# CUHK-AIM-Group/Depth-Aware-Endoscopy-SR

Hardware: AMD Instinct MI355X
Metric: LR frames/sec fwd+bwd at x8 (128x160 LR) (higher is better)
Workload: dtype f32; 1 GPU; Kvasir x8 synthetic, batch=16 per GPU, fp32, DepthNet nb=16 nf=64 L=256 K=10 (BASELINE.json configs[1]); step = fwd + L1 + dynamic loss + bwd + Adam; global_batch=16, scale=8, parallelism=dp1, mode=train, device=cuda, full=False, hip_graph=False

## Files before the change

### depth-aware-endoscopy-sr_amd/csrc/conv_api.hip

```cpp
#include "dasr_common.h"
#include "conv_kernels.h"

static int check_geom(const ConvGeom& g) {
    if (g.B <= 0 || g.H <= 0 || g.W <= 0 || g.Cin <= 0 || g.Ho <= 0 || g.Wo <= 0 || g.Cout <= 0 || g.KH <= 0 ||
        g.KW <= 0 || g.stride <= 0 || g.pad < 0)
        return DASR_E_SHAPE;
    int eh, ew;
    if (!g.transposed) {
        eh = (g.H + 2 * g.pad - g.KH) / g.stride + 1;
        ew = (g.W + 2 * g.pad - g.KW) / g.stride + 1;
    } else {
        eh = (g.H - 1) * g.stride - 2 * g.pad + g.KH;
        ew = (g.W - 1) * g.stride - 2 * g.pad + g.KW;
    }
    if (eh != g.Ho || ew != g.Wo) return DASR_E_SHAPE;
    return DASR_OK;
}

static int conv2d_fwd_dispatch(const ConvGeom& g, const float* x, const float* w, const float* bias, const float* residual,
                               float* y, int act, int ps_r, void* stream) {
    if (conv_mfma_supported(g)) return conv_mfma_fwd(g, x, w, bias, residual, y, act, ps_r, stream);
    if (conv_c1_supported(g) && ps_r == 1 && !residual) return conv_c1_fwd(g, x, w, bias, y, act, stream);
    if (conv9_mfma_supported(g) && act == DASR_ACT_NONE && ps_r == 1 && !residual)
        return conv9_mfma_fwd(g, x, w, bias, y, stream);
    if (conv_gather_fwd_supported(g) && ps_r == 1 && !residual) return conv_gather_fwd(g, x, w, bias, y, act, stream);
    return conv_direct_fwd(g, x, w, bias, residual, y, act, ps_r, stream);
}
extern "C" int dasr_conv2d_fwd(const float* x, const float* w, const float* bias, const float* residual, float* y,
                               float* y_amax, int B, int H, int W, int Cin, int Ho, int Wo, int Cout, int KH, int KW,
                               int stride, int pad, int transposed, int act, int ps_r, void* stream) {
    DASR_CHECK_PTR(x); DASR_CHECK_PTR(w); DASR_CHECK_PTR(y);
    ConvGeom g{B, H, W, Cin, Ho, Wo, Cout, KH, KW, stride, pad, transposed};
    int rc = check_geom(g);
    if (rc) return rc;
    if (act < 0 || act > 2) return DASR_E_UNSUPPORTED;
    if (ps_r < 1) ps_r = 1;
    if (ps_r > 1 && (Cout % (ps_r * ps_r)) != 0) return DASR_E_SHAPE;
    if (!y_amax) return conv2d_fwd_dispatch(g, x, w, bias, residual, y, act, ps_r, stream);
    if (!conv_mfma_supported(g) && conv_c1_supported(g) && ps_r == 1 && !residual)
        return conv_c1_fwd(g, x, w, bias, y, act, stream, y_amax);
    rc = conv2d_fwd_dispatch(g, x, w, bias, residual, y, act, ps_r, stream);
    if (rc) return rc;
    return absmax_raise(y, (size_t)B * Ho * Wo * Cout, y_amax, stream);
}

extern "C" size_t dasr_conv2d_fwd_stats_workspace(int B, int H, int W, int Cin, int Cout) {
    if (B <= 0 || H <= 0 || W <= 0 || Cin <= 0 || Cout <= 0) return 0;
    ConvGeom g{B, H, W, Cin, H, W, Cout, 3, 3, 1, 1, 0};
    size_t fused = conv_mfma_fwd_stats_supported(g) ? conv_mfma_fwd_stats_workspace(g) : 0;
    size_t plain = dasr_instnorm_stats_workspace(B, H * W, Cout);
    return fused > plain ? fused : plain;
}
extern "C" int dasr_conv2d_fwd_stats(const float* x, const float* w, const float* bias, float* y, float* mean, float* var,
                                     void* workspace, size_t workspace_bytes, int B, int H, int W, int Cin, int Cout,
                                     void* stream) {
    DASR_CHECK_PTR(x); DASR_CHECK_PTR(w); DASR_CHECK_PTR(y); DASR_CHECK_PTR(mean); DASR_CHECK_PTR(var);
    DASR_CHECK_PTR(workspace);
    ConvGeom g{B, H, W, Cin, H, W, Cout, 3, 3, 1, 1, 0};
    int rc = check_geom(g);
    if (rc) return rc;
    if (workspace_bytes < dasr_conv2d_fwd_stats_workspace(B, H, W, Cin, Cout)) return DASR_E_WORKSPACE;
    if (conv_mfma_fwd_stats_supported(g)) return conv_mfma_fwd_stats(g, x, w, bias, y, mean, var, workspace, stream);
    rc = dasr_conv2d_fwd(x, w, bias, nullptr, y, nullptr, B, H, W, Cin, H, W, Cout, 3, 3, 1, 1, 0, DASR_ACT_NONE, 1, stream);
    if (rc) return rc;
    return dasr_instnorm_stats(y, mean, var, workspace, workspace_bytes, B, H * W, Cout, stream);
}

extern "C" int dasr_conv2d_epilogue_bwd(const float* dy, const float* y, float* dconv, float* dconv_amax, int B, int Ho, int Wo,
                                        int Cout, int act, int ps_r, void* stream) {
    DASR_CHECK_PTR(dy); DASR_CHECK_PTR(y); DASR_CHECK_PTR(dconv);
    DASR_CHECK_SHAPE(B > 0 && Ho > 0 && Wo > 0 && Cout > 0);
    if (act < 0 || act > 2) return DASR_E_UNSUPPORTED;
    if (ps_r < 1) ps_r = 1;
    if (ps_r > 1 && (Cout % (ps_r * ps_r)) != 0) return DASR_E_SHAPE;
    ConvGeom g{B, Ho, Wo, 1, Ho, Wo, Cout, 1, 1, 1, 0, 0};
    return conv_epilogue_bwd(g, dy, y, dconv, act, ps_r, stream, dconv_amax);
}

extern "C" int dasr_conv2d_dgrad(const float* dconv, const float* w, float* dx, int accumulate, int B, int H, int W,
                                 int Cin, int Ho, int Wo, int Cout, int KH, int KW, int stride, int pad,
                                 int transposed, void* stream) {
    DASR_CHECK_PTR(dconv); DASR_CHECK_PTR(w); DASR_CHECK_PTR(dx);
    ConvGeom g{B, H, W, Cin, Ho, Wo, Cout, KH, KW, stride, pad, transposed};
    int rc = check_geom(g);
    if (rc) return rc;
    if (conv_mfma_dgrad_supported(g)) return conv_mfma_dgrad(g, dconv, w, dx, accumulate, nullptr, 0, 1, stream);
    if (conv9_mfma_supported(g)) return conv9_mfma_dgrad(g, dconv, w, dx, accumulate, nullptr, 0, 1, stream);
    if (conv_gather_dgrad_supported(g)) return conv_gather_dgrad(g, dconv, w, dx, accumulate, stream);
    return conv_direct_dgrad(g, dconv, w, dx, accumulate, stream);
}

extern "C" size_t dasr_conv2d_wgrad_workspace(int B, int H, int W, int Cin, int Ho, int Wo, int Cout, int KH, int KW,
                                              int stride, int pad, int transposed) {
    ConvGeom g{B, H, W, Cin, Ho, Wo, Cout, KH, KW, stride, pad, transposed};
    if (check_geom(g) == DASR_OK && conv_mfma_wgrad_supported(g)) return conv_mfma_wgrad_workspace(g);
    if (check_geom(g) == DASR_OK && conv9_mfma_supported(g)) return conv9_mfma_wgrad_workspace(g);
    if (check_geom(g) == DASR_OK && conv_gather_wgrad_supported(g)) return conv_gather_wgrad_workspace(g);
    return 0;
}

extern "C" int dasr_conv2d_wgrad(const float* x, const float* dconv, float* dw, float* dbias, void* workspace,
                                 size_t workspace_bytes, int B, int H, int W, int Cin, int Ho, int Wo, int Cout, int KH,
                                 int KW, int stride, int pad, int transposed, void* stream) {
    DASR_CHECK_PTR(x); DASR_CHECK_PTR(dconv); DASR_CHECK_PTR(dw);
    ConvGeom g{B, H, W, Cin, Ho, Wo, Cout, KH, KW, stride, pad, transposed};
    int rc = check_geom(g);
    if (rc) return rc;
    if (conv_c1_supported(g)) return conv_c1_wgrad(g, x, dconv, nullptr, DASR_ACT_NONE, dw, dbias, stream);
    if (conv_mfma_wgrad_supported(g)) {
        if (!workspace) return DASR_E_NULL;
        if (workspace_bytes < conv_mfma_wgrad_workspace(g)) return DASR_E_WORKSPACE;
        return conv_mfma_wgrad(g, x, dconv, dw, dbias, workspace, stream);
    } else if (conv9_mfma_supported(g)) {
        if (!workspace) return DASR_E_NULL;
        if (workspace_bytes < conv9_mfma_wgrad_workspace(g)) return DASR_E_WORKSPACE;
        rc = conv9_mfma_wgrad(g, x, dconv, dw, workspace, stream);
    } else if (conv_gather_wgrad_supported(g)) {
        if (!workspace) return DASR_E_NULL;
        if (workspace_bytes < conv_gather_wgrad_workspace(g)) return DASR_E_WORKSPACE;
        rc = conv_gather_wgrad(g, x, dconv, dw, workspace, stream);
    } else {
        rc = conv_direct_wgrad(g, x, dconv, dw, stream);
    }
    if (rc) return rc;
    if (dbias) rc = conv_colsum(dconv, dbias, (size_t)B * Ho * Wo, Cout, stream);
    return rc;
}

extern "C" int dasr_conv2d_wgrad_act(const float* x, const float* dy, const float* y, float* dw, float* dbias,
                                     float* dconv_scratch, void* workspace, size_t workspace_bytes, int B, int H, int W,
                                     int Cin, int Ho, int Wo, int Cout, int KH, int KW, int stride, int pad,
                                     int transposed, int act, void* stream) {
    DASR_CHECK_PTR(x); DASR_CHECK_PTR(dy); DASR_CHECK_PTR(y); DASR_CHECK_PTR(dw);
    ConvGeom g{B, H, W, Cin, Ho, Wo, Cout, KH, KW, stride, pad, transposed};
    int rc = check_geom(g);
    if (rc) return rc;
    if (act < 0 || act > 2) return DASR_E_UNSUPPORTED;
    if (conv_c1_supported(g)) return conv_c1_wgrad(g, x, dy, y, act, dw, dbias, stream);
    DASR_CHECK_PTR(dconv_scratch);
    rc = conv_epilogue_bwd(g, dy, y, dconv_scratch, act, 1, stream);
    if (rc) return rc;
    return dasr_conv2d_wgrad(x, dconv_scratch, dw, dbias, workspace, workspace_bytes, B, H, W, Cin, Ho, Wo, Cout, KH, KW,
                             stride, pad, transposed, stream);
}

extern "C" int dasr_conv2d_wgrad_act_fused(int B, int H, int W, int Cin, int Ho, int Wo, int Cout, int KH, int KW,
                                           int stride, int pad, int transposed) {
    ConvGeom g{B, H, W, Cin, Ho, Wo, Cout, KH, KW, stride, pad, transposed};
    if (check_geom(g) != DASR_OK) return 0;
    return conv_c1_supported(g) ? 1 : 0;
}

extern "C" int dasr_conv2d_dgrad_act_supported(int B, int H, int W, int Cin, int Ho, int Wo, int Cout, int KH, int KW,
                                               int stride, int pad, int transposed, int ps_r) {
    ConvGeom g{B, H, W, Cin, Ho, Wo, Cout, KH, KW, stride, pad, transposed};
    if (check_geom(g) != DASR_OK) return 0;
    if (ps_r < 1) ps_r = 1;
    if ((H % ps_r) != 0 || (W % ps_r) != 0) return 0;
    return (conv_mfma_dgrad_supported(g) || conv9_mfma_supported(g)) ? 1 : 0;
}

extern "C" int dasr_conv2d_dgrad_act(const float* dconv, const float* w, const float* x_act, float* dprev, int B, int H,
                                     int W, int Cin, int Ho, int Wo, int Cout, int KH, int KW, int stride, int pad,
                                     int transposed, int act, int ps_r, void* stream) {
    DASR_CHECK_PTR(dconv); DASR_CHECK_PTR(w); DASR_CHECK_PTR(x_act); DASR_CHECK_PTR(dprev);
    if (act < 0 || act > 2) return DASR_E_UNSUPPORTED;
    if (!dasr_conv2d_dgrad_act_supported(B, H, W, Cin, Ho, Wo, Cout, KH, KW, stride, pad, transposed, ps_r))
        return DASR_E_UNSUPPORTED;
    ConvGeom g{B, H, W, Cin, Ho, Wo, Cout, KH, KW, stride, pad, transposed};
    if (conv_mfma_dgrad_supported(g)) return conv_mfma_dgrad(g, dconv, w, dprev, 0, x_act, act, ps_r, stream);
    return conv9_mfma_dgrad(g, dconv, w, dprev, 0, x_act, act, ps_r, stream);
}

static int bf16_kind(const ConvGeom& g) {
    if (conv_bf16_supported(g)) return 1;
    if (conv_c1_supported(g)) return 2;
    if (conv9_mfma_supported(g)) return 3;
    return 0;
}
extern "C" int dasr_conv2d_fwd_bf16(const void* x, const void* w, const float* bias, const unsigned short* residual,
                                    void* y, int B, int H, int W, int Cin, int Ho, int Wo, int Cout, int KH, int KW,
                                    int stride, int pad, int transposed, int act, int ps_r, void* stream) {
    DASR_CHECK_PTR(x); DASR_CHECK_PTR(w); DASR_CHECK_PTR(y);
    ConvGeom g{B, H, W, Cin, Ho, Wo, Cout, KH, KW, stride, pad, transposed};
    int rc = check_geom(g);
    if (rc) return rc;
    if (act < 0 || act > 2) return DASR_E_UNSUPPORTED;
    if (ps_r < 1) ps_r = 1;
    if (ps_r > 1 && (Cout % (ps_r * ps_r)) != 0) return DASR_E_SHAPE;
    switch (bf16_kind(g)) {
        case 1:
            return conv_bf16_fwd(g, (const bf16_t*)x, (const bf16_t*)w, bias, (const bf16_t*)residual, (bf16_t*)y, act, ps_r,
                                 stream);
        case 2:
            if (ps_r != 1 || residual) return DASR_E_UNSUPPORTED;
            return conv_c1_fwd_bf16(g, (const float*)x, (const float*)w, bias, (bf16_t*)y, act, stream);
        case 3:
            if (ps_r != 1 || residual || act != DASR_ACT_NONE) return DASR_E_UNSUPPORTED;
            return conv9_bf16_fwd(g, (const bf16_t*)x, (const float*)w, bias, (float*)y, stream);
    }
    return DASR_E_UNSUPPORTED;
}
extern "C" int dasr_conv2d_epilogue_bwd_bf16(const unsigned short* dy, const unsigned short* y, unsigned short* dconv,
                                             int B, int Ho, int Wo, int Cout, int act, int ps_r, void* stream) {
    DASR_CHECK_PTR(dy); DASR_CHECK_PTR(y); DASR_CHECK_PTR(dconv);
    DASR_CHECK_SHAPE(B > 0 && Ho > 0 && Wo > 0 && Cout > 0);
    if (act < 0 || act > 2) return DASR_E_UNSUPPORTED;
    if (ps_r < 1) ps_r = 1;
    if (ps_r > 1 && (Cout % (ps_r * ps_r)) != 0) return DASR_E_SHAPE;
    ConvGeom g{B, Ho, Wo, 1, Ho, Wo, Cout, 1, 1, 1, 0, 0};
    return conv_epilogue_bwd_bf16(g, (const bf16_t*)dy, (const bf16_t*)y, (bf16_t*)dconv, act, ps_r, stream);
}
extern "C" int dasr_conv2d_dgrad_bf16(const void* dconv, const void* w, unsigned short* dx, int accumulate, int B, int H,
                                      int W, int Cin, int Ho, int Wo, int Cout, int KH, int KW, int stride, int pad,
                                      int transposed, void* stream) {
    DASR_CHECK_PTR(dconv); DASR_CHECK_PTR(w); DASR_CHECK_PTR(dx);
    ConvGeom g{B, H, W, Cin, Ho, Wo, Cout, KH, KW, stride, pad, transposed};
    int rc = check_geom(g);
    if (rc) return rc;
    if (conv_bf16_dgrad_supported(g))
        return conv_bf16_dgrad(g, (const bf16_t*)dconv, (const bf16_t*)w, (bf16_t*)dx, accumulate, stream);
    if (conv9_mfma_supported(g))
        return conv9_bf16_dgrad(g, (const float*)dconv, (const float*)w, (bf16_t*)dx, accumulate, stream);
    return DASR_E_UNSUPPORTED;
}
extern "C" size_t dasr_conv2d_wgrad_workspace_bf16(int B, int H, int W, int Cin, int Ho, int Wo, int Cout, int KH, int KW,
                                                   int stride, int pad, int transposed) {
    ConvGeom g{B, H, W, Cin, Ho, Wo, Cout, KH, KW, stride, pad, transposed};
    if (check_geom(g) != DASR_OK) return 0;
    if (conv_bf16_wgrad_supported(g)) return conv_bf16_wgrad_workspace(g);
    if (conv9_mfma_supported(g)) return conv9_bf16_wgrad_workspace(g);
    return 0;
}
extern "C" int dasr_conv2d_wgrad_bf16(const unsigned short* x, const void* dconv, float* dw, float* dbias, void* workspace,
                                      size_t workspace_bytes, int B, int H, int W, int Cin, int Ho, int Wo, int Cout, int KH,
                                      int KW, int stride, int pad, int transposed, void* stream) {
    DASR_CHECK_PTR(x); DASR_CHECK_PTR(dconv); DASR_CHECK_PTR(dw); DASR_CHECK_PTR(workspace);
    ConvGeom g{B, H, W, Cin, Ho, Wo, Cout, KH, KW, stride, pad, transposed};
    int rc = check_geom(g);
    if (rc) return rc;
    if (conv_bf16_wgrad_supported(g)) {
        if (workspace_bytes < conv_bf16_wgrad_workspace(g)) return DASR_E_WORKSPACE;
        return conv_bf16_wgrad(g, (const bf16_t*)x, (const bf16_t*)dconv, dw, dbias, workspace, stream);
    }
    if (conv9_mfma_supported(g)) {
        if (workspace_bytes < conv9_bf16_wgrad_workspace(g)) return DASR_E_WORKSPACE;
        rc = conv9_bf16_wgrad(g, (const bf16_t*)x, (const float*)dconv, dw, workspace, stream);
        if (rc) return rc;
        if (dbias) rc = conv_colsum((const float*)dconv, dbias, (size_t)B * Ho * Wo, Cout, stream);
        return rc;
    }
    return DASR_E_UNSUPPORTED;
}
extern "C" int dasr_conv2d_wgrad_act_bf16(const float* x, const unsigned short* dy, const unsigned short* y, float* dw,
                                          float* dbias, int B, int H, int W, int Cin, int Ho, int Wo, int Cout, int KH,
                                          int KW, int stride, int pad, int transposed, int act, void* stream) {
    DASR_CHECK_PTR(x); DASR_CHECK_PTR(dy); DASR_CHECK_PTR(y); DASR_CHECK_PTR(dw);
    ConvGeom g{B, H, W, Cin, Ho, Wo, Cout, KH, KW, stride, pad, transposed};
    int rc = check_geom(g);
    if (rc) return rc;
    if (act < 0 || act > 2) return DASR_E_UNSUPPORTED;
    if (!conv_c1_supported(g)) return DASR_E_UNSUPPORTED;
    return conv_c1_wgrad_bf16(g, x, (const bf16_t*)dy, (const bf16_t*)y, act, dw, dbias, stream);
}
```

### depth-aware-endoscopy-sr_amd/csrc/conv_c1.hip

```cpp
#include "dasr_common.h"
#include "bf16.h"
#include "conv_kernels.h"

#define C1_MAXW 4096
template <int CIN>
__device__ __forceinline__ void c1_stage_rows(const float* __restrict__ x, float* sRow, int b, int y, int H, int W) {
    const float* xb = x + (size_t)b * H * W * CIN;
    const int RW = (W + 2) * CIN, n = 3 * RW;
    for (int i0 = threadIdx.x; i0 < n; i0 += 4 * 256) {
        float v[4];
        bool in[4];
#pragma unroll
        for (int u = 0; u < 4; ++u) {
            const int i = i0 + 256 * u < n ? i0 + 256 * u : 0;
            const int r = i / RW, c = i - r * RW;
            const int iy = y + r - 1, ix = c / CIN - 1;
            in[u] = iy >= 0 && iy < H && ix >= 0 && ix < W;
            v[u] = xb[in[u] ? ((size_t)iy * W + ix) * CIN + c % CIN : 0];
        }
#pragma unroll
        for (int u = 0; u < 4; ++u)
            if (i0 + 256 * u < n) sRow[i0 + 256 * u] = in[u] ? v[u] : 0.f;
    }
}

template <typename T, int CIN>
__global__ void __launch_bounds__(256) k_conv3x3_c1_fwd(const float* __restrict__ x, const float* __restrict__ w,
                                                        const float* __restrict__ bias, T* __restrict__ y, int B,
                                                        int H, int W, int Cout, int act, float* __restrict__ amax) {
    DASR_DYN_SMEM(smem);
    float* sRow = (float*)smem;
    const int nq = Cout / 4;
    const int q = threadIdx.x % nq, pl = threadIdx.x / nq, npl = 256 / nq;
    constexpr int NT = 9 * CIN;
    const int RW = (W + 2) * CIN;
    float4 wt[NT];
#pragma unroll
    for (int t = 0; t < NT; ++t) wt[t] = *(const float4*)(w + (size_t)t * Cout + 4 * q);
    const float4 bv = bias ? *(const float4*)(bias + 4 * q) : make_float4(0.f, 0.f, 0.f, 0.f);
    const float slope = act == DASR_ACT_LRELU02 ? 0.2f : 1.f;
    const bool relu = act == DASR_ACT_RELU;
    auto neg = [&](float v) { return relu ? 0.f : slope * v; };
    float om = 0.f;
    for (int row = blockIdx.x; row < B * H; row += gridDim.x) {
        const int b = row / H, py = row - b * H;
        __syncthreads();
        c1_stage_rows<CIN>(x, sRow, b, py, H, W);
        __syncthreads();
        T* yrow = y + ((size_t)row * W) * Cout + 4 * q;
        for (int px = pl; px < W; px += npl) {
            float4 acc = bv;
#pragma unroll
            for (int t = 0; t < NT; ++t) {
                const float d = sRow[(t / (3 * CIN)) * RW + (px + (t / CIN) % 3) * CIN + t % CIN];
                acc.x = fmaf(d, wt[t].x, acc.x); acc.y = fmaf(d, wt[t].y, acc.y);
                acc.z = fmaf(d, wt[t].z, acc.z); acc.w = fmaf(d, wt[t].w, acc.w);
            }
            acc.x = acc.x > 0.f ? acc.x : neg(acc.x); acc.y = acc.y > 0.f ? acc.y : neg(acc.y);
            acc.z = acc.z > 0.f ? acc.z : neg(acc.z); acc.w = acc.w > 0.f ? acc.w : neg(acc.w);
            st4(yrow + (size_t)px * Cout, acc);
            om = dasr_amax4(om, acc);
        }
    }
    if (amax) dasr_amax_commit(amax, om, sRow, dasr_flat_wg(), dasr_flat_nwg());
}

template <typename T, int CIN, bool HASY>
__global__ void __launch_bounds__(256) k_conv3x3_c1_wgrad(const float* __restrict__ x, const T* __restrict__ dy,
                                                          const T* __restrict__ yact, float* __restrict__ dw,
                                                          float* __restrict__ dbias, int B, int H, int W, int Cout,
                                                          int act) {
    DASR_DYN_SMEM(smem);
    constexpr int NT = 9 * CIN;
    const int RW = (W + 2) * CIN;
    float* red = (float*)smem;
    float* sRow = red + 256 * 4;
    const int nq = Cout / 4;
    const int q = threadIdx.x % nq, pl = threadIdx.x / nq, npl = 256 / nq;
    const float slope = act == DASR_ACT_RELU ? 0.f : act == DASR_ACT_LRELU02 ? 0.2f : 1.f;
    float4 acc[NT + 1];
#pragma unroll
    for (int t = 0; t < NT + 1; ++t) acc[t] = make_float4(0.f, 0.f, 0.f, 0.f);
    constexpr int NPX = sizeof(T) == 2 ? 8 : 4;
    typedef typename raw4<T>::type Raw;
    Raw gq[NPX], yq[NPX];
    const int nrows = B * H, step = NPX * npl;
    auto issue = [&](int row, int base) {
        const size_t ro = ((size_t)row * W) * Cout + 4 * q;
#pragma unroll
        for (int u = 0; u < NPX; ++u) {
            const int px = base + pl + u * npl < W ? base + pl + u * npl : W - 1;
            gq[u] = ld4_raw(dy + ro + (size_t)px * Cout);
            if (HASY) yq[u] = ld4_raw(yact + ro + (size_t)px * Cout);
        }
    };
    if ((int)blockIdx.x < nrows) issue(blockIdx.x, 0);
    for (int row = blockIdx.x; row < nrows; row += gridDim.x) {
        const int b = row / H, py = row - b * H;
        __syncthreads();
        c1_stage_rows<CIN>(x, sRow, b, py, H, W);
        __syncthreads();
        for (int base = 0; base < W; base += step) {
            float4 g[NPX];
#pragma unroll
            for (int u = 0; u < NPX; ++u) {
                g[u] = cvt4<T>(gq[u]);
                if (HASY) {
                    const float4 yv = cvt4<T>(yq[u]);
                    g[u].x *= yv.x > 0.f ? 1.f : slope; g[u].y *= yv.y > 0.f ? 1.f : slope;
                    g[u].z *= yv.z > 0.f ? 1.f : slope; g[u].w *= yv.w > 0.f ? 1.f : slope;
                }
            }
            {
                int nb = base + step, nr = row;
                if (nb >= W) {
                    nb = 0;
                    nr = row + (int)gridDim.x < nrows ? row + (int)gridDim.x : row;
                }
                DASR_SCHED_BARRIER();
                issue(nr, nb);
                DASR_SCHED_BARRIER();
            }
#pragma unroll
            for (int u = 0; u < NPX; ++u) {
                const int px = base + pl + u * npl;
                if (px >= W) g[u] = make_float4(0.f, 0.f, 0.f, 0.f);
                const int pc = px < W ? px : W - 1;
                acc[NT].x += g[u].x; acc[NT].y += g[u].y; acc[NT].z += g[u].z; acc[NT].w += g[u].w;
#pragma unroll
                for (int t = 0; t < NT; ++t) {
                    const float d = sRow[(t / (3 * CIN)) * RW + (pc + (t / CIN) % 3) * CIN + t % CIN];
                    acc[t].x = fmaf(d, g[u].x, acc[t].x); acc[t].y = fmaf(d, g[u].y, acc[t].y);
                    acc[t].z = fmaf(d, g[u].z, acc[t].z); acc[t].w = fmaf(d, g[u].w, acc[t].w);
                }
            }
        }
    }
#pragma unroll
    for (int t = 0; t < NT + 1; ++t) {
        __syncthreads();
        *(float4*)(red + threadIdx.x * 4) = acc[t];
        __syncthreads();
        for (int co = threadIdx.x; co < Cout; co += 256) {
            const int qq = co / 4, j = co % 4;
            float s = 0.f;
            for (int l = 0; l < npl; ++l) s += red[(l * nq + qq) * 4 + j];
            if (t < NT) atomicAdd(&dw[(size_t)t * Cout + co], s);
            else if (dbias) atomicAdd(&dbias[co], s);
        }
    }
}

__global__ void __launch_bounds__(256) k_c1_zero(float* __restrict__ dw, int nw, float* __restrict__ dbias, int nb) {
    const int i = blockIdx.x * 256 + threadIdx.x;
    if (i < nw) dw[i] = 0.f;
    else if (dbias && i < nw + nb) dbias[i - nw] = 0.f;
}

bool conv_c1_supported(const ConvGeom& g) {
    return g.KH == 3 && g.KW == 3 && g.stride == 1 && g.pad == 1 && !g.transposed && (g.Cin == 1 || g.Cin == 3) &&
           (g.Cout % 4) == 0 && g.Cout <= (g.Cin == 1 ? 1024 : 256) && (256 % (g.Cout / 4)) == 0 && g.H == g.Ho &&
           g.W == g.Wo && g.W <= C1_MAXW;
}
template <typename T>
static int conv_c1_fwd_impl(const ConvGeom& g, const float* x, const float* w, const float* bias, T* y, int act, void* stream,
                            float* amax = nullptr) {
    unsigned grid = (unsigned)(g.B * g.H);
    if (grid > 256 * 8) grid = 256 * 8;
    const size_t lds = sizeof(float) * 3 * (g.W + 2) * g.Cin;
    if (g.Cin == 3) DASR_LAUNCH((k_conv3x3_c1_fwd<T, 3>), dim3(grid), dim3(256), lds, stream, x, w, bias, y, g.B, g.H, g.W, g.Cout, act, amax);
    else            DASR_LAUNCH((k_conv3x3_c1_fwd<T, 1>), dim3(grid), dim3(256), lds, stream, x, w, bias, y, g.B, g.H, g.W, g.Cout, act, amax);
    DASR_RETURN_LAUNCH_STATUS();
}
int conv_c1_fwd(const ConvGeom& g, const float* x, const float* w, const float* bias, float* y, int act, void* stream,
                float* amax) {
    return conv_c1_fwd_impl<float>(g, x, w, bias, y, act, stream, amax);
}
int conv_c1_fwd_bf16(const ConvGeom& g, const float* x, const float* w, const float* bias, bf16_t* y, int act, void* stream) {
    return conv_c1_fwd_impl<bf16_t>(g, x, w, bias, y, act, stream);
}
template <typename T>
static int conv_c1_wgrad_impl(const ConvGeom& g, const float* x, const T* dy, const T* yact, int act, float* dw, float* dbias,
                              void* stream) {
    DASR_LAUNCH(k_c1_zero, dim3(dasr_cdiv((size_t)(9 * g.Cin + 1) * g.Cout, 256)), dim3(256), 0, stream, dw, 9 * g.Cin * g.Cout,
                dbias, g.Cout);
    unsigned grid = (unsigned)(g.B * g.H);
#ifndef C1_WGRAD_WGS_BF16
#define C1_WGRAD_WGS_BF16 1024
#endif
#ifndef C1_WGRAD_WGS_F32
#define C1_WGRAD_WGS_F32 512
#endif
    const unsigned cap = sizeof(T) == 2 ? C1_WGRAD_WGS_BF16 : C1_WGRAD_WGS_F32;
    if (grid > cap) grid = cap;
    const size_t lds = sizeof(float) * (256 * 4 + 3 * (g.W + 2) * g.Cin);
#define C1_WGRAD(CIN, HASY) \
    DASR_LAUNCH((k_conv3x3_c1_wgrad<T, CIN, HASY>), dim3(grid), dim3(256), lds, stream, x, dy, yact, dw, dbias, g.B, g.H, g.W, g.Cout, act)
    const bool hasy = yact != nullptr && act != DASR_ACT_NONE;
    if (g.Cin == 3) { if (hasy) C1_WGRAD(3, true); else C1_WGRAD(3, false); }
    else            { if (hasy) C1_WGRAD(1, true); else C1_WGRAD(1, false); }
#undef C1_WGRAD
    DASR_RETURN_LAUNCH_STATUS();
}
int conv_c1_wgrad(const ConvGeom& g, const float* x, const float* dy, const float* yact, int act, float* dw, float* dbias,
                  void* stream) {
    return conv_c1_wgrad_impl<float>(g, x, dy, yact, act, dw, dbias, stream);
}
int conv_c1_wgrad_bf16(const ConvGeom& g, const float* x, const bf16_t* dy, const bf16_t* yact, int act, float* dw,
                       float* dbias, void* stream) {
    return conv_c1_wgrad_impl<bf16_t>(g, x, dy, yact, act, dw, dbias, stream);
}
```

### depth-aware-endoscopy-sr_amd/csrc/conv_direct.hip

```cpp
#include "dasr_common.h"
#include "bf16.h"
#include "conv_kernels.h"

__global__ void __launch_bounds__(256) k_conv_direct_fwd(ConvGeom g, const float* __restrict__ x,
                                                         const float* __restrict__ w, const float* __restrict__ bias,
                                                         const float* __restrict__ residual, float* __restrict__ y,
                                                         int act, int ps_r) {
    size_t n = (size_t)g.B * g.Ho * g.Wo * g.Cout;
    for (size_t idx = (size_t)blockIdx.x * blockDim.x + threadIdx.x; idx < n; idx += (size_t)gridDim.x * blockDim.x) {
        int co = (int)(idx % g.Cout);
        size_t pix = idx / g.Cout;
        int ox = (int)(pix % g.Wo), oy = (int)((pix / g.Wo) % g.Ho), b = (int)(pix / ((size_t)g.Wo * g.Ho));
        float acc = bias ? bias[co] : 0.f;
        for (int kh = 0; kh < g.KH; ++kh) {
            int iy;
            if (!g.transposed) {
                iy = oy * g.stride - g.pad + kh;
            } else {
                int ty = oy + g.pad - kh;
                if (ty < 0 || (ty % g.stride) != 0) continue;
                iy = ty / g.stride;
            }
            if (iy < 0 || iy >= g.H) continue;
            for (int kw = 0; kw < g.KW; ++kw) {
// ... 16 lines not shown
        y[conv_out_index(g, b, oy, ox, co, ps_r)] = acc;
    }
}

template <typename T>
__global__ void __launch_bounds__(256) k_conv_epilogue_bwd(ConvGeom g, const T* __restrict__ dy,
                                                           const T* __restrict__ y, T* __restrict__ dconv,
                                                           int act, int ps_r, float* __restrict__ amax) {
    __shared__ float s_part[16];
    size_t n = (size_t)g.B * g.Ho * g.Wo * g.Cout;
    float om = 0.f;
    for (size_t idx = (size_t)blockIdx.x * blockDim.x + threadIdx.x; idx < n; idx += (size_t)gridDim.x * blockDim.x) {
        int co = (int)(idx % g.Cout);
        size_t pix = idx / g.Cout;
        int ox = (int)(pix % g.Wo), oy = (int)((pix / g.Wo) % g.Ho), b = (int)(pix / ((size_t)g.Wo * g.Ho));
        size_t o = conv_out_index(g, b, oy, ox, co, ps_r);
        const float v = ld1(dy + o) * dasr_act_grad_from_out(ld1(y + o), act);
        st1(dconv + idx, v);
        om = dasr_amax1(om, v);
    }
    if (amax) dasr_amax_commit(amax, om, s_part, dasr_flat_wg(), dasr_flat_nwg());
}

__global__ void __launch_bounds__(256) k_conv_direct_dgrad(ConvGeom g, const float* __restrict__ dconv,
                                                           const float* __restrict__ w, float* __restrict__ dx,
                                                           int accumulate) {
    size_t n = (size_t)g.B * g.H * g.W * g.Cin;
    for (size_t idx = (size_t)blockIdx.x * blockDim.x + threadIdx.x; idx < n; idx += (size_t)gridDim.x * blockDim.x) {
        int ci = (int)(idx % g.Cin);
        size_t pix = idx / g.Cin;
        int ix = (int)(pix % g.W), iy = (int)((pix / g.W) % g.H), b = (int)(pix / ((size_t)g.W * g.H));
        float acc = 0.f;
        for (int kh = 0; kh < g.KH; ++kh) {
            int oy;
            if (!g.transposed) {
                int ty = iy + g.pad - kh;
                if (ty < 0 || (ty % g.stride) != 0) continue;
                oy = ty / g.stride;
            } else {
                oy = iy * g.stride - g.pad + kh;
            }
            if (oy < 0 || oy >= g.Ho) continue;
            for (int kw = 0; kw < g.KW; ++kw) {
                int ox;
                if (!g.transposed) {
                    int tx = ix + g.pad - kw;
                    if (tx < 0 || (tx % g.stride) != 0) continue;
                    ox = tx / g.stride;
                } else {
                    ox = ix * g.stride - g.pad + kw;
                }
                if (ox < 0 || ox >= g.Wo) continue;
                const float* dp = dconv + (((size_t)b * g.Ho + oy) * g.Wo + ox) * g.Cout;
                const float* wp = w + ((size_t)(kh * g.KW + kw) * g.Cin + ci) * g.Cout;
                for (int co = 0; co < g.Cout; ++co) acc = fmaf(dp[co], wp[co], acc);
            }
        }
        dx[idx] = accumulate ? dx[idx] + acc : acc;
    }
}

__global__ void __launch_bounds__(256) k_conv_direct_wgrad(ConvGeom g, const float* __restrict__ x,
                                                           const float* __restrict__ dconv, float* __restrict__ dw,
                                                           size_t pix_per_split) {
    size_t nW = (size_t)g.KH * g.KW * g.Cin * g.Cout;
    size_t e = (size_t)blockIdx.x * blockDim.x + threadIdx.x;
    if (e >= nW) return;
    int co = (int)(e % g.Cout);
    int ci = (int)((e / g.Cout) % g.Cin);
    int tap = (int)(e / ((size_t)g.Cout * g.Cin));
    int kh = tap / g.KW, kw = tap % g.KW;
    size_t npix = (size_t)g.B * g.Ho * g.Wo;
    size_t p0 = (size_t)blockIdx.y * pix_per_split;
    size_t p1 = p0 + pix_per_split < npix ? p0 + pix_per_split : npix;
    float acc = 0.f;
    for (size_t p = p0; p < p1; ++p) {
        int ox = (int)(p % g.Wo), oy = (int)((p / g.Wo) % g.Ho), b = (int)(p / ((size_t)g.Wo * g.Ho));
        int iy, ix;
        if (!g.transposed) {
            iy = oy * g.stride - g.pad + kh;
            ix = ox * g.stride - g.pad + kw;
        } else {
            int ty = oy + g.pad - kh, tx = ox + g.pad - kw;
            if (ty < 0 || tx < 0 || (ty % g.stride) != 0 || (tx % g.stride) != 0) continue;
            iy = ty / g.stride;
            ix = tx / g.stride;
        }
        if (iy < 0 || iy >= g.H || ix < 0 || ix >= g.W) continue;
        acc = fmaf(x[(((size_t)b * g.H + iy) * g.W + ix) * g.Cin + ci], dconv[p * g.Cout + co], acc);
    }
    atomicAdd(&dw[e], acc);
}

__global__ void __launch_bounds__(256) k_colsum(const float* __restrict__ m, float* __restrict__ out, size_t rows,
                                                int C, size_t rows_per_split) {
    __shared__ float red[256];
    int c = blockIdx.x * 64 + (threadIdx.x & 63);
    int rl = threadIdx.x >> 6;
    size_t r0 = (size_t)blockIdx.y * rows_per_split;
    size_t r1 = r0 + rows_per_split < rows ? r0 + rows_per_split : rows;
    float acc = 0.f;
    if (c < C)
        for (size_t r = r0 + rl; r < r1; r += 4) acc += m[r * C + c];
    red[threadIdx.x] = acc;
    __syncthreads();
    if (rl == 0 && c < C) atomicAdd(&out[c], red[threadIdx.x] + red[threadIdx.x + 64] + red[threadIdx.x + 128] +
                                                 red[threadIdx.x + 192]);
}

__global__ void __launch_bounds__(256) k_colsum_small(const float* __restrict__ m, float* __restrict__ out, size_t rows,
                                                      int C) {
    __shared__ float red[8][4];
    float acc[8];
#pragma unroll
    for (int c = 0; c < 8; ++c) acc[c] = 0.f;
    for (size_t r = (size_t)blockIdx.x * 256 + threadIdx.x; r < rows; r += (size_t)gridDim.x * 256) {
        const float* p = m + r * C;
#pragma unroll
        for (int c = 0; c < 8; ++c)
            if (c < C) acc[c] += p[c];
    }
#pragma unroll
    for (int c = 0; c < 8; ++c) {
        float v = acc[c];
        for (int off = 32; off > 0; off >>= 1) v += __shfl_down(v, off, 64);
        if ((threadIdx.x & 63) == 0) red[c][threadIdx.x >> 6] = v;
    }
    __syncthreads();
    if (threadIdx.x < C) atomicAdd(&out[threadIdx.x], red[threadIdx.x][0] + red[threadIdx.x][1] + red[threadIdx.x][2] +
                                                          red[threadIdx.x][3]);
}

int conv_direct_fwd(const ConvGeom& g, const float* x, const float* w, const float* bias, const float* residual,
                    float* y, int act, int ps_r, void* stream) {
    size_t n = (size_t)g.B * g.Ho * g.Wo * g.Cout;
    DASR_LAUNCH(k_conv_direct_fwd, dim3(dasr_ew_grid(n)), dim3(256), 0, stream, g, x, w, bias, residual, y, act, ps_r);
    DASR_RETURN_LAUNCH_STATUS();
}
template <typename T>
__global__ void __launch_bounds__(256) k_conv_epilogue_bwd_flat4(const T* __restrict__ dy, const T* __restrict__ y,
                                                                 T* __restrict__ dconv, size_t n4, int act,
                                                                 float* __restrict__ amax) {
    __shared__ float s_part[16];
    float om = 0.f;
    for (size_t i = (size_t)blockIdx.x * blockDim.x + threadIdx.x; i < n4; i += (size_t)gridDim.x * blockDim.x) {
        const float4 d = ld4(dy + 4 * i), v = ld4(y + 4 * i);
        const float4 o = make_float4(d.x * dasr_act_grad_from_out(v.x, act), d.y * dasr_act_grad_from_out(v.y, act),
                                     d.z * dasr_act_grad_from_out(v.z, act), d.w * dasr_act_grad_from_out(v.w, act));
        st4(dconv + 4 * i, o);
        om = dasr_amax4(om, o);
    }
    if (amax) dasr_amax_commit(amax, om, s_part, dasr_flat_wg(), dasr_flat_nwg());
}
template <int R, typename T>
__global__ void __launch_bounds__(256) k_conv_epilogue_bwd_ps(const T* __restrict__ dy, const T* __restrict__ y,
                                                              T* __restrict__ dconv, int Wo, int Cq, int act, int rows,
                                                              float* __restrict__ amax) {
    __shared__ float s_part[16];
    const int e0 = blockIdx.x * 256 + threadIdx.x;
    const bool livee = e0 < Wo * Cq;
    const int e = livee ? e0 : Wo * Cq - 1;
    const int ox = e / Cq, c = e - ox * Cq;
    const size_t srow = (size_t)Wo * R * Cq;
    float om = 0.f;
    for (size_t row0 = blockIdx.y; row0 < (size_t)rows; row0 += 2 * (size_t)gridDim.y) {
        const size_t row1 = row0 + gridDim.y;
        const bool two = row1 < (size_t)rows;
        const size_t rws[2] = {row0, two ? row1 : row0};
        float out[2][R * R];
#pragma unroll
        for (int h = 0; h < 2; ++h) {
            const T* dyp = dy + rws[h] * R * srow + (size_t)ox * R * Cq + c;
            const T* yp = y + rws[h] * R * srow + (size_t)ox * R * Cq + c;
#pragma unroll
            for (int i = 0; i < R; ++i)
#pragma unroll
                for (int j = 0; j < R; ++j) {
                    const size_t o = (size_t)i * srow + (size_t)j * Cq;
                    out[h][i * R + j] = ld1(dyp + o) * dasr_act_grad_from_out(ld1(yp + o), act);
                }
        }
#pragma unroll
        for (int h = 0; h < 2; ++h) {
            if (h == 1 && !two) break;
            T* dst = dconv + (rws[h] * Wo + ox) * (size_t)(Cq * R * R) + (size_t)c * (R * R);
            if (livee) {
                if (R == 2) {
                    st4(dst, make_float4(out[h][0], out[h][1], out[h][2], out[h][3]));
                } else {
#pragma unroll
                    for (int q = 0; q < R * R; ++q) st1(dst + q, out[h][q]);
                }
            }
#pragma unroll
            for (int q = 0; q < R * R; ++q) om = dasr_amax1(om, out[h][q]);
        }
    }
    if (amax) dasr_amax_commit(amax, om, s_part, dasr_flat_wg(), dasr_flat_nwg());
}

template <typename T>
static int conv_epilogue_bwd_impl(const ConvGeom& g, const T* dy, const T* y, T* dconv, int act, int ps_r, void* stream,
                                  float* amax = nullptr) {
    size_t n = (size_t)g.B * g.Ho * g.Wo * g.Cout;
    const size_t rows = (size_t)g.B * g.Ho;
    if (ps_r <= 1 && (n % 4) == 0) {
        DASR_LAUNCH((k_conv_epilogue_bwd_flat4<T>), dim3(dasr_ew_grid(n / 4)), dim3(256), 0, stream, dy, y, dconv, n / 4, act, amax);
    } else if ((ps_r == 2 || ps_r == 3) && (g.Cout % (ps_r * ps_r)) == 0 && rows < ((size_t)1 << 31) &&
               (size_t)g.Wo * (g.Cout / (ps_r * ps_r)) < (1u << 30)) {
        const int Cq = g.Cout / (ps_r * ps_r);
        const unsigned gx = dasr_cdiv((size_t)g.Wo * Cq, 256);
        size_t gy = rows < 65535 ? rows : 65535;
        if (amax && (size_t)gx * gy > DASR_AMAX_MAX_PARTS) gy = DASR_AMAX_MAX_PARTS / gx > 0 ? DASR_AMAX_MAX_PARTS / gx : 1;
        if (amax && (size_t)gx * gy > DASR_AMAX_MAX_PARTS) return DASR_E_UNSUPPORTED;
        const dim3 grid(gx, (unsigned)gy);
        if (ps_r == 2)
            DASR_LAUNCH((k_conv_epilogue_bwd_ps<2, T>), grid, dim3(256), 0, stream, dy, y, dconv, g.Wo, Cq, act, (int)rows, amax);
        else
            DASR_LAUNCH((k_conv_epilogue_bwd_ps<3, T>), grid, dim3(256), 0, stream, dy, y, dconv, g.Wo, Cq, act, (int)rows, amax);
    } else {
        DASR_LAUNCH((k_conv_epilogue_bwd<T>), dim3(dasr_ew_grid(n)), dim3(256), 0, stream, g, dy, y, dconv, act, ps_r, amax);
    }
    DASR_RETURN_LAUNCH_STATUS();
}
int conv_epilogue_bwd(const ConvGeom& g, const float* dy, const float* y, float* dconv, int act, int ps_r, void* stream,
                      float* amax) {
    return conv_epilogue_bwd_impl<float>(g, dy, y, dconv, act, ps_r, stream, amax);
}
int conv_epilogue_bwd_bf16(const ConvGeom& g, const bf16_t* dy, const bf16_t* y, bf16_t* dconv, int act, int ps_r,
                           void* stream) {
    return conv_epilogue_bwd_impl<bf16_t>(g, dy, y, dconv, act, ps_r, stream);
}
int conv_direct_dgrad(const ConvGeom& g, const float* dconv, const float* w, float* dx, int accumulate, void* stream) {
    size_t n = (size_t)g.B * g.H * g.W * g.Cin;
    DASR_LAUNCH(k_conv_direct_dgrad, dim3(dasr_ew_grid(n)), dim3(256), 0, stream, g, dconv, w, dx, accumulate);
    DASR_RETURN_LAUNCH_STATUS();
}
int conv_colsum(const float* m, float* out, size_t rows, int C, void* stream) {
    hipError_t e = hipMemsetAsync(out, 0, sizeof(float) * C, (hipStream_t)stream);
    if (e != hipSuccess) return (int)e;
    if (C <= 8) {
        DASR_LAUNCH(k_colsum_small, dim3(dasr_ew_grid(rows)), dim3(256), 0, stream, m, out, rows, C);
        DASR_RETURN_LAUNCH_STATUS();
    }
    unsigned nsplit = (unsigned)((rows + 255) / 256);
    if (nsplit > 2048) nsplit = 2048;
    if (nsplit < 1) nsplit = 1;
    size_t rps = (rows + nsplit - 1) / nsplit;
    DASR_LAUNCH(k_colsum, dim3(dasr_cdiv(C, 64), nsplit), dim3(256), 0, stream, m, out, rows, C, rps);
    DASR_RETURN_LAUNCH_STATUS();
}
int conv_direct_wgrad(const ConvGeom& g, const float* x, const float* dconv, float* dw, void* stream) {
    size_t nW = (size_t)g.KH * g.KW * g.Cin * g.Cout;
    hipError_t e = hipMemsetAsync(dw, 0, sizeof(float) * nW, (hipStream_t)stream);
    if (e != hipSuccess) return (int)e;
    size_t npix = (size_t)g.B * g.Ho * g.Wo;
    unsigned gx = dasr_cdiv(nW, 256);
    unsigned nsplit = 4096 / gx;
    if (nsplit < 1) nsplit = 1;
    size_t max_split = (npix + 63) / 64;
    if (nsplit > max_split) nsplit = (unsigned)max_split;
    if (nsplit > 65535) nsplit = 65535;
    size_t pps = (npix + nsplit - 1) / nsplit;
    DASR_LAUNCH(k_conv_direct_wgrad, dim3(gx, nsplit), dim3(256), 0, stream, g, x, dconv, dw, pps);
    DASR_RETURN_LAUNCH_STATUS();
}
```

### depth-aware-endoscopy-sr_amd/csrc/conv_kernels.h

```cpp
#pragma once
#include "dasr_common.h"
#include "bf16.h"

struct ConvGeom {
    int B, H, W, Cin, Ho, Wo, Cout, KH, KW, stride, pad, transposed;
};

__host__ __device__ __forceinline__ size_t conv_out_index(const ConvGeom& g, int b, int oy, int ox, int co, int ps_r) {
    if (ps_r <= 1) return (((size_t)b * g.Ho + oy) * g.Wo + ox) * g.Cout + co;
    int rr = ps_r * ps_r;
    int c = co / rr, i = (co / ps_r) % ps_r, j = co % ps_r;
    return (((size_t)b * g.Ho * ps_r + (size_t)oy * ps_r + i) * ((size_t)g.Wo * ps_r) + (size_t)ox * ps_r + j) *
               (g.Cout / rr) + c;
}

int conv_direct_fwd(const ConvGeom& g, const float* x, const float* w, const float* bias, const float* residual,
                    float* y, int act, int ps_r, void* stream);
int conv_epilogue_bwd(const ConvGeom& g, const float* dy, const float* y, float* dconv, int act, int ps_r,
                      void* stream, float* amax = nullptr);
int conv_direct_dgrad(const ConvGeom& g, const float* dconv, const float* w, float* dx, int accumulate, void* stream);
int conv_direct_wgrad(const ConvGeom& g, const float* x, const float* dconv, float* dw, void* stream);
int conv_colsum(const float* m, float* out, size_t rows, int C, void* stream);

bool conv_mfma_supported(const ConvGeom& g);
bool conv_mfma_fwd_stats_supported(const ConvGeom& g);
size_t conv_mfma_fwd_stats_workspace(const ConvGeom& g);
int conv_mfma_fwd_stats(const ConvGeom& g, const float* x, const float* w, const float* bias, float* y, float* mean,
                        float* var, void* workspace, void* stream);
bool conv_mfma_dgrad_supported(const ConvGeom& g);
bool conv_mfma_wgrad_supported(const ConvGeom& g);
int conv_mfma_fwd(const ConvGeom& g, const float* x, const float* w, const float* bias, const float* residual,
                  float* y, int act, int ps_r, void* stream);
int conv_mfma_dgrad(const ConvGeom& g, const float* dconv, const float* w, float* dx, int accumulate,
                    const float* mask_src, int mask_act, int unps_r, void* stream);
size_t conv_mfma_wgrad_workspace(const ConvGeom& g);
int conv_mfma_wgrad(const ConvGeom& g, const float* x, const float* dconv, float* dw, float* dbias, void* workspace,
                    void* stream);

bool conv9_mfma_supported(const ConvGeom& g);
int conv9_mfma_fwd(const ConvGeom& g, const float* x, const float* w, const float* bias, float* y, void* stream);
int conv9_mfma_dgrad(const ConvGeom& g, const float* dconv, const float* w, float* dx, int accumulate,
                     const float* mask_src, int mask_act, int unps_r, void* stream);
size_t conv9_mfma_wgrad_workspace(const ConvGeom& g);
int conv9_mfma_wgrad(const ConvGeom& g, const float* x, const float* dconv, float* dw, void* workspace, void* stream);

bool conv_gather_fwd_supported(const ConvGeom& g);
bool conv_gather_dgrad_supported(const ConvGeom& g);
bool conv_gather_wgrad_supported(const ConvGeom& g);
int conv_gather_fwd(const ConvGeom& g, const float* x, const float* w, const float* bias, float* y, int act,
                    void* stream);
int conv_gather_dgrad(const ConvGeom& g, const float* dconv, const float* w, float* dx, int accumulate, void* stream);
size_t conv_gather_wgrad_workspace(const ConvGeom& g);
int conv_gather_wgrad(const ConvGeom& g, const float* x, const float* dconv, float* dw, void* workspace, void* stream);
int wgrad_reduce_launch(const float* slabs, float* dw, size_t n, int P, void* stream, const float* bslabs = nullptr,
                        float* dbias = nullptr, int Cout = 0);

bool conv_c1_supported(const ConvGeom& g);
int conv_c1_fwd(const ConvGeom& g, const float* x, const float* w, const float* bias, float* y, int act, void* stream,
                float* amax = nullptr);
int absmax_raise(const float* x, size_t n, float* amax, void* stream);
int conv_c1_wgrad(const ConvGeom& g, const float* x, const float* dy, const float* yact, int act, float* dw, float* dbias,
                  void* stream);

bool conv_bf16_supported(const ConvGeom& g);
bool conv_bf16_dgrad_supported(const ConvGeom& g);
bool conv_bf16_wgrad_supported(const ConvGeom& g);
int conv_bf16_fwd(const ConvGeom& g, const bf16_t* x, const bf16_t* w, const float* bias, const bf16_t* residual,
                  bf16_t* y, int act, int ps_r, void* stream);
int conv_bf16_dgrad(const ConvGeom& g, const bf16_t* dconv, const bf16_t* w, bf16_t* dx, int accumulate, void* stream);
size_t conv_bf16_wgrad_workspace(const ConvGeom& g);
int conv_bf16_wgrad(const ConvGeom& g, const bf16_t* x, const bf16_t* dconv, float* dw, float* dbias, void* workspace,
                    void* stream);
bool conv_bf16_v2_supported(int H, int W, int Cin, int Cout, int ps_r, bool has_residual, bool accumulate);
int conv_bf16_v2_fwd(const ConvGeom& g, const bf16_t* x, const bf16_t* w, const float* bias, const bf16_t* residual,
                     bf16_t* y, int act, int ps_r, void* stream);
int conv_bf16_v2_dgrad(const ConvGeom& g, const bf16_t* dconv, const bf16_t* w, bf16_t* dx, int accumulate, void* stream);
int conv_epilogue_bwd_bf16(const ConvGeom& g, const bf16_t* dy, const bf16_t* y, bf16_t* dconv, int act, int ps_r,
                           void* stream);
int conv_c1_fwd_bf16(const ConvGeom& g, const float* x, const float* w, const float* bias, bf16_t* y, int act, void* stream);
int conv_c1_wgrad_bf16(const ConvGeom& g, const float* x, const bf16_t* dy, const bf16_t* yact, int act, float* dw,
                       float* dbias, void* stream);
int conv9_bf16_fwd(const ConvGeom& g, const bf16_t* x, const float* w, const float* bias, float* y, void* stream);
int conv9_bf16_dgrad(const ConvGeom& g, const float* dconv, const float* w, bf16_t* dx, int accumulate, void* stream);
size_t conv9_bf16_wgrad_workspace(const ConvGeom& g);
int conv9_bf16_wgrad(const ConvGeom& g, const bf16_t* x, const float* dconv, float* dw, void* workspace, void* stream);

bool conv9_split_supported(const ConvGeom& g);
int conv9_split_fwd(const ConvGeom& g, const float* x, const float* xmax, const float* w, const float* wmax, const float* bias,
                    float* y, void* stream);
int conv9_split_dgrad(const ConvGeom& g, const float* dconv, const float* dmax, const float* w, const float* wmax, float* dx,
                      int accumulate, void* stream);
size_t conv9_split_wgrad_workspace(const ConvGeom& g);
int conv9_split_wgrad(const ConvGeom& g, const float* x, const float* xmax, const float* dconv, const float* dmax, float* dw,
                      void* workspace, void* stream);
```

### depth-aware-endoscopy-sr_amd/csrc/conv_split_bf16.hip

```cpp
#include "bf16.h"
#include "conv_kernels.h"

typedef _Float16 f16_t;
typedef _Float16 f16x8 __attribute__((ext_vector_type(8)));
typedef _Float16 f16x2_t __attribute__((ext_vector_type(2)));

#define SP_HW 34
#define SP_NWV 8
#define SP_NTHR 512
#define SP_TH 16
#define SP_HPIX (18 * SP_HW)
#define SP_NHP 5
#define SP_HBYTES (SP_NHP * SP_NTHR * 16)
#define SP_EPITCH 144

DASR_DEVICE_CONST __attribute__((aligned(64))) unsigned sp_zero_page[64] = {0};

struct ConvSplitArgs {
    const float* x;
    const bf16_t* ws;
    const float* bias;
    const float* residual;
    float* y;
    int B, H, W, Cin, Cout, accumulate, act, ps_r;
    int tiles_x, tiles_y, nsl, nitems, Q, G8;
    const float* xmax;
    const float* wmax;
    float* ymax;
};

template <int N>
__device__ __forceinline__ void sp_wait_vm() {
#ifndef DASR_HIPEMU
    asm volatile("s_waitcnt vmcnt(%0)" ::"n"(N) : "memory");
#endif
}

__device__ __forceinline__ void sp_wait_vm_n(int n) {
    switch (n) {
#define SP_W(N) case N: sp_wait_vm<N>(); break;
        SP_W(0) SP_W(1) SP_W(2) SP_W(3) SP_W(4) SP_W(5) SP_W(6) SP_W(7) SP_W(8) SP_W(9) SP_W(10) SP_W(11) SP_W(12)
#undef SP_W
        default: sp_wait_vm<0>(); break;
    }
}

__device__ __forceinline__ void sp_split3(const float (&x)[8], bf16x8& a0, bf16x8& a1, bf16x8& a2) {
#pragma unroll
    for (int e = 0; e < 8; e += 2) {
        const bf16x2_t h0 = dasr_f2bf2(x[e], x[e + 1]);
        const float r0 = x[e] - dasr_bf2f(h0[0]), r1 = x[e + 1] - dasr_bf2f(h0[1]);
        const bf16x2_t h1 = dasr_f2bf2(r0, r1);
        const float s0 = r0 - dasr_bf2f(h1[0]), s1 = r1 - dasr_bf2f(h1[1]);
        const bf16x2_t h2 = dasr_f2bf2(s0, s1);
        a0[e] = h0[0]; a0[e + 1] = h0[1];
        a1[e] = h1[0]; a1[e + 1] = h1[1];
        a2[e] = h2[0]; a2[e + 1] = h2[1];
    }
}

__host__ __device__ static inline int sp_scale_exp(float m) {
    unsigned u;
    memcpy(&u, &m, 4);
    int k = 14 - ((int)((u >> 23) & 0xffu) - 127);
    return k < -60 ? -60 : (k > 60 ? 60 : k);
}
__host__ __device__ static inline float sp_pow2(int k) {
    const unsigned u = (unsigned)(127 + k) << 23;
    float f;
    memcpy(&f, &u, 4);
    return f;
}
__device__ __forceinline__ void sp_split2(const float (&x)[8], float s, f16x8& a0, f16x8& a1) {
#pragma unroll
    for (int e = 0; e < 8; e += 2) {
        const float v0 = x[e] * s, v1 = x[e + 1] * s;
        const f16_t h0 = (f16_t)v0, g0 = (f16_t)v1;
        a0[e] = h0; a0[e + 1] = g0;
        a1[e] = (f16_t)(v0 - (float)h0); a1[e + 1] = (f16_t)(v1 - (float)g0);
    }
}
template <int NP> struct SpFrag;
template <> struct SpFrag<3> {
    typedef bf16x8 type;
    typedef bf16_t elem;
    static __device__ __forceinline__ void split(const float (&x)[8], float, type (&a)[3]) { sp_split3(x, a[0], a[1], a[2]); }
    static __device__ __forceinline__ f32x16 mma(const type (&w)[3], const type (&x)[3], f32x16 c) {
        c = __builtin_amdgcn_mfma_f32_32x32x16_bf16(w[2], x[0], c, 0, 0, 0);
        c = __builtin_amdgcn_mfma_f32_32x32x16_bf16(w[1], x[1], c, 0, 0, 0);
        c = __builtin_amdgcn_mfma_f32_32x32x16_bf16(w[0], x[2], c, 0, 0, 0);
        c = __builtin_amdgcn_mfma_f32_32x32x16_bf16(w[1], x[0], c, 0, 0, 0);
        c = __builtin_amdgcn_mfma_f32_32x32x16_bf16(w[0], x[1], c, 0, 0, 0);
        c = __builtin_amdgcn_mfma_f32_32x32x16_bf16(w[0], x[0], c, 0, 0, 0);
        return c;
    }
};
template <> struct SpFrag<2> {
    typedef f16x8 type;
    typedef f16_t elem;
    static __device__ __forceinline__ void split(const float (&x)[8], float s, type (&a)[2]) { sp_split2(x, s, a[0], a[1]); }
    static __device__ __forceinline__ f32x16 mma(const type (&w)[2], const type (&x)[2], f32x16 c) {
        c = __builtin_amdgcn_mfma_f32_32x32x16_f16(w[1], x[0], c, 0, 0, 0);
        c = __builtin_amdgcn_mfma_f32_32x32x16_f16(w[0], x[1], c, 0, 0, 0);
        c = __builtin_amdgcn_mfma_f32_32x32x16_f16(w[0], x[0], c, 0, 0, 0);
        return c;
    }
};
struct SpScale { float sx, inv; };
__device__ __forceinline__ float sp_amax_share(const float* buf) {
    int n;
    memcpy(&n, buf, 4);
    float m = 0.f;
    for (int i = threadIdx.x; i < n; i += blockDim.x) m = fmaxf(m, buf[1 + i]);
#pragma unroll
    for (int o = 32; o > 0; o >>= 1) m = fmaxf(m, __shfl_xor(m, o));
    return m;
}
template <int NP>
__device__ __forceinline__ void sp_scales_gather(const float* xmax, const float* wmax, float* s_red) {
    if (NP == 2) {
        const float mx = sp_amax_share(xmax), mw = sp_amax_share(wmax);
        if ((threadIdx.x & 63) == 0) {
            s_red[threadIdx.x >> 6] = mx;
            s_red[16 + (threadIdx.x >> 6)] = mw;
        }
    }
}
template <int NP>
__device__ __forceinline__ SpScale sp_scales_take(const float* s_red) {
    SpScale r = {1.f, 1.f};
    if (NP == 2) {
        const int nw = (int)(blockDim.x >> 6);
        float mx = s_red[0], mw = s_red[16];
        for (int w = 1; w < nw; ++w) { mx = fmaxf(mx, s_red[w]); mw = fmaxf(mw, s_red[16 + w]); }
        const int kx = sp_scale_exp(mx), kw = sp_scale_exp(mw);
        r.sx = sp_pow2(kx);
        r.inv = sp_pow2(-(kx + kw));
    }
    return r;
}

typedef _Float16 f16x4 __attribute__((ext_vector_type(4)));
template <int NWV = SP_NWV>
__device__ __forceinline__ void sp_presplit(char* hb, float sx, int tid) {
    constexpr int NHP = SP_HBYTES / (1024 * NWV);
    float4 raw[NHP];
#pragma unroll
    for (int u = 0; u < NHP; ++u) raw[u] = *(const float4*)(hb + 1024 * NWV * u + 16 * tid);
#pragma unroll
    for (int u = 0; u < NHP; ++u) {
        const float f[4] = {raw[u].x * sx, raw[u].y * sx, raw[u].z * sx, raw[u].w * sx};
        f16x8 o;
#pragma unroll
        for (int j = 0; j < 4; ++j) {
            const f16_t h0 = (f16_t)f[j];
            o[j] = h0;
            o[4 + j] = (f16_t)(f[j] - (float)h0);
        }
        *(f16x8*)(hb + 1024 * NWV * u + 16 * tid) = o;
    }
}
__device__ __forceinline__ f16x8 sp_frag(const char* px, int lh, int key, int pl) {
    const f16x4 lo = *(const f16x4*)(px + ((((2 * lh) ^ key)) << 4) + 8 * pl);
    const f16x4 hi = *(const f16x4*)(px + ((((2 * lh + 1) ^ key)) << 4) + 8 * pl);
    f16x8 r;
    __builtin_memcpy(&r, &lo, 8);
    __builtin_memcpy((char*)&r + 8, &hi, 8);
    return r;
}

template <int NT, int NP, int RW = 2>
__device__ __forceinline__ void sp_epilogue(f32x16 (&acc)[RW][NT], const ConvSplitArgs& a, char* const scr, const float* sBias,
                                            const float inv, const int x0, const int y0, const int n0, const int bb,
                                            const int rbase, const int lane, const int li, const int lh, float& om) {
    const int wvalid = a.W - x0;
    const bool is_relu = a.act == DASR_ACT_RELU;
    const float slope = a.act == DASR_ACT_LRELU02 ? 0.2f : 1.f;
    const bool has_act = a.act != DASR_ACT_NONE;
#pragma unroll
    for (int m = 0; m < RW; ++m) {
        const int gy = y0 + rbase + m;
#pragma unroll
        for (int n = 0; n < NT; ++n) {
#pragma unroll
            for (int g = 0; g < 4; ++g) {
                f32x4 pk = {acc[m][n][4 * g], acc[m][n][4 * g + 1], acc[m][n][4 * g + 2], acc[m][n][4 * g + 3]};
                *(f32x4*)(scr + li * SP_EPITCH + (8 * g + 4 * lh) * 4) = pk;
            }
            DASR_WAVE_SYNC();
            if (gy < a.H) {
                if (a.ps_r == 1) {
#pragma unroll
                    for (int u = 0; u < 2; ++u) {
                        const int v = lane + 64 * u, pix = v >> 2, cg = v & 3;
                        if (pix >= wvalid) continue;
                        const float4 lo = *(const float4*)(scr + pix * SP_EPITCH + 32 * cg);
                        const float4 hi = *(const float4*)(scr + pix * SP_EPITCH + 32 * cg + 16);
                        float o[8] = {lo.x, lo.y, lo.z, lo.w, hi.x, hi.y, hi.z, hi.w};
                        if (NP == 2) {
                            const float* bp = sBias + n0 + 32 * n + 8 * cg;
#pragma unroll
                            for (int t = 0; t < 8; ++t) o[t] = fmaf(o[t], inv, bp[t]);
                        }
                        const size_t idx = (((size_t)bb * a.H + gy) * a.W + x0 + pix) * a.Cout + n0 + 32 * n + 8 * cg;
                        if (a.residual) {
                            const float4 r0 = *(const float4*)(a.residual + idx), r1 = *(const float4*)(a.residual + idx + 4);
                            o[0] += r0.x; o[1] += r0.y; o[2] += r0.z; o[3] += r0.w;
                            o[4] += r1.x; o[5] += r1.y; o[6] += r1.z; o[7] += r1.w;
                        }
                        if (has_act) {
#pragma unroll
                            for (int t = 0; t < 8; ++t) o[t] = is_relu ? fmaxf(o[t], 0.f) : fmaxf(o[t], o[t] * slope);
                        }
                        float* yp = a.y + idx;
                        if (a.accumulate) {
                            const float4 o0 = *(const float4*)yp, o1 = *(const float4*)(yp + 4);
                            o[0] += o0.x; o[1] += o0.y; o[2] += o0.z; o[3] += o0.w;
                            o[4] += o1.x; o[5] += o1.y; o[6] += o1.z; o[7] += o1.w;
                        }
                        *(float4*)yp = make_float4(o[0], o[1], o[2], o[3]);
                        *(float4*)(yp + 4) = make_float4(o[4], o[5], o[6], o[7]);
                        om = dasr_amax4(dasr_amax4(om, make_float4(o[0], o[1], o[2], o[3])), make_float4(o[4], o[5], o[6], o[7]));
                    }
                } else {
                    const int Cq = a.Cout / 4;
#pragma unroll
                    for (int u = 0; u < 2; ++u) {
                        const int v = lane + 64 * u, j = v & 1, pix = (v >> 1) & 31, i = v >> 6;
                        if (pix >= wvalid) continue;
                        const float* sp = (const float*)(scr + pix * SP_EPITCH) + 2 * i + j;
                        float o[8];
#pragma unroll
                        for (int t = 0; t < 8; ++t) {
                            const float q = NP == 2 ? fmaf(sp[4 * t], inv, sBias[n0 + 32 * n + 4 * t + 2 * i + j]) : sp[4 * t];
                            o[t] = !has_act ? q : (is_relu ? fmaxf(q, 0.f) : fmaxf(q, q * slope));
                        }
                        float* yp = a.y + (((size_t)bb * a.H * 2 + 2 * gy + i) * ((size_t)a.W * 2) + 2 * (x0 + pix) + j) * Cq +
                                    (n0 + 32 * n) / 4;
                        *(float4*)yp = make_float4(o[0], o[1], o[2], o[3]);
                        *(float4*)(yp + 4) = make_float4(o[4], o[5], o[6], o[7]);
                        om = dasr_amax4(dasr_amax4(om, make_float4(o[0], o[1], o[2], o[3])), make_float4(o[4], o[5], o[6], o[7]));
                    }
                }
            }
            DASR_WAVE_SYNC();
        }
    }
}

template <int NT, int NP, int RW = 2, int CW = 1>
__global__ void __launch_bounds__(64 * (SP_TH / RW), RW == 4 ? 1 : 2) k_conv3x3_split(ConvSplitArgs a) {
    DASR_DYN_SMEM(smem);
    typedef SpFrag<NP> F;
    static_assert(CW == 1 || (CW == 2 && NP == 2 && RW == 2 && (NT % 2) == 0), "channel halves: fp16 x 2, eight waves");
    constexpr int MR = RW * CW, NW = NT / CW;
    constexpr int NWV = SP_TH / RW, NTHR = 64 * NWV, NHP = SP_HBYTES / (16 * NTHR);
    constexpr int NTILE = 32 * NT, PIECE = NTILE * 32, SLAB = NP * PIECE;
    constexpr int WP = SLAB / 16;
    constexpr int WQ = WP / NTHR, WR = (WP - WQ * NTHR) / 64;
    char* const sH = smem;
    constexpr int TPS = NP == 2 ? 3 : 1, NS = 9 / TPS;
    constexpr int R = 3, D = 2;
    char* const sW = smem + 2 * SP_HBYTES;
    float* const sBias = (float*)(sW + R * TPS * SLAB);
    float* const sRed = sBias + a.Cout;
    const int tid = threadIdx.x, lane = tid & 63, wv = DASR_UNIFORM((int)(tid >> 6));
    const int li = lane & 31, lh = lane >> 5;
    const int wr = wv / CW, wc = wv % CW;
    const int nwq = WQ + (wv < WR ? 1 : 0);
    const dasr_lds_addr_t ldsH = DASR_LDS_ADDR(sH) + 1024 * wv, ldsW = DASR_LDS_ADDR(sW) + 1024 * wv;

    const int xcd = blockIdx.x & 7, jwg = blockIdx.x >> 3;
    const int ibeg = xcd * a.Q;
    const int iend = ibeg + a.Q < a.nitems ? ibeg + a.Q : a.nitems;
    int item = ibeg + jwg;
    if (item >= iend) {
        if (a.ymax) dasr_amax_commit_idle(a.ymax, dasr_flat_wg(), dasr_flat_nwg());
        return;
    }
    const int NC = a.Cin >> 4;
    const int pixb = a.Cin * 4, rowb = a.W * pixb;
    const size_t sampb = (size_t)a.H * rowb;
    const char* const zp = (const char*)sp_zero_page;

    for (int i = tid; i < a.Cout; i += NTHR) sBias[i] = a.bias ? a.bias[i] : 0.f;
    sp_scales_gather<NP>(a.xmax, a.wmax, sRed);
    __syncthreads();
    const SpScale sc = sp_scales_take<NP>(sRed);

    int x0, y0, n0, bb;
    auto decode = [&](int it, int& ox0, int& oy0, int& on0, int& ob) {
        const int ns = it % a.nsl, pt = it / a.nsl;
        const int tile = pt % (a.tiles_x * a.tiles_y);
        ob = pt / (a.tiles_x * a.tiles_y);
        ox0 = (tile % a.tiles_x) * 32;
        oy0 = (tile / a.tiles_x) * SP_TH;
        on0 = ns * NTILE;
    };
    decode(item, x0, y0, n0, bb);
    int hoff[NHP];
    unsigned hok = 0;
    const char* hxb;
    auto halo_setup = [&](int fx0, int fy0, int fb, bool real) {
        hxb = (const char*)a.x + (size_t)fb * sampb;
        const int org = (fy0 - 1) * rowb + (fx0 - 1) * pixb;
        int t = tid;
#ifndef DASR_HIPEMU
        asm volatile("" : "+v"(t));
#endif
        hok = 0;
#pragma unroll
        for (int u = 0; u < NHP; ++u) {
            const int P = (t >> 2) + (NTHR / 4) * u;
            const int pr = P / SP_HW, pc = P - pr * SP_HW;
            hoff[u] = org + pr * rowb + pc * pixb + 16 * ((t & 3) ^ ((P >> 2) & 3));
            const bool ok = real && P < SP_HPIX && (unsigned)(fy0 - 1 + pr) < (unsigned)a.H && (unsigned)(fx0 - 1 + pc) < (unsigned)a.W;
            hok |= ok ? (1u << u) : 0u;
        }
    };
    auto halo_issue = [&](int u, int cc, int buf) {
        const char* src = ((hok >> u) & 1u) ? hxb + hoff[u] + 64 * cc : zp;
        DASR_GLDS16(src, ldsH + buf * SP_HBYTES + 1024 * NWV * u);
    };
    auto w_issue = [&](int cc, int st, int fn0) {
#pragma unroll
        for (int j = 0; j < TPS; ++j) {
            const int tap = CW == 2 ? 3 * j + st : TPS * st + j;
            const char* src = (const char*)a.ws + (size_t)(((fn0 / NTILE) * 9 + tap) * NC + cc) * SLAB + 16 * tid;
            const dasr_lds_addr_t dst = ldsW + ((st % R) * TPS + j) * SLAB;
#pragma unroll
            for (int q = 0; q < WQ; ++q) DASR_GLDS16(src + 16 * NTHR * q, dst + 1024 * NWV * q);
            if (WR > 0 && wv < WR) DASR_GLDS16(src + 16 * NTHR * WQ, dst + 1024 * NWV * WQ);
        }
    };
    constexpr int HC0 = (NHP + 1) / 2;
    auto halo_first = [](int st) { return TPS == 1 ? st : (st == 0 ? 0 : (st == 1 ? HC0 : NHP)); };
    auto halo_count = [](int st) { return TPS == 1 ? (st < NHP ? 1 : 0) : (st == 0 ? HC0 : (st == 1 ? NHP - HC0 : 0)); };

    const int Pl = MR * wr * SP_HW + li;
    const int boff = li * 32 + ((lh ^ ((li >> 3) & 1)) << 4) + wc * NW * 1024;

    int par = 0;
    float om = 0.f;
    halo_setup(x0, y0, bb, true);
#pragma unroll
    for (int u = 0; u < NHP; ++u) halo_issue(u, 0, 0);
#pragma unroll
    for (int t = 0; t < D; ++t) w_issue(0, t, n0);

    for (;;) {
        const int nitem = item + a.G8;
        const bool has_next = nitem < iend;
        int nx0 = x0, ny0 = y0, nn0 = n0, nb = bb;
        if (has_next) decode(nitem, nx0, ny0, nn0, nb);

        f32x16 acc[MR][NW];
#pragma unroll
        for (int n = 0; n < NW; ++n)
#pragma unroll
            for (int g = 0; g < 4; ++g) {
                float4 bv = *(const float4*)(sBias + n0 + 32 * n + 8 * g + 4 * lh);
                if (NP == 2) bv = make_float4(0.f, 0.f, 0.f, 0.f);
#pragma unroll
                for (int m = 0; m < MR; ++m) {
                    acc[m][n][4 * g] = bv.x; acc[m][n][4 * g + 1] = bv.y;
                    acc[m][n][4 * g + 2] = bv.z; acc[m][n][4 * g + 3] = bv.w;
                }
            }

        for (int cc = 0; cc < NC; ++cc) {
            const bool last = cc == NC - 1;
            if (last) halo_setup(nx0, ny0, nb, has_next);
            const int fcc = last ? 0 : cc + 1;
            const char* const hb = sH + par * SP_HBYTES;
#pragma unroll
            for (int st = 0; st < NS; ++st) {
                {
                    int nh = 0;
#pragma unroll
                    for (int k = 1; k < D; ++k) nh += halo_count((st - k + NS) % NS);
                    sp_wait_vm_n(nh + (D - 1) * TPS * nwq);
                }
                if (NP == 2 && st == 0) {
                    sp_presplit<NWV>(sH + par * SP_HBYTES, sc.sx, tid);
                    DASR_LDS_BARRIER();
                } else {
                    DASR_RAW_BARRIER();
                }
#pragma unroll
                for (int u = 0; u < halo_count(st); ++u) halo_issue(halo_first(st) + u, fcc, par ^ 1);
                if (st + D < NS) w_issue(cc, st + D, n0);
                else             w_issue(fcc, st + D - NS, last ? nn0 : n0);
                if constexpr (CW == 2) {
                    int Pq = Pl;
#ifndef DASR_HIPEMU
                    asm volatile("" : "+v"(Pq));
#endif
                    typename F::type A6[MR + 2][NP];
#pragma unroll
                    for (int r = 0; r < MR + 2; ++r) {
// ... 292 lines not shown
    while (lo < hi) {
        const int mid = (lo + hi + 1) >> 1;
        if (jobs[mid].wg_begin <= (int)blockIdx.x) lo = mid; else hi = mid - 1;
    }
    const dasr_split_job J = jobs[lo];
    sp_split_weights<2>(J.w_packed, J.w_split, J.Cin, J.Cout, J.wmax, blockIdx.x - J.wg_begin, 1 << 30);
}

__global__ void __launch_bounds__(256) k_absmax(const float* __restrict__ x, size_t n4, size_t n, float* __restrict__ out) {
    __shared__ float s_part[16];
    unsigned m = 0;
    const size_t stride = (size_t)gridDim.x * 256;
    if (n4 > 0)
        for (size_t i = (size_t)blockIdx.x * 256 + threadIdx.x; i < n4; i += 4 * stride) {
            float4 v[4];
#pragma unroll
            for (int u = 0; u < 4; ++u) {
                const size_t j = i + u * stride;
                v[u] = ((const float4*)x)[j < n4 ? j : n4 - 1];
            }
#pragma unroll
            for (int u = 0; u < 4; ++u) {
                unsigned a, b, c, d;
                memcpy(&a, &v[u].x, 4); memcpy(&b, &v[u].y, 4); memcpy(&c, &v[u].z, 4); memcpy(&d, &v[u].w, 4);
                a &= 0x7fffffffu; b &= 0x7fffffffu; c &= 0x7fffffffu; d &= 0x7fffffffu;
                a = a > b ? a : b; c = c > d ? c : d; a = a > c ? a : c;
                m = m > a ? m : a;
            }
        }
    if (blockIdx.x == 0)
        for (size_t i = 4 * n4 + threadIdx.x; i < n; i += 256) {
            unsigned a;
            memcpy(&a, x + i, 4);
            a &= 0x7fffffffu;
            m = m > a ? m : a;
        }
#pragma unroll
    for (int o = 32; o > 0; o >>= 1) {
        const unsigned t = (unsigned)__shfl_xor((int)m, o);
        m = m > t ? m : t;
    }
    if ((threadIdx.x & 63) == 0) memcpy(&s_part[threadIdx.x >> 6], &m, 4);
    __syncthreads();
    if (threadIdx.x == 0) {
        unsigned r[4];
        memcpy(r, s_part, 16);
        unsigned a = r[0] > r[1] ? r[0] : r[1], b = r[2] > r[3] ? r[2] : r[3];
        a = a > b ? a : b;
        memcpy(&out[1 + blockIdx.x], &a, 4);
        if (blockIdx.x == 0) {
            const int np = (int)gridDim.x;
            memcpy(out, &np, 4);
        }
    }
}

static bool sp_ok(int H, int W, int K, int N) {
    return H > 0 && W > 0 && (K % 16) == 0 && (N % 32) == 0 && N <= 1024 && (size_t)H * W * (K > N ? K : N) * 4 < ((size_t)1 << 31);
}
extern "C" int dasr_conv3x3_split_supported(int H, int W, int Cin, int Cout) {
    return (sp_ok(H, W, Cin, Cout) && sp_ok(H, W, Cout, Cin)) ? 1 : 0;
}
int absmax_raise(const float* x, size_t n, float* amax, void* stream) {
    DASR_CHECK_PTR(x); DASR_CHECK_PTR(amax);
    DASR_CHECK_SHAPE(n > 0 && (((size_t)x) & 15) == 0);
    const size_t n4 = n / 4;
    size_t g = (n4 + 256 * 8 - 1) / (256 * 8);
    if (g > 2048) g = 2048;
    if (g < 1) g = 1;
    DASR_LAUNCH(k_absmax, dim3((unsigned)g), dim3(256), 0, stream, x, n4, n, amax);
    DASR_RETURN_LAUNCH_STATUS();
}
extern "C" int dasr_absmax(const float* x, size_t n, float* amax, void* stream) { return absmax_raise(x, n, amax, stream); }
static unsigned sp_weight_slabs_all(int Cin, int Cout) {
    return (unsigned)((Cout / sp_ntile(Cout)) * 9 * (Cin / 16) + (Cin / sp_ntile(Cin)) * 9 * (Cout / 16));
}
static unsigned sp_weight_slabs(int Cin, int Cout) {
    const unsigned n = sp_weight_slabs_all(Cin, Cout);
    return n > 2048 ? 2048 : n;
}
extern "C" size_t dasr_conv3x3_split_weights_bytes(int Cin, int Cout) {
    if (Cin <= 0 || Cout <= 0) return 0;
    return sizeof(bf16_t) * (size_t)54 * Cin * Cout;
}
extern "C" size_t dasr_conv3x3_split2_weights_bytes(int Cin, int Cout) {
    if (Cin <= 0 || Cout <= 0) return 0;
    return sizeof(f16_t) * (size_t)36 * Cin * Cout;
}
extern "C" int dasr_conv3x3_split_weights(const float* w_packed, unsigned short* w_split, int Cin, int Cout, void* stream) {
    DASR_CHECK_PTR(w_packed); DASR_CHECK_PTR(w_split);
    DASR_CHECK_SHAPE(Cin > 0 && Cout > 0 && (Cin % 32) == 0 && (Cout % 32) == 0);
    DASR_LAUNCH((k_split_weights<3>), dim3(sp_weight_slabs(Cin, Cout)), dim3(256), 0, stream, w_packed, w_split, Cin, Cout,
                (const float*)nullptr);
    DASR_RETURN_LAUNCH_STATUS();
}
extern "C" int dasr_conv3x3_split2_weights(const float* w_packed, const float* wmax, unsigned short* w_split, int Cin, int Cout,
                                           void* stream) {
    DASR_CHECK_PTR(w_packed); DASR_CHECK_PTR(w_split); DASR_CHECK_PTR(wmax);
    DASR_CHECK_SHAPE(Cin > 0 && Cout > 0 && (Cin % 32) == 0 && (Cout % 32) == 0);
    DASR_LAUNCH((k_split_weights<2>), dim3(sp_weight_slabs(Cin, Cout)), dim3(256), 0, stream, w_packed, w_split, Cin, Cout,
                wmax);
    DASR_RETURN_LAUNCH_STATUS();
}
extern "C" int dasr_conv3x3_split2_weights_slabs(int Cin, int Cout) {
    if (Cin <= 0 || Cout <= 0 || (Cin % 32) != 0 || (Cout % 32) != 0) return 0;
    return (int)sp_weight_slabs_all(Cin, Cout);
}
extern "C" int dasr_conv3x3_split2_weights_multi(const dasr_split_job* jobs_host, const dasr_split_job* jobs_device, int njobs,
                                                 void* stream) {
    DASR_CHECK_PTR(jobs_host); DASR_CHECK_PTR(jobs_device);
    DASR_CHECK_SHAPE(njobs > 0);
    long long total = 0;
    for (int j = 0; j < njobs; ++j) {
        const dasr_split_job& J = jobs_host[j];
        DASR_CHECK_PTR(J.w_packed); DASR_CHECK_PTR(J.w_split); DASR_CHECK_PTR(J.wmax);
        DASR_CHECK_SHAPE(J.Cin > 0 && J.Cout > 0 && (J.Cin % 32) == 0 && (J.Cout % 32) == 0);
        DASR_CHECK_SHAPE(J.wg_begin == total);
        total += sp_weight_slabs_all(J.Cin, J.Cout);
        DASR_CHECK_SHAPE(total < (1ll << 30));
    }
    DASR_LAUNCH(k_split_weights_multi, dim3((unsigned)total), dim3(256), 0, stream, jobs_device, njobs);
    DASR_RETURN_LAUNCH_STATUS();
}
template <int NP>
static int sp_launch(ConvSplitArgs& a, void* stream) {
    const int NT = sp_ntile(a.Cout) / 32;
    a.tiles_x = (a.W + 31) / 32;
    a.tiles_y = (a.H + SP_TH - 1) / SP_TH;
    a.nsl = a.Cout / (32 * NT);
    a.nitems = a.tiles_x * a.tiles_y * a.B * a.nsl;
    a.Q = (a.nitems + 7) / 8;
    a.G8 = a.Q < 32 ? a.Q : 32;
    if ((dasr_get_conv_bf16_impl() & 3) == 2) a.G8 = 1;
    const bool chunk2 = NT == 2 && NP == 2 && (dasr_get_conv_bf16_impl() & 512) != 0;
    const size_t lds = 2 * (size_t)SP_HBYTES +
                       (NT == 1 || chunk2 ? 2 * (size_t)(9 * NP * 32 * NT * 32) : 3 * (size_t)((NP == 2 ? 3 : 1) * NP * 32 * NT * 32)) +
                       sizeof(float) * (size_t)(a.Cout + 32);
    if (lds > 160 * 1024) return DASR_E_UNSUPPORTED;
    const dim3 grid(8 * a.G8);
    if (NT == 4 && NP == 2 && (dasr_get_conv_bf16_impl() & 256) != 0)
        DASR_LAUNCH((k_conv3x3_split<4, 2, 4>), grid, dim3(256), lds, stream, a);
    else if (NT == 4 && NP == 2 && (dasr_get_conv_bf16_impl() & 1024) == 0)
        DASR_LAUNCH((k_conv3x3_split<4, 2, 2, 2>), grid, dim3(SP_NTHR), lds, stream, a);
    else if (NT == 2 && NP == 2 && (dasr_get_conv_bf16_impl() & 1024) != 0)
        DASR_LAUNCH((k_conv3x3_split<2, 2, 2, 2>), grid, dim3(SP_NTHR), lds, stream, a);
    else if (NT == 4) DASR_LAUNCH((k_conv3x3_split<4, NP>), grid, dim3(SP_NTHR), lds, stream, a);
    else if (chunk2)  DASR_LAUNCH((k_conv3x3_split_n32<2, 2>), grid, dim3(SP_NTHR), lds, stream, a);
    else if (NT == 2) DASR_LAUNCH((k_conv3x3_split<2, NP>), grid, dim3(SP_NTHR), lds, stream, a);
    else              DASR_LAUNCH((k_conv3x3_split_n32<NP>), grid, dim3(SP_NTHR), lds, stream, a);
    DASR_RETURN_LAUNCH_STATUS();
}
static int sp_fwd(const float* x, const float* xmax, const unsigned short* w_split, const float* wmax, const float* bias,
                  const float* residual, float* y, float* ymax, int B, int H, int W, int Cin, int Cout, int act, int ps_r,
                  void* stream) {
    DASR_CHECK_PTR(x); DASR_CHECK_PTR(w_split); DASR_CHECK_PTR(y);
    DASR_CHECK_SHAPE(B > 0);
    if (!dasr_conv3x3_split_supported(H, W, Cin, Cout)) return DASR_E_UNSUPPORTED;
    if (act < 0 || act > 2) return DASR_E_UNSUPPORTED;
    if (ps_r < 1) ps_r = 1;
    if (ps_r > 2 || (ps_r == 2 && (residual != nullptr || (Cout % 128) != 0))) return DASR_E_UNSUPPORTED;
    ConvSplitArgs a{x, (const bf16_t*)w_split, bias, residual, y, B, H, W, Cin, Cout, 0, act, ps_r, 0, 0, 0, 0, 0, 0, xmax, wmax, ymax};
    return xmax ? sp_launch<2>(a, stream) : sp_launch<3>(a, stream);
}
extern "C" int dasr_conv3x3_fwd_split(const float* x, const unsigned short* w_split, const float* bias,
                                      const float* residual, float* y, int B, int H, int W, int Cin, int Cout, int act,
                                      int ps_r, void* stream) {
    return sp_fwd(x, nullptr, w_split, nullptr, bias, residual, y, nullptr, B, H, W, Cin, Cout, act, ps_r, stream);
}
extern "C" int dasr_conv3x3_fwd_split2(const float* x, const float* xmax, const unsigned short* w_split, const float* wmax,
                                       const float* bias, const float* residual, float* y, float* y_amax, int B, int H,
                                       int W, int Cin, int Cout, int act, int ps_r, void* stream) {
    DASR_CHECK_PTR(xmax); DASR_CHECK_PTR(wmax);
    return sp_fwd(x, xmax, w_split, wmax, bias, residual, y, y_amax, B, H, W, Cin, Cout, act, ps_r, stream);
}
static int sp_dgrad(const float* dconv, const float* dmax, const unsigned short* w_split, const float* wmax, float* dx,
                    int accumulate, int B, int H, int W, int Cin, int Cout, void* stream) {
    DASR_CHECK_PTR(dconv); DASR_CHECK_PTR(w_split); DASR_CHECK_PTR(dx);
    DASR_CHECK_SHAPE(B > 0);
    if (!dasr_conv3x3_split_supported(H, W, Cin, Cout)) return DASR_E_UNSUPPORTED;
    const size_t mode1 = (size_t)9 * (dmax ? 2 : 3) * Cin * Cout;
    ConvSplitArgs a{dconv, (const bf16_t*)w_split + mode1, nullptr, nullptr, dx, B, H, W, Cout, Cin,
                    accumulate, DASR_ACT_NONE, 1, 0, 0, 0, 0, 0, 0, dmax, wmax, nullptr};
    return dmax ? sp_launch<2>(a, stream) : sp_launch<3>(a, stream);
}
extern "C" int dasr_conv3x3_dgrad_split(const float* dconv, const unsigned short* w_split, float* dx, int accumulate, int B,
                                        int H, int W, int Cin, int Cout, void* stream) {
    return sp_dgrad(dconv, nullptr, w_split, nullptr, dx, accumulate, B, H, W, Cin, Cout, stream);
}
extern "C" int dasr_conv3x3_dgrad_split2(const float* dconv, const float* dmax, const unsigned short* w_split, const float* wmax,
                                         float* dx, int accumulate, int B, int H, int W, int Cin, int Cout, void* stream) {
    DASR_CHECK_PTR(dmax); DASR_CHECK_PTR(wmax);
    return sp_dgrad(dconv, dmax, w_split, wmax, dx, accumulate, B, H, W, Cin, Cout, stream);
}

#define SW_TW 32
__host__ __device__ constexpr int sw_th(int MT, int NTW) { return MT * NTW == 4 ? 2 : (MT * NTW == 2 ? 4 : 8); }

struct SplitWgradArgs {
    const float* xmax;
    const float* dmax;
    const float* x;
    const float* dy;
    float* slabs;
    float* bslabs;
    int B, H, W, Cin, Cout;
    int P, ntiles;
};

__device__ __forceinline__ void sp_split_pair(float v0, float v1, bf16x2_t& h0, bf16x2_t& h1, bf16x2_t& h2) {
    h0 = dasr_f2bf2(v0, v1);
    const float r0 = v0 - dasr_bf2f(h0[0]), r1 = v1 - dasr_bf2f(h0[1]);
    h1 = dasr_f2bf2(r0, r1);
    h2 = dasr_f2bf2(r0 - dasr_bf2f(h1[0]), r1 - dasr_bf2f(h1[1]));
}

__device__ __forceinline__ void sp_split_pair2(float v0, float v1, float s, f16x2_t& h0, f16x2_t& h1) {
    v0 *= s; v1 *= s;
    h0[0] = (f16_t)v0; h0[1] = (f16_t)v1;
    h1[0] = (f16_t)(v0 - (float)h0[0]); h1[1] = (f16_t)(v1 - (float)h0[1]);
}

template <int MT, int NTW, int NP>
__global__ void __launch_bounds__(256, 2) k_conv3x3_wgrad_split(SplitWgradArgs a) {
    DASR_DYN_SMEM(smem);
    typedef SpFrag<NP> F;
    typedef typename F::elem E;
    constexpr int CIG = 32 * MT, COG = 32 * NTW, TH = sw_th(MT, NTW), HW = SW_TW + 2;
    constexpr int PAIRS = MT * NTW, G = 4 / PAIRS;
    float* sX = (float*)smem;
    float* sD = sX + (TH + 2) * HW * CIG;
    const int tid = threadIdx.x, lane = tid & 63, wv = DASR_UNIFORM((int)(tid >> 6));
    const int li = lane & 31, lh = lane >> 5;
    const int pair = wv % PAIRS, grp = wv / PAIRS;
    const int mt = pair / NTW, nt = pair % NTW;
    const int cgroups = a.Cout / COG;
    const int bgrp = blockIdx.x, bpar = blockIdx.y;
    const int ci0 = (bgrp / cgroups) * CIG, co0 = (bgrp % cgroups) * COG;
    const int tiles_x = (a.W + SW_TW - 1) / SW_TW, tiles_y = (a.H + TH - 1) / TH;

    f32x16 acc[9];
#pragma unroll
    for (int t = 0; t < 9; ++t)
#pragma unroll
        for (int r = 0; r < 16; ++r) acc[t][r] = 0.f;
    const bool do_bias = a.bslabs != nullptr && ci0 == 0 && tid < COG;
    float bsum = 0.f;
    float sx = 1.f, sd = 1.f, inv = 1.f;
    if (NP == 2) {
        __shared__ float s_red[32];
        sp_scales_gather<2>(a.xmax, a.dmax, s_red);
        __syncthreads();
        const int nw = (int)(blockDim.x >> 6);
        float mx = s_red[0], md = s_red[16];
        for (int w = 1; w < nw; ++w) { mx = fmaxf(mx, s_red[w]); md = fmaxf(md, s_red[16 + w]); }
        const int kx = sp_scale_exp(mx), kd = sp_scale_exp(md);
        sx = sp_pow2(kx); sd = sp_pow2(kd); inv = sp_pow2(-(kx + kd));
    }

    for (int tile = bpar; tile < a.ntiles; tile += a.P) {
        const int tx = tile % tiles_x, ty = (tile / tiles_x) % tiles_y, b = tile / (tiles_x * tiles_y);
        const int x0 = tx * SW_TW, y0 = ty * TH;
        constexpr int NX = (TH + 2) * HW * (CIG / 4), NXI = (NX + 255) / 256;
        constexpr int ND = TH * SW_TW * (COG / 4), NDI = (ND + 255) / 256;
        constexpr int XA = NDI >= 8 ? 1 : (8 - NDI < NXI ? 8 - NDI : NXI);
        float4 vx[NXI - XA > XA ? NXI - XA : XA], vd[NDI];
        auto ldx = [&](int u) {
            const int idx = tid + 256 * u;
            const int c4 = idx % (CIG / 4), pix = idx / (CIG / 4);
            const int gy = y0 + pix / HW - 1, gx = x0 + pix % HW - 1;
            float4 v = make_float4(0.f, 0.f, 0.f, 0.f);
            if (idx < NX && gy >= 0 && gy < a.H && gx >= 0 && gx < a.W)
                v = *(const float4*)(a.x + (((size_t)b * a.H + gy) * a.W + gx) * a.Cin + ci0 + 4 * c4);
            return v;
        };
        auto stx = [&](int u, float4 v) {
            const int idx = tid + 256 * u;
            if (idx < NX) *(float4*)(sX + (idx / (CIG / 4)) * CIG + 4 * (idx % (CIG / 4))) = v;
        };
#pragma unroll
        for (int u = 0; u < XA; ++u) vx[u] = ldx(u);
#pragma unroll
        for (int u = 0; u < NDI; ++u) {
            const int idx = tid + 256 * u;
            const int c4 = idx % (COG / 4), pix = idx / (COG / 4);
            const int gy = y0 + pix / SW_TW, gx = x0 + pix % SW_TW;
            float4 v = make_float4(0.f, 0.f, 0.f, 0.f);
            if (idx < ND && gy < a.H && gx < a.W)
                v = *(const float4*)(a.dy + (((size_t)b * a.H + gy) * a.W + gx) * a.Cout + co0 + 4 * c4);
            vd[u] = v;
        }
        __syncthreads();
#pragma unroll
        for (int u = 0; u < XA; ++u) stx(u, vx[u]);
#pragma unroll
        for (int u = 0; u < NDI; ++u) {
            const int idx = tid + 256 * u;
            if (idx < ND) *(float4*)(sD + (idx / (COG / 4)) * COG + 4 * (idx % (COG / 4))) = vd[u];
        }
#pragma unroll
        for (int u = XA; u < NXI; ++u) vx[u - XA] = ldx(u);
#pragma unroll
        for (int u = XA; u < NXI; ++u) stx(u, vx[u - XA]);
        __syncthreads();
        if (do_bias) {
#pragma unroll 8
            for (int px = 0; px < TH * SW_TW; ++px) bsum += sD[px * COG + tid];
        }
#pragma unroll 1
        for (int s = grp; s < TH * 2; s += G) {
            const int py = s >> 1, pc = 16 * (s & 1) + 8 * lh;
            typename F::type Bd[NP];
            {
                const float* dp = sD + (py * SW_TW + pc) * COG + 32 * nt + li;
#pragma unroll
                for (int e = 0; e < 8; e += 2) {
                    if constexpr (NP == 3) {
                        bf16x2_t h0, h1, h2;
                        sp_split_pair(dp[e * COG], dp[(e + 1) * COG], h0, h1, h2);
                        Bd[0][e] = h0[0]; Bd[0][e + 1] = h0[1];
                        Bd[1][e] = h1[0]; Bd[1][e + 1] = h1[1];
                        Bd[2][e] = h2[0]; Bd[2][e + 1] = h2[1];
                    } else {
                        f16x2_t h0, h1;
                        sp_split_pair2(dp[e * COG], dp[(e + 1) * COG], sd, h0, h1);
                        Bd[0][e] = h0[0]; Bd[0][e + 1] = h0[1];
                        Bd[1][e] = h1[0]; Bd[1][e + 1] = h1[1];
// ... 358 lines not shown
```

### depth-aware-endoscopy-sr_amd/csrc/dasr_common.h

```cpp
#pragma once

#ifdef DASR_HIPEMU
#include "hipemu.h"
#define DASR_LAUNCH(kernel, grid, block, shmem, stream, ...) \
    hipemu::launch((grid), (block), (shmem), [&]() { kernel(__VA_ARGS__); })
#define DASR_DYN_SMEM(name) char* name = hipemu::dyn_smem
#define DASR_DEVICE_BUILD 0
#define DASR_UNIFORM(x) (x)
#define DASR_MUL24(a, b) ((a) * (b))
#define DASR_SCHED_BARRIER() ((void)0)
#define DASR_WAVE_SYNC() hipemu::wave_barrier()
typedef char* dasr_lds_addr_t;
#define DASR_LDS_ADDR(p) ((char*)(p))
#define DASR_GLDS16(gsrc, lds_base) memcpy((lds_base) + 16 * hipemu::lane_id(), (const void*)(gsrc), 16)
#define DASR_WAIT_VM(n) ((void)0)
#define DASR_RAW_BARRIER() hipemu::block_barrier()
#define DASR_LDS_BARRIER() hipemu::block_barrier()
#define DASR_SETPRIO(n) ((void)0)
#define DASR_SCHED_GROUP(mask, n) ((void)0)
#define DASR_DEVICE_CONST static const
#else
#include <hip/hip_runtime.h>
#define DASR_LAUNCH(kernel, grid, block, shmem, stream, ...) \
    hipLaunchKernelGGL(kernel, (grid), (block), (shmem), (hipStream_t)(stream), __VA_ARGS__)
#define DASR_DYN_SMEM(name) extern __shared__ __attribute__((aligned(16))) char name[]
#define DASR_DEVICE_BUILD 1
#define DASR_UNIFORM(x) __builtin_amdgcn_readfirstlane(x)
#define DASR_MUL24(a, b) __mul24((a), (b))
#define DASR_SCHED_BARRIER() __builtin_amdgcn_sched_barrier(0)
#define DASR_WAVE_SYNC() do { __builtin_amdgcn_fence(__ATOMIC_RELEASE, "wavefront"); __builtin_amdgcn_wave_barrier(); __builtin_amdgcn_fence(__ATOMIC_ACQUIRE, "wavefront"); } while (0)
typedef float f32x4 __attribute__((ext_vector_type(4)));
typedef float f32x16 __attribute__((ext_vector_type(16)));
typedef unsigned dasr_lds_addr_t;
#define DASR_LDS_ADDR(p) ((unsigned)(size_t)(__attribute__((address_space(3))) char*)(p))
__device__ __forceinline__ void dasr_glds16(const void* gsrc, unsigned lds_base_uniform) {
    unsigned keep;
    asm volatile("s_mov_b32 %0, m0\n\ts_mov_b32 m0, %2\n\ts_nop 0\n\tglobal_load_lds_dwordx4 %1, off\n\ts_mov_b32 m0, %0"
                 : "=&s"(keep) : "v"(gsrc), "s"(lds_base_uniform) : "memory");
}
#define DASR_GLDS16(gsrc, lds_base) dasr_glds16((const void*)(gsrc), __builtin_amdgcn_readfirstlane(lds_base))
#define DASR_WAIT_VM(n) asm volatile("s_waitcnt vmcnt(" #n ")" ::: "memory")
#define DASR_RAW_BARRIER() do { asm volatile("" ::: "memory"); __builtin_amdgcn_s_barrier(); asm volatile("" ::: "memory"); } while (0)
#define DASR_LDS_BARRIER() do { asm volatile("s_waitcnt lgkmcnt(0)" ::: "memory"); __builtin_amdgcn_s_barrier(); asm volatile("" ::: "memory"); } while (0)
#define DASR_SETPRIO(n) __builtin_amdgcn_s_setprio(n)
#define DASR_SCHED_GROUP(mask, n) __builtin_amdgcn_sched_group_barrier((mask), (n), 0)
#define DASR_DEVICE_CONST __device__ const
#endif

#include "../../include/dasr.h"

#define DASR_CHECK_PTR(p) \
    do {                  \
        if (!(p)) return DASR_E_NULL; \
    } while (0)
#define DASR_CHECK_SHAPE(cond) \
    do {                       \
        if (!(cond)) return DASR_E_SHAPE; \
    } while (0)
#define DASR_RETURN_LAUNCH_STATUS() return (int)hipGetLastError()

static inline unsigned dasr_cdiv(size_t a, size_t b) { return (unsigned)((a + b - 1) / b); }
static inline unsigned dasr_ew_grid(size_t n, unsigned block = 256) {
    size_t g = (n + block - 1) / block;
    if (g > 256 * 8) g = 256 * 8;
    if (g < 1) g = 1;
    return (unsigned)g;
}

__device__ __forceinline__ float dasr_amax1(float m, float v) { return fmaxf(m, fabsf(v)); }
__device__ __forceinline__ float dasr_amax4(float m, float4 o) {
    return fmaxf(fmaxf(m, fmaxf(fabsf(o.x), fabsf(o.y))), fmaxf(fabsf(o.z), fabsf(o.w)));
}
__device__ __forceinline__ void dasr_amax_commit(float* amax, float m, float* s_part, unsigned wg, unsigned nwg) {
#pragma unroll
    for (int o = 32; o > 0; o >>= 1) m = fmaxf(m, __shfl_xor(m, o));
    __syncthreads();
    if ((threadIdx.x & 63) == 0) s_part[threadIdx.x >> 6] = m;
    __syncthreads();
    if (threadIdx.x == 0) {
        const int nw = (int)((blockDim.x * blockDim.y * blockDim.z + 63) >> 6);
        float r = s_part[0];
        for (int w = 1; w < nw; ++w) r = fmaxf(r, s_part[w]);
        amax[1 + wg] = r;
        if (wg == 0) {
            const int n = (int)nwg;
            memcpy(amax, &n, 4);
        }
    }
}
__device__ __forceinline__ void dasr_amax_commit_idle(float* amax, unsigned wg, unsigned nwg) {
    if (threadIdx.x == 0) {
        amax[1 + wg] = 0.f;
        if (wg == 0) {
            const int n = (int)nwg;
            memcpy(amax, &n, 4);
        }
    }
}
__device__ __forceinline__ unsigned dasr_flat_wg() { return blockIdx.x + gridDim.x * (blockIdx.y + gridDim.y * blockIdx.z); }
__device__ __forceinline__ unsigned dasr_flat_nwg() { return gridDim.x * gridDim.y * gridDim.z; }

__device__ __forceinline__ float dasr_act(float v, int act) {
    if (act == DASR_ACT_RELU) return v > 0.f ? v : 0.f;
    if (act == DASR_ACT_LRELU02) return v > 0.f ? v : 0.2f * v;
    return v;
}
__device__ __forceinline__ float dasr_act_grad_from_out(float out, int act) {
    if (act == DASR_ACT_RELU) return out > 0.f ? 1.f : 0.f;
    if (act == DASR_ACT_LRELU02) return out > 0.f ? 1.f : 0.2f;
    return 1.f;
}

__device__ __forceinline__ float dasr_double_in_scale(float var, float eps) {
    float r1 = 1.0f / sqrtf(var + eps);
    float v2 = var / (var + eps);
    return r1 / sqrtf(v2 + eps);
}
__device__ __forceinline__ float dasr_double_in_dscale(float var, float eps) {
    float a = var + eps;
    float v2 = var / a;
    float b = v2 + eps;
    float s = (1.0f / sqrtf(a)) / sqrtf(b);
    return s * (-0.5f / a - 0.5f * (eps / (a * a)) / b);
}
```

### depth-aware-endoscopy-sr_amd/graph.py

```python
import math

import torch

from . import ops
from .tape import Tape, Var, accum


FUSE_DGRAD_ACT = False

SIDE_STREAM = True
import os as _os
import threading as _threading
TAIL_WGRAD_SIDE = False
FUSE_INSTNORM_STATS = False
ENCODER_S2D = True
SPLIT_BF16 = True
SPLIT_WGRAD = True
SPLIT_PIECES = 2
FUSE_AMAX = True
SPLIT_CONV9 = True
SPLIT_MIN_PIXELS = 1 << 14
WGRAD_STREAM = False
_SIDE = {}
_SIDE_LOCK = _threading.Lock()


def _side_stream(device, which="branch"):
    key = (str(device), which)
    with _SIDE_LOCK:
        if key not in _SIDE:
            _SIDE[key] = torch.cuda.Stream(device=device, priority=-1)
        return _SIDE[key]


def _folded(tape, key, tensors, make):
    cache = tape.fold_cache
    if tape.enabled or cache is None or key is None:
        return make()
    ver = tuple((t.data_ptr(), ops.tensor_version(t)) for t in tensors)
    key = key + (str(tensors[0].device),)
    hit = cache.get(key)
    if hit is not None and hit[0] == ver:
        return hit[1]
    val = make()
    cache[key] = (ver, val)
    return val


PREPACK = True


class Prepack:

    def __init__(self):
        self.sig = None
        self.ready = False
        self.entries = {}
        self.tables = None
        self.misses = 0
        self.off = False
        self.lock = _threading.Lock()

    def __deepcopy__(self, memo):
        return Prepack()

    def __reduce__(self):
        return (Prepack, ())

    @staticmethod
    def signature(inp, act_dtype):
        return (tuple(inp.shape), str(inp.device), str(act_dtype), SPLIT_BF16, SPLIT_WGRAD, SPLIT_PIECES, SPLIT_CONV9,
                SPLIT_MIN_PIXELS, ENCODER_S2D)

    def begin(self, P, sig):
        if self.ready and sig == self.sig and all(P[n].data.data_ptr() == ptr and P[n].data.shape == shp
                                                  for n, ptr, shp in self.sources):
            ops.weight_pack_multi(self.tables[0])
            if self.tables[1] is not None:
                ops.conv3x3_split2_weights_multi(self.tables[1])
            self.misses = 0
            return
        if self.ready:
            self.misses += 1
            self.off = self.off or self.misses >= 3
        self.sig, self.ready, self.entries, self.tables = sig, False, {}, None

    def get(self, key):
        return self.entries.get(key) if self.ready else None

    def note(self, key, jobs, w, inv=None):
        if not self.ready and not self.off and key is not None:
            self.entries[key] = {"jobs": jobs, "w": w, "inv": inv, "split": None}

    def note_split(self, key, split):
        if not self.ready and key in self.entries:
            self.entries[key]["split"] = split

    def finish(self):
        if self.ready or not self.entries:
            return
        pj, sj, keep, sources = [], [], [], []
        npk = nsl = 0
        for e in self.entries.values():
            w, am = e["w"], None
            if e["split"] is not None:
                am = ops.amax_buffer(w)
                if isinstance(e["split"][0], str):
                    e["split"] = (e["split"][0], am)
                else:
                    ws = e["split"][0]
                    job, n = ops.split_job(w, am, ws, nsl)
                    sj.append(job)
                    nsl += n
                    e["split"] = (ws, am)
            for v, g, transposed, o_off, plain in e["jobs"]:
                job, n = ops.pack_job(v.data, g.data if g is not None else None, w, e["inv"], am, transposed, o_off, plain, npk)
                pj.append(job)
                npk += n
                for t in (v, g):
                    if t is not None:
                        sources.append((t.name, t.data.data_ptr(), t.data.shape))
            keep.append((w, e["inv"], am, e["split"]))
            e["jobs"] = None
        dev = keep[0][0].device
        self.tables = (ops.JobTable(pj, dev, keep), ops.JobTable(sj, dev, keep) if sj else None)
        self.sources = sources
        self.ready = True


def pack(tape, v, g=None, transposed=False, dtype=torch.float32):
    srcs = [v.data] + ([g.data] if g is not None else [])
    key = ("pack", v.name, str(dtype)) if v.name else None
    pp = tape.prepack if (key is not None and (g is None or g.name)) else None
    hit = pp.get(key) if pp is not None else None
    if hit is not None:
        w, inv = hit["w"], hit["inv"]
    else:
        w, inv = _folded(tape, key, srcs,
                         lambda: ops.weight_pack(v.data, g.data if g is not None else None, transposed, dtype=dtype))
        if pp is not None:
            pp.note(key, [(v, g, transposed, 0, False)], w, inv)
    out = Var(w, v.requires_grad or (g is not None and g.requires_grad))
    if pp is not None:
        out.pack = key
        out.split = hit["split"] if hit is not None else None

    def bwd():
        if out.grad is None:
            return
        if out.grad_event is not None:
            torch.cuda.current_stream().wait_event(out.grad_event)
            out.grad.record_stream(torch.cuda.current_stream())
        dv, dg = ops.weight_pack_bwd(out.grad, v.data, g.data if g is not None else None, inv, transposed)
        out.grad = None
        accum(v, dv)
        if g is not None:
            accum(g, dg)

    tape.record(bwd)
    return out


def pack_pair(tape, va, vb, dtype=torch.float32):
    Oa, I, KH, KW = va.data.shape
    Ob = vb.data.shape[0]

    def make():
        w = ops.empty((2, KH, KW, I, Oa + Ob), va.data, dtype)
        ops.weight_pack(va.data, None, False, out=w, o_off=0)
        ops.weight_pack(vb.data, None, False, out=w, o_off=Oa)
        return w

    key = ("pair", va.name, str(dtype)) if va.name else None
    pp = tape.prepack if (key is not None and vb.name) else None
    hit = pp.get(key) if pp is not None else None
    if hit is not None:
        w = hit["w"]
    else:
        w = _folded(tape, key, [va.data, vb.data], make)
        if pp is not None:
            pp.note(key, [(va, None, False, 0, False), (vb, None, False, Oa, False)], w)
    out = Var(w, va.requires_grad or vb.requires_grad)
    if pp is not None:
        out.pack = key
        out.split = hit["split"] if hit is not None else None

    def bwd():
        if out.grad is None:
            return
        if out.grad_event is not None:
            torch.cuda.current_stream().wait_event(out.grad_event)
            out.grad.record_stream(torch.cuda.current_stream())
        da, _ = ops.weight_pack_bwd(out.grad, va.data, None, None, False, o_off=0)
        db, _ = ops.weight_pack_bwd(out.grad, vb.data, None, None, False, o_off=Oa)
        out.grad = None
        accum(va, da)
        accum(vb, db)

    tape.record(bwd)
    return out


def bias_pair(tape, ba, bb):
    na, nb = ba.data.numel(), bb.data.numel()

    def make():
        buf = ops.empty((na + nb,), ba.data)
        ops.copy_(buf[:na], ba.data)
        ops.copy_(buf[na:], bb.data)
        return buf

    key = ("bias", ba.name) if ba.name else None
    pp = tape.prepack if (key is not None and bb.name and ba.data.dtype == torch.float32) else None
    hit = pp.get(key) if pp is not None else None
    if hit is not None:
        buf = hit["w"]
    else:
        buf = _folded(tape, key, [ba.data, bb.data], make)
        if pp is not None:
            pp.note(key, [(ba, None, False, 0, True), (bb, None, False, na, True)], buf)
    out = Var(buf, ba.requires_grad or bb.requires_grad)

    def bwd():
        if out.grad is None:
            return
        if out.grad_event is not None:
            torch.cuda.current_stream().wait_event(out.grad_event)
            out.grad.record_stream(torch.cuda.current_stream())
        g = out.grad
        out.grad = None
        accum(ba, g[:na])
        accum(bb, g[na:])

    tape.record(bwd)
    return out


def _is_c9(w):
    return isinstance(w.split, tuple) and isinstance(w.split[0], str)


def _amax(var):
    a = ops.get_amax(var.data)
    if a is not None:
        return a
    key = torch.cuda.current_stream().cuda_stream if var.data.is_cuda else 0
    if var.amax is None or var.amax[0] != key:
        var.amax = (key, ops.absmax(var.data))
    return var.amax[1]


def _amax_t(t):
    a = ops.get_amax(t)
    return a if a is not None else ops.absmax(t)


def want_amax(tape, like, shape=None):
    if not (SPLIT_BF16 and SPLIT_PIECES == 2 and FUSE_AMAX) or like.dtype != torch.float32 or tape.act_dtype != torch.float32:
        return None
    shape = tuple(like.shape) if shape is None else shape
    if len(shape) != 4 or shape[0] * shape[1] * shape[2] < SPLIT_MIN_PIXELS:
        return None
    return ops.amax_buffer(like)


def conv(tape, x, w, bias=None, *, stride=1, pad=1, transposed=False, act=ops.ACT_NONE, ps_r=1, residual=None,
         side_wgrad=False, want_stats=False, out_dtype=None):
    stats = None
    f32 = x.data.dtype == torch.float32 and out_dtype in (None, torch.float32)
    if (want_stats and FUSE_INSTNORM_STATS and f32 and act == ops.ACT_NONE and ps_r == 1 and residual is None and
            stride == 1 and pad == 1 and not transposed and tuple(w.data.shape[1:3]) == (3, 3)):
        y, mean, var = ops.conv2d_fwd_stats(x.data, w.data, bias.data if bias is not None else None)
        stats = (mean, var)
    elif (SPLIT_BF16 and f32 and w.data.dtype == torch.float32 and stride == 1 and pad == 1 and not transposed
          and tuple(w.data.shape[1:3]) == (3, 3)
          and (ps_r == 1 or (ps_r == 2 and residual is None and w.data.shape[4] % 128 == 0))
          and x.data.shape[0] * x.data.shape[1] * x.data.shape[2] >= SPLIT_MIN_PIXELS
          and ops.conv3x3_split_supported(x.data.shape[1], x.data.shape[2], w.data.shape[3], w.data.shape[4])):
        if w.split is None:
            w.split = _folded(tape, ("split%d" % SPLIT_PIECES, "@%x" % w.data.data_ptr()), [w.data],
                              (lambda: ops.conv3x3_split2_weights(w.data)) if SPLIT_PIECES == 2 else
                              (lambda: ops.conv3x3_split_weights(w.data)))
            if w.pack is not None and isinstance(w.split, tuple):
                tape.prepack.note_split(w.pack, w.split)
        if isinstance(w.split, tuple):
            y = ops.conv3x3_fwd_split2(x.data, _amax(x), w.split, bias.data if bias is not None else None, w.data.shape[4],
                                       residual.data if residual is not None else None, act, ps_r,
                                       amax=want_amax(tape, x.data))
        else:
            y = ops.conv3x3_fwd_split(x.data, w.split, bias.data if bias is not None else None, w.data.shape[4],
                                      residual.data if residual is not None else None, act, ps_r)
    elif (SPLIT_BF16 and SPLIT_PIECES == 2 and SPLIT_CONV9 and f32 and w.data.dtype == torch.float32 and stride == 1 and pad == 4
          and not transposed and tuple(w.data.shape[1:3]) == (9, 9) and act == ops.ACT_NONE and ps_r == 1 and residual is None
          and x.data.shape[0] * x.data.shape[1] * x.data.shape[2] >= SPLIT_MIN_PIXELS
          and ops.conv9_split_supported(x.data.shape[1], x.data.shape[2], w.data.shape[3], w.data.shape[4])):
        if w.split is None:
            w.split = ("c9", _folded(tape, ("c9max", "@%x" % w.data.data_ptr()), [w.data], lambda: ops.absmax(w.data[0])))
            if w.pack is not None:
                tape.prepack.note_split(w.pack, w.split)
        y = ops.conv9_fwd_split2(x.data, _amax(x), w.data, w.split[1], bias.data if bias is not None else None)
    else:
        am = want_amax(tape, x.data) if (f32 and x.data.shape[3] in (1, 3) and ps_r == 1) else None
        y = ops.conv2d_fwd(x.data, w.data, bias.data if bias is not None else None,
                           residual.data if residual is not None else None, stride, pad, transposed, act, ps_r, out_dtype,
                           amax=am)
    needs = x.requires_grad or w.requires_grad or (bias is not None and bias.requires_grad) or \
        (residual is not None and residual.requires_grad)
    out = Var(y, needs)
    out.stats = stats
    x.uses += 1
    if residual is not None:
        residual.uses += 1
    if (act != ops.ACT_NONE or ps_r > 1) and residual is None:
        out.epilogue = (act, ps_r)
    KH, KW, Cin, Cout = w.data.shape[1:]
    wshape = (KH, KW, Cin, Cout)
    B, H, W_, _ = x.data.shape
    Ho, Wo = ops.conv_out_hw(H, W_, KH, KW, stride, pad, transposed)

    def bwd():
        if out.grad is None:
            return
        dy = out.grad
        out.grad = None
        if out.grad_event is not None:
            torch.cuda.current_stream().wait_event(out.grad_event)
            dy.record_stream(torch.cuda.current_stream())
        if not x.requires_grad and residual is None and ps_r == 1 and act != ops.ACT_NONE:
            dw, db = ops.conv2d_wgrad_act(x.data, dy, y, wshape, act, stride, pad, transposed,
                                          want_bias=bias is not None)
            accum(w, dw)
            if bias is not None:
                accum(bias, db)
            return
        if out.grad_is_preact:
            dconv = dy
        elif act != ops.ACT_NONE or ps_r > 1:
            dconv = ops.conv2d_epilogue_bwd(dy, y, Ho, Wo, Cout, act, ps_r,
                                            amax=want_amax(tape, dy, (B, Ho, Wo, Cout)) if isinstance(w.split, tuple) else None)
        else:
            dconv = dy
        dmax = None
        if w.requires_grad or (bias is not None and bias.requires_grad):
            ws = _side_stream(dconv.device, "wgrad") if (WGRAD_STREAM and dconv.is_cuda) else None
            if ws is None and side_wgrad and TAIL_WGRAD_SIDE and SIDE_STREAM and dconv.is_cuda:
                ws = _side_stream(dconv.device)
            if ws is None and _is_c9(w):
                dmax = _amax_t(dconv)
                dw, db = ops.conv9_wgrad_split2(x.data, _amax(x), dconv, dmax, want_bias=bias is not None)
            elif ws is None and w.split is not None and SPLIT_WGRAD:
                if isinstance(w.split, tuple):
                    dmax = _amax_t(dconv)
                    dw, db = ops.conv3x3_wgrad_split2(x.data, _amax(x), dconv, dmax, want_bias=bias is not None)
                else:
                    dw, db = ops.conv3x3_wgrad_split(x.data, dconv, want_bias=bias is not None)
            elif ws is None:
                dw, db = ops.conv2d_wgrad(x.data, dconv, wshape, stride, pad, transposed, want_bias=bias is not None)
            else:
                cur = torch.cuda.current_stream()
                ready = cur.record_event()
                if ws not in tape.side_streams:
                    tape.side_streams.append(ws)
                with torch.cuda.stream(ws):
                    ws.wait_event(ready)
                    dconv.record_stream(ws)
                    dw, db = ops.conv2d_wgrad(x.data, dconv, wshape, stride, pad, transposed,
                                              want_bias=bias is not None)
                    done = ws.record_event()
                w.grad_event = done
                if bias is not None:
                    bias.grad_event = done
            accum(w, dw)
            if bias is not None:
                accum(bias, db)
        if x.requires_grad:
            if (FUSE_DGRAD_ACT and f32 and x.grad is None and x.uses == 1 and x.epilogue is not None and
                    ops.conv2d_dgrad_act_supported(x.data.shape, w.data, dconv.shape, stride, pad, transposed,
                                                   x.epilogue[1])):
                x.grad = ops.conv2d_dgrad_act(dconv, w.data, x.data, x.epilogue[0], x.epilogue[1], stride, pad,
                                              transposed)
                x.grad_is_preact = True
            elif _is_c9(w):
                if dmax is None:
                    dmax = _amax_t(dconv)
                x.grad = ops.conv9_dgrad_split2(dconv, dmax, w.data, w.split[1], x.data.shape, out=x.grad)
            elif isinstance(w.split, tuple):
                if dmax is None:
                    dmax = _amax_t(dconv)
                x.grad = ops.conv3x3_dgrad_split2(dconv, dmax, w.split, x.data.shape, out=x.grad)
            elif w.split is not None:
                if x.grad is None:
                    x.grad = ops.conv3x3_dgrad_split(dconv, w.split, x.data.shape)
                else:
                    ops.conv3x3_dgrad_split(dconv, w.split, x.data.shape, out=x.grad)
            elif x.grad is None:
                x.grad = ops.conv2d_dgrad(dconv, w.data, x.data.shape, stride, pad, transposed, out_dtype=x.data.dtype)
            else:
                ops.conv2d_dgrad(dconv, w.data, x.data.shape, stride, pad, transposed, out=x.grad)
        if residual is not None:
            accum(residual, dconv)

    tape.record(bwd)
    return out


def to_bf16(tape, x):
    x.uses += 1
    out = Var(ops.cast_to_bf16(x.data), x.requires_grad)

    def bwd():
        if out.grad is None:
            return
        g = out.grad
        out.grad = None
        if x.requires_grad:
            if x.grad is None:
                x.grad = ops.cast_to_f32(g)
            else:
                ops.accumulate_(x.grad, g)

    tape.record(bwd)
    return out


def to_f32(tape, x):
    x.uses += 1
    out = Var(ops.cast_to_f32(x.data), x.requires_grad)

    def bwd():
        if out.grad is None:
            return
        g = out.grad
        out.grad = None
        if x.requires_grad:
            accum(x, ops.cast_to_bf16(g))

    tape.record(bwd)
    return out


def space_to_depth2(tape, x, valid_hw=None):
    x.uses += 1
    out = Var(ops.space_to_depth2(x.data, valid_hw), x.requires_grad)

    def bwd():
        if out.grad is None:
            return
        g = out.grad
        out.grad = None
        if x.requires_grad:
            if x.grad is None:
                x.grad = ops.depth_to_space2_bwd(g, x.data.shape, x.data.dtype, valid_hw=valid_hw)
            else:
                ops.depth_to_space2_bwd(g, x.data.shape, x.data.dtype, out=x.grad, valid_hw=valid_hw)

    tape.record(bwd)
    return out


def expand_s2(tape, wp):
    _, _, _, Cin, Cout = wp.data.shape
    out = Var(_folded(tape, ("s2", "@%x" % wp.data.data_ptr()), [wp.data], lambda: ops.weight_expand_s2(wp.data)), wp.requires_grad)

    def bwd():
        if out.grad is None:
            return
        if out.grad_event is not None:
            torch.cuda.current_stream().wait_event(out.grad_event)
            out.grad.record_stream(torch.cuda.current_stream())
        g = out.grad
        out.grad = None
        accum(wp, ops.weight_collapse_s2(g, Cin, Cout))

    tape.record(bwd)
    return out


def expand_t2(tape, wp, bias):
    _, _, _, Cin, Cout = wp.data.shape
    w4, b4 = _folded(tape, ("t2", "@%x" % wp.data.data_ptr()), [wp.data] + ([bias.data] if bias is not None else []),
                     lambda: ops.weight_expand_t2(wp.data, bias.data if bias is not None else None))
    wout = Var(w4, wp.requires_grad)
    bout = Var(b4, bias.requires_grad) if bias is not None else None

    def bwd():
        if wout.grad is None:
            return
        for v in (wout, bout):
            if v is not None and v.grad_event is not None:
                torch.cuda.current_stream().wait_event(v.grad_event)
                if v.grad is not None:
                    v.grad.record_stream(torch.cuda.current_stream())
# ... 350 lines not shown
```

### depth-aware-endoscopy-sr_amd/ops.py

```python
import ctypes

import torch

from . import _lib

ACT_NONE, ACT_RELU, ACT_LRELU = 0, 1, 2
IN_EPS = 1e-5


BF16 = torch.bfloat16


def _p(t, allow_none=False):
    return _lib.ptr(t, allow_none)


def _pa(t, allow_none=False):
    if t is None:
        return _lib.ptr(t, allow_none)
    return _lib.ptr(t, allow_none, dtype=t.dtype if t.dtype in (torch.float32, BF16) else torch.float32)


def _is_bf(*ts):
    kinds = {t.dtype for t in ts if t is not None}
    if len(kinds) > 1:
        raise TypeError("dasr_amd: mixed activation dtypes %s" % sorted(str(k) for k in kinds))
    return kinds == {BF16}


def _call(name, *args):
    fn = getattr(_lib.get(), name)
    _lib.check(fn(*args, _lib.stream()), name)


def empty(shape, like, dtype=torch.float32):
    return torch.empty(shape, dtype=dtype, device=like.device)


def nchw_to_nhwc(x):
    B, C, H, W = x.shape
    out = empty((B, H, W, C), x)
    _call("dasr_nchw_to_nhwc", _p(x), _p(out), B, C, H, W)
    return out


def nhwc_to_nchw(x):
    B, H, W, C = x.shape
    out = empty((B, C, H, W), x)
    _call("dasr_nhwc_to_nchw", _p(x), _p(out), B, C, H, W)
    return out


def clamp_to_nchw(y, lo, hi):
    B, H, W, C = y.shape
    out = empty((B, C, H, W), y)
    _call("dasr_clamp_to_nchw", _p(y), _p(out), B, C, H, W, float(lo), float(hi))
    return out


def clamp_to_nchw_bwd(dout, y, lo, hi):
    B, H, W, C = y.shape
    dy = empty(y.shape, y)
    _call("dasr_clamp_to_nchw_bwd", _p(dout), _p(y), _p(dy), B, C, H, W, float(lo), float(hi))
    return dy


def resize_nearest_nchw(x, H, W):
    B, C, h, w = x.shape
    if (h, w) == (H, W):
        return x
    out = empty((B, C, H, W), x)
    _call("dasr_resize_nearest_nchw", _p(x), _p(out), B * C, h, w, H, W)
    return out


def resize_nearest_u8(region, H, W):
    B, h, w = region.shape
    if (h, w) == (H, W):
        return region
    out = torch.empty((B, H, W), dtype=torch.uint8, device=region.device)
    _call("dasr_resize_nearest_u8", _lib.ptr(region, dtype=torch.uint8), _lib.ptr(out, dtype=torch.uint8), B, h, w, H, W)
    return out


AMAX_FLOATS = 4097


def amax_buffer(like):
    return torch.empty((AMAX_FLOATS,), dtype=torch.float32, device=like.device)


def amax_value(buf):
    h = buf.detach().cpu()
    n = int(h[:1].view(torch.int32).item())
    assert 1 <= n < AMAX_FLOATS, n
    return float(h[1:1 + n].max().item())


def set_amax(t, amax):
    if amax is not None:
        t._dasr_amax = amax
    return t


def get_amax(t):
    return getattr(t, "_dasr_amax", None)


def drop_amax(t):
    if t is not None and getattr(t, "_dasr_amax", None) is not None:
        t._dasr_amax = None


def add(a, b):
    out = torch.empty_like(a)
    if _is_bf(a, b):
        _call("dasr_add_bf16", _pa(a), _pa(b), _pa(out), a.numel())
    else:
        _call("dasr_add", _p(a), _p(b), _p(out), a.numel())
    return out


def accumulate_(dst, src):
    assert dst.shape == src.shape
    drop_amax(dst)
    if dst.dtype == torch.float32 and src.dtype == BF16:
        _call("dasr_cast_bf16_to_f32", _pa(src), _p(dst), 1, dst.numel())
    elif _is_bf(dst, src):
        _call("dasr_accumulate_bf16", _pa(dst), _pa(src), dst.numel())
    else:
        _call("dasr_accumulate", _p(dst), _p(src), dst.numel())
    return dst


def copy_(dst, src):
    assert dst.numel() == src.numel() and dst.dtype == src.dtype
    drop_amax(dst)
    if dst.dtype == BF16:
        assert dst.numel() % 2 == 0
        _call("dasr_copy", _pa(dst), _pa(src), dst.numel() // 2)
    else:
        _call("dasr_copy", _p(dst), _p(src), dst.numel())
    return dst


def cast_to_bf16(x):
    out = torch.empty(x.shape, dtype=BF16, device=x.device)
    _call("dasr_cast_f32_to_bf16", _p(x), _pa(out), x.numel())
    return out


def cast_to_f32(x):
    out = torch.empty(x.shape, dtype=torch.float32, device=x.device)
    _call("dasr_cast_bf16_to_f32", _pa(x), _p(out), 0, x.numel())
    return out


def set_conv_bf16_impl(impl):
    _call("dasr_set_conv_bf16_impl", int(impl))


def conv_bf16_v2_launches():
    return int(_lib.get().dasr_conv_bf16_v2_launches())


def tensor_version(t):
    try:
        return t._version
    except RuntimeError:
        return -1


def space_to_depth2(x, valid_hw=None):
    B, H, W, C = x.shape
    Hv, Wv = valid_hw if valid_hw is not None else (H, W)
    out = torch.empty((B, (H + 1) // 2, (W + 1) // 2, 4 * C), dtype=BF16, device=x.device)
    _call("dasr_space_to_depth2_bf16", _pa(x), 1 if x.dtype == BF16 else 0, _pa(out), B, H, W, C, Hv, Wv)
    return out


def depth_to_space2_bwd(dy, x_shape, dtype, out=None, valid_hw=None):
    B, H, W, C = x_shape
    Hv, Wv = valid_hw if valid_hw is not None else (H, W)
    acc = out is not None
    if out is None:
        out = torch.empty(tuple(x_shape), dtype=dtype, device=dy.device)
    drop_amax(out)
    _call("dasr_depth_to_space2_bwd_bf16", _pa(dy), _pa(out), 1 if out.dtype == BF16 else 0, 1 if acc else 0, B, H, W, C,
          Hv, Wv)
    return out


def weight_expand_s2(w_packed):
    _, KH, KW, Cin, Cout = w_packed.shape
    assert (KH, KW) == (3, 3)
    out = torch.empty((2, 3, 3, 4 * Cin, Cout), dtype=BF16, device=w_packed.device)
    _call("dasr_weight_expand_s2_bf16", _p(w_packed), _pa(out), Cin, Cout)
    return out


def weight_collapse_s2(dw_expanded, Cin, Cout):
    out = torch.empty((3, 3, Cin, Cout), dtype=torch.float32, device=dw_expanded.device)
    _call("dasr_weight_collapse_s2", _p(dw_expanded), _p(out), Cin, Cout)
    return out


def weight_expand_t2(w_packed, bias):
    _, KH, KW, Cin, Cout = w_packed.shape
    assert (KH, KW) == (3, 3)
    out = torch.empty((2, 3, 3, Cin, 4 * Cout), dtype=BF16, device=w_packed.device)
    b4 = torch.empty((4 * Cout,), dtype=torch.float32, device=w_packed.device) if bias is not None else None
    _call("dasr_weight_expand_t2_bf16", _p(w_packed), _p(bias, True), _pa(out), _p(b4, True), Cin, Cout)
    return out, b4


def weight_collapse_t2(dw_expanded, db_expanded, Cin, Cout):
    dw = torch.empty((3, 3, Cin, Cout), dtype=torch.float32, device=dw_expanded.device)
    db = torch.empty((Cout,), dtype=torch.float32, device=dw_expanded.device) if db_expanded is not None else None
    _call("dasr_weight_collapse_t2", _p(dw_expanded), _p(db_expanded, True), _p(dw), _p(db, True), Cin, Cout)
    return dw, db


def zeros(shape, like):
    return torch.zeros(shape, dtype=torch.float32, device=like.device)


def weight_pack(v, g, transposed=False, out=None, o_off=0, dtype=torch.float32):
    if transposed:
        I, O, KH, KW = v.shape
    else:
        O, I, KH, KW = v.shape
    if out is None:
        out = empty((2, KH, KW, I, O), v, dtype)
    ldo = out.shape[4]
    inv = empty((I if transposed else O,), v) if g is not None else None
    if out.dtype == BF16:
        _call("dasr_weight_pack_fwd_bf16", _p(v), _p(g, True), _pa(out), _p(inv, True), O, I, KH, KW, int(transposed), ldo,
              int(o_off))
    else:
        _call("dasr_weight_pack_fwd", _p(v), _p(g, True), _p(out), _p(inv, True), O, I, KH, KW, int(transposed), ldo,
              int(o_off))
    return out, inv


class PackJob(ctypes.Structure):
    _fields_ = [("v", ctypes.c_void_p), ("g", ctypes.c_void_p), ("w", ctypes.c_void_p), ("inv_norm", ctypes.c_void_p),
                ("amax", ctypes.c_void_p)] + [(n, ctypes.c_int) for n in
                                              ("O", "I", "KK", "transposed", "ldo", "o_off", "bf16", "plain", "wg_begin", "reserved")]


class SplitJob(ctypes.Structure):
    _fields_ = [("w_packed", ctypes.c_void_p), ("wmax", ctypes.c_void_p), ("w_split", ctypes.c_void_p)] + \
               [(n, ctypes.c_int) for n in ("Cin", "Cout", "wg_begin", "reserved")]


class JobTable:

    def __init__(self, jobs, device, keep):
        self.n = len(jobs)
        self.host = (type(jobs[0]) * self.n)(*jobs)
        self.dev = torch.frombuffer(bytearray(bytes(self.host)), dtype=torch.uint8).to(device)
        self.keep = keep


def pack_job(v, g, w, inv, amax, transposed, o_off, plain, wg_begin):
    if plain:
        O, I, KK, ldo = v.numel(), 1, 1, w.numel()
    else:
        if transposed:
            I, O, KH, KW = v.shape
        else:
            O, I, KH, KW = v.shape
        KK, ldo = KH * KW, w.shape[4]
    bf = w.dtype == BF16
    return PackJob(_p(v), _p(g, True), _lib.ptr(w, False, w.dtype), _p(inv, True), _p(amax, True), O, I, KK, int(transposed), ldo,
                   int(o_off), int(bf), int(plain), int(wg_begin), 0), (I if transposed else O)


def weight_pack_multi(table):
    _call("dasr_weight_pack_multi", ctypes.addressof(table.host), table.dev.data_ptr(), table.n)


def split_job(w, wmax, ws, wg_begin):
    KH, KW, Cin, Cout = _wdims(w)
    assert (KH, KW) == (3, 3) and w.dtype == torch.float32
    return (SplitJob(_p(w), _p(wmax), _lib.ptr(ws, False, torch.float16), Cin, Cout, int(wg_begin), 0),
            int(_lib.get().dasr_conv3x3_split2_weights_slabs(Cin, Cout)))


def conv3x3_split2_weights_multi(table):
    _call("dasr_conv3x3_split2_weights_multi", ctypes.addressof(table.host), table.dev.data_ptr(), table.n)


def weight_pack_bwd(dw, v, g, inv, transposed=False, o_off=0):
    if transposed:
        I, O, KH, KW = v.shape
    else:
        O, I, KH, KW = v.shape
    dv = torch.empty_like(v)
    dg = torch.empty_like(g) if g is not None else None
    assert dw.dim() == 4, "weight gradients are plain HWIO"
    _call("dasr_weight_pack_bwd", _p(dw), _p(v), _p(g, True), _p(inv, True), _p(dv), _p(dg, True), O, I, KH, KW,
          int(transposed), dw.shape[3], int(o_off))
    return dv, dg


def conv_out_hw(H, W, KH, KW, stride, pad, transposed):
    if transposed:
        return (H - 1) * stride - 2 * pad + KH, (W - 1) * stride - 2 * pad + KW
    return (H + 2 * pad - KH) // stride + 1, (W + 2 * pad - KW) // stride + 1


def pack_hwio(w4):
    KH, KW, I, O = w4.shape
    out = torch.empty((2, KH, KW, I, O), dtype=w4.dtype, device=w4.device)
    out[0].copy_(w4)
    out[1].view(KH, KW, O, I).copy_(w4.permute(0, 1, 3, 2))
    return out


def _wdims(w):
    if w.dim() != 5 or w.shape[0] != 2:
        raise ValueError("dasr_amd: convolution kernels must be packed (ops.weight_pack / ops.pack_hwio)")
    return tuple(w.shape[1:])


def conv2d_fwd(x, w, bias=None, residual=None, stride=1, pad=1, transposed=False, act=ACT_NONE, ps_r=1, out_dtype=None,
               amax=None):
    B, H, W, Cin = x.shape
    KH, KW, wi, Cout = _wdims(w)
    assert wi == Cin, (w.shape, x.shape)
    Ho, Wo = conv_out_hw(H, W, KH, KW, stride, pad, transposed)
    bf = x.dtype == BF16 or out_dtype == BF16
    ydt = torch.float32
    if bf and not (KH == 9 and Cout <= 3):
        ydt = BF16
    if ps_r > 1:
        y = empty((B, Ho * ps_r, Wo * ps_r, Cout // (ps_r * ps_r)), x, ydt)
    else:
        y = empty((B, Ho, Wo, Cout), x, ydt)
    if bf:
        _call("dasr_conv2d_fwd_bf16", _pa(x), _pa(w), _p(bias, True), _pa(residual, True), _pa(y), B, H, W, Cin, Ho, Wo,
              Cout, KH, KW, stride, pad, int(transposed), act, ps_r)
    else:
        _call("dasr_conv2d_fwd", _p(x), _p(w), _p(bias, True), _p(residual, True), _p(y), _p(amax, True), B, H, W, Cin, Ho, Wo,
              Cout, KH, KW, stride, pad, int(transposed), act, ps_r)
        set_amax(y, amax)
    return y


def conv2d_epilogue_bwd(dy, y, Ho, Wo, Cout, act, ps_r, amax=None):
    B = y.shape[0]
    dconv = empty((B, Ho, Wo, Cout), y, y.dtype)
    if _is_bf(dy, y):
        _call("dasr_conv2d_epilogue_bwd_bf16", _pa(dy), _pa(y), _pa(dconv), B, Ho, Wo, Cout, act, ps_r)
    else:
        _call("dasr_conv2d_epilogue_bwd", _p(dy), _p(y), _p(dconv), _p(amax, True), B, Ho, Wo, Cout, act, ps_r)
        set_amax(dconv, amax)
    return dconv


def conv2d_dgrad(dconv, w, x_shape, stride=1, pad=1, transposed=False, out=None, out_dtype=torch.float32):
    B, H, W, Cin = x_shape
    KH, KW, _, Cout = _wdims(w)
    _, Ho, Wo, _ = dconv.shape
    acc = out is not None
    if out is None:
        out = torch.empty(x_shape, dtype=out_dtype, device=dconv.device)
    drop_amax(out)
    if out.dtype == BF16:
        _call("dasr_conv2d_dgrad_bf16", _pa(dconv), _pa(w), _pa(out), int(acc), B, H, W, Cin, Ho, Wo, Cout, KH, KW, stride,
              pad, int(transposed))
    else:
        _call("dasr_conv2d_dgrad", _p(dconv), _p(w), _p(out), int(acc), B, H, W, Cin, Ho, Wo, Cout, KH, KW, stride, pad,
              int(transposed))
    return out


def conv2d_dgrad_act_supported(x_shape, w, dconv_shape, stride, pad, transposed, ps_r):
    B, H, W, Cin = x_shape
    KH, KW, _, Cout = _wdims(w)
    _, Ho, Wo, _ = dconv_shape
    return bool(_lib.get().dasr_conv2d_dgrad_act_supported(B, H, W, Cin, Ho, Wo, Cout, KH, KW, stride, pad,
                                                          int(transposed), ps_r))


def conv2d_dgrad_act(dconv, w, x_act, act, ps_r, stride=1, pad=1, transposed=False):
    B, H, W, Cin = x_act.shape
    KH, KW, _, Cout = _wdims(w)
    _, Ho, Wo, _ = dconv.shape
    out = torch.empty((B, H // ps_r, W // ps_r, Cin * ps_r * ps_r), dtype=torch.float32, device=dconv.device)
    _call("dasr_conv2d_dgrad_act", _p(dconv), _p(w), _p(x_act), _p(out), B, H, W, Cin, Ho, Wo, Cout, KH, KW, stride, pad,
          int(transposed), act, ps_r)
    return out


def conv2d_wgrad(x, dconv, w_shape, stride=1, pad=1, transposed=False, want_bias=True):
    B, H, W, Cin = x.shape
    KH, KW, _, Cout = w_shape
    _, Ho, Wo, _ = dconv.shape
    lib = _lib.get()
    bf = x.dtype == BF16
    wsfn = lib.dasr_conv2d_wgrad_workspace_bf16 if bf else lib.dasr_conv2d_wgrad_workspace
    nbytes = wsfn(B, H, W, Cin, Ho, Wo, Cout, KH, KW, stride, pad, int(transposed))
    ws = torch.empty((max(1, (nbytes + 3) // 4),), dtype=torch.float32, device=x.device)
    dw = empty(w_shape, x)
    db = empty((Cout,), x) if want_bias else None
    if bf:
        _call("dasr_conv2d_wgrad_bf16", _pa(x), _pa(dconv), _p(dw), _p(db, True), _p(ws), nbytes, B, H, W, Cin, Ho, Wo,
              Cout, KH, KW, stride, pad, int(transposed))
    else:
        _call("dasr_conv2d_wgrad", _p(x), _p(dconv), _p(dw), _p(db, True), _p(ws), nbytes, B, H, W, Cin, Ho, Wo, Cout, KH,
              KW, stride, pad, int(transposed))
    return dw, db


def conv2d_wgrad_act(x, dy, y, w_shape, act, stride=1, pad=1, transposed=False, want_bias=True):
    B, H, W, Cin = x.shape
    KH, KW, _, Cout = w_shape
    _, Ho, Wo, _ = y.shape
    lib = _lib.get()
    if _is_bf(dy, y):
        dw = empty(w_shape, x)
        db = empty((Cout,), x) if want_bias else None
        _call("dasr_conv2d_wgrad_act_bf16", _p(x), _pa(dy), _pa(y), _p(dw), _p(db, True), B, H, W, Cin, Ho, Wo, Cout, KH, KW,
              stride, pad, int(transposed), act)
        return dw, db
    nbytes = lib.dasr_conv2d_wgrad_workspace(B, H, W, Cin, Ho, Wo, Cout, KH, KW, stride, pad, int(transposed))
    ws = torch.empty((max(1, (nbytes + 3) // 4),), dtype=torch.float32, device=x.device)
    fused = bool(lib.dasr_conv2d_wgrad_act_fused(B, H, W, Cin, Ho, Wo, Cout, KH, KW, stride, pad, int(transposed)))
    scratch = None if fused else torch.empty_like(y)
    dw = empty(w_shape, x)
    db = empty((Cout,), x) if want_bias else None
    _call("dasr_conv2d_wgrad_act", _p(x), _p(dy), _p(y), _p(dw), _p(db, True), _p(scratch, True), _p(ws), nbytes, B, H,
          W, Cin, Ho, Wo, Cout, KH, KW, stride, pad, int(transposed), act)
    return dw, db


def conv3x3_split_supported(H, W, Cin, Cout):
    return bool(_lib.get().dasr_conv3x3_split_supported(H, W, Cin, Cout))


def conv3x3_split_weights(w):
    KH, KW, Cin, Cout = _wdims(w)
    assert (KH, KW) == (3, 3) and w.dtype == torch.float32
    n = int(_lib.get().dasr_conv3x3_split_weights_bytes(Cin, Cout)) // 2
    ws = torch.empty((n,), dtype=BF16, device=w.device)
    _call("dasr_conv3x3_split_weights", _p(w), _pa(ws), Cin, Cout)
    return ws


def conv3x3_fwd_split(x, ws, bias, Cout, residual=None, act=ACT_NONE, ps_r=1):
    B, H, W, Cin = x.shape
    if ps_r > 1:
        y = empty((B, H * ps_r, W * ps_r, Cout // (ps_r * ps_r)), x)
    else:
        y = empty((B, H, W, Cout), x)
    _call("dasr_conv3x3_fwd_split", _p(x), _pa(ws), _p(bias, True), _p(residual, True), _p(y), B, H, W, Cin, Cout, act, ps_r)
    return y


def conv3x3_wgrad_split(x, dconv, want_bias=True):
    B, H, W, Cin = x.shape
    Cout = dconv.shape[3]
    nbytes = int(_lib.get().dasr_conv3x3_wgrad_split_workspace(B, H, W, Cin, Cout))
    ws = torch.empty((max(1, (nbytes + 3) // 4),), dtype=torch.float32, device=x.device)
    dw = empty((3, 3, Cin, Cout), x)
    db = empty((Cout,), x) if want_bias else None
    _call("dasr_conv3x3_wgrad_split", _p(x), _p(dconv), _p(dw), _p(db, True), _p(ws), nbytes, B, H, W, Cin, Cout)
    return dw, db


def conv3x3_dgrad_split(dconv, ws, x_shape, out=None):
    B, H, W, Cin = x_shape
    Cout = dconv.shape[3]
    acc = out is not None
    if out is None:
        out = empty(tuple(x_shape), dconv)
    drop_amax(out)
    _call("dasr_conv3x3_dgrad_split", _p(dconv), _pa(ws), _p(out), 1 if acc else 0, B, H, W, Cin, Cout)
    return out


def absmax(x):
    assert x.dtype == torch.float32 and x.is_contiguous()
    out = amax_buffer(x)
    _call("dasr_absmax", _p(x), x.numel(), _p(out))
    return out


def conv3x3_split2_weights(w):
    KH, KW, Cin, Cout = _wdims(w)
    assert (KH, KW) == (3, 3) and w.dtype == torch.float32
    wmax = absmax(w[0])
    n = int(_lib.get().dasr_conv3x3_split2_weights_bytes(Cin, Cout)) // 2
    ws = torch.empty((n,), dtype=torch.float16, device=w.device)
    _call("dasr_conv3x3_split2_weights", _p(w), _p(wmax), _lib.ptr(ws, False, torch.float16), Cin, Cout)
    return ws, wmax


def conv3x3_fwd_split2(x, xmax, ws, bias, Cout, residual=None, act=ACT_NONE, ps_r=1, amax=None):
    B, H, W, Cin = x.shape
    if ps_r > 1:
        y = empty((B, H * ps_r, W * ps_r, Cout // (ps_r * ps_r)), x)
    else:
        y = empty((B, H, W, Cout), x)
    _call("dasr_conv3x3_fwd_split2", _p(x), _p(xmax), _lib.ptr(ws[0], False, torch.float16), _p(ws[1]), _p(bias, True),
          _p(residual, True), _p(y), _p(amax, True), B, H, W, Cin, Cout, act, ps_r)
    return set_amax(y, amax)


def conv3x3_wgrad_split2(x, xmax, dconv, dmax, want_bias=True):
    B, H, W, Cin = x.shape
    Cout = dconv.shape[3]
    nbytes = int(_lib.get().dasr_conv3x3_wgrad_split_workspace(B, H, W, Cin, Cout))
    ws = torch.empty((max(1, (nbytes + 3) // 4),), dtype=torch.float32, device=x.device)
    dw = empty((3, 3, Cin, Cout), x)
    db = empty((Cout,), x) if want_bias else None
    _call("dasr_conv3x3_wgrad_split2", _p(x), _p(xmax), _p(dconv), _p(dmax), _p(dw), _p(db, True), _p(ws), nbytes, B, H, W, Cin,
          Cout)
    return dw, db


def conv3x3_dgrad_split2(dconv, dmax, ws, x_shape, out=None):
    B, H, W, Cin = x_shape
    Cout = dconv.shape[3]
    acc = out is not None
    if out is None:
        out = empty(tuple(x_shape), dconv)
    drop_amax(out)
    _call("dasr_conv3x3_dgrad_split2", _p(dconv), _p(dmax), _lib.ptr(ws[0], False, torch.float16), _p(ws[1]), _p(out), 1 if acc else 0, B, H, W, Cin, Cout)
    return out


def conv9_split_supported(H, W, Cin, Cout):
    return bool(_lib.get().dasr_conv9_split_supported(H, W, Cin, Cout))


def conv9_fwd_split2(x, xmax, w, wmax, bias):
    B, H, W, Cin = x.shape
    Cout = w.shape[4]
    y = empty((B, H, W, Cout), x)
    _call("dasr_conv9_fwd_split2", _p(x), _p(xmax), _p(w), _p(wmax), _p(bias, True), _p(y), B, H, W, Cin, Cout)
    return y


def conv9_dgrad_split2(dconv, dmax, w, wmax, x_shape, out=None):
    B, H, W, Cin = x_shape
    Cout = dconv.shape[3]
    acc = out is not None
    if out is None:
        out = empty(tuple(x_shape), dconv)
    drop_amax(out)
    _call("dasr_conv9_dgrad_split2", _p(dconv), _p(dmax), _p(w), _p(wmax), _p(out), 1 if acc else 0, B, H, W, Cin, Cout)
    return out


def conv9_wgrad_split2(x, xmax, dconv, dmax, want_bias=True):
    B, H, W, Cin = x.shape
    Cout = dconv.shape[3]
    nbytes = int(_lib.get().dasr_conv9_wgrad_split2_workspace(B, H, W, Cin, Cout))
    ws = torch.empty((max(1, (nbytes + 3) // 4),), dtype=torch.float32, device=x.device)
    dw = empty((9, 9, Cin, Cout), x)
    db = empty((Cout,), x) if want_bias else None
    _call("dasr_conv9_wgrad_split2", _p(x), _p(xmax), _p(dconv), _p(dmax), _p(dw), _p(db, True), _p(ws), nbytes, B, H, W, Cin, Cout)
    return dw, db


def conv2d_fwd_stats(x, w, bias):
    B, H, W, Cin = x.shape
    KH, KW, Cin2, Cout = w.shape[1:]
    assert (KH, KW) == (3, 3) and Cin2 == Cin
    y = empty((B, H, W, Cout), x)
    mean = empty((B, Cout), x)
    var = empty((B, Cout), x)
    nbytes = int(_lib.get().dasr_conv2d_fwd_stats_workspace(B, H, W, Cin, Cout))
    ws = torch.empty((max(1, (nbytes + 3) // 4),), dtype=torch.float32, device=x.device)
    _call("dasr_conv2d_fwd_stats", _p(x), _p(w), _p(bias, True), _p(y), _p(mean), _p(var), _p(ws), nbytes, B, H, W, Cin,
          Cout)
    return y, mean, var


def instnorm_stats(x):
    B, H, W, C = x.shape
    mean = empty((B, C), x)
    var = empty((B, C), x)
    nbytes = _lib.get().dasr_instnorm_stats_workspace(B, H * W, C)
    ws = torch.empty((max(1, nbytes // 4),), dtype=torch.float32, device=x.device)
    if x.dtype == BF16:
        _call("dasr_instnorm_stats_bf16", _pa(x), _p(mean), _p(var), _p(ws), nbytes, B, H * W, C)
    else:
        _call("dasr_instnorm_stats", _p(x), _p(mean), _p(var), _p(ws), nbytes, B, H * W, C)
    return mean, var


def dynk_fwd(st, A_w, A_b, Wg, Wb):
    B, K, L = st.shape
    C = Wg.shape[0]
    stp = torch.empty_like(st)
    D = empty((B, 2, 9, K, C), st)
    _call("dasr_dynk_fwd", _p(st), _p(A_w), _p(A_b), _p(Wg), _p(Wb), _p(stp), _p(D), B, K, L, C)
    return stp, D


def dynk_bwd(dD, st, stp, A_w, Wg, Wb, dst_accum):
    B, K, L = st.shape
    C = Wg.shape[0]
    dWg, dWb = torch.empty_like(Wg), torch.empty_like(Wb)
    dA_w = torch.empty_like(A_w)
    dA_b = empty((K,), st)
    scratch = torch.empty_like(st)
    _call("dasr_dynk_bwd", _p(dD), _p(st), _p(stp), _p(A_w), _p(Wg), _p(Wb), _p(dWg), _p(dWb), _p(dA_w), _p(dA_b),
          _p(dst_accum), _p(scratch), B, K, L, C)
    return dWg, dWb, dA_w, dA_b


def soft_mask_max_regions():
    return int(_lib.get().dasr_sean_soft_mask_max_regions())


def mask_compress(mask):
    B, K, H, W = mask.shape
    region = torch.empty((B, H, W), dtype=torch.uint8, device=mask.device)
    flag = torch.empty((1,), dtype=torch.int32, device=mask.device)
    _call("dasr_mask_compress", _p(mask), _lib.ptr(region, dtype=torch.uint8), _lib.ptr(flag, dtype=torch.int32), B, K,
          H, W)
    return region, flag


def depth_to_masks(depth, num_masks=10, fixed_edges=None, want_planes=True):
    h, w = depth.shape[-2:]
    B = depth.numel() // (h * w)
    d = depth.contiguous()
    planes = torch.empty((B, num_masks, h, w), dtype=torch.float32, device=d.device) if want_planes else None
    region = torch.empty((B, h, w), dtype=torch.uint8, device=d.device)
    nbytes = int(_lib.get().dasr_depth_to_masks_workspace(B, h * w))
    ws = torch.empty((max(nbytes, 4) // 4,), dtype=torch.float32, device=d.device)
    _call("dasr_depth_to_masks", _p(d), _p(fixed_edges, True) if fixed_edges is not None else None,
          _p(planes) if planes is not None else None, _lib.ptr(region, dtype=torch.uint8), _p(ws), nbytes, B, h * w,
          num_masks)
    return planes, region


def _rf(region, flag):
    if region is None:
        return None, None
    return _lib.ptr(region, dtype=torch.uint8), (_lib.ptr(flag, dtype=torch.int32) if flag is not None else None)


def sean_fwd(t, mean, var, gb2, mask, region, flag, D, bias_g, bias_b, alpha_g, alpha_b, residual, relu, amax=None):
    B, H, W, C = t.shape
    K = mask.shape[1]
    assert mask.shape == (B, K, H, W) and gb2.shape == (B, H, W, 2 * C) and D.shape == (B, 2, 9, K, C)
    out = torch.empty_like(t)
    rp, fp = _rf(region, flag)
    if _is_bf(t, gb2, residual):
        _call("dasr_sean_fwd_bf16", _pa(t), _p(mean), _p(var), _pa(gb2), _p(mask), rp, fp, _p(D), _p(bias_g), _p(bias_b),
              _p(alpha_g), _p(alpha_b), _pa(residual, True), _pa(out), int(relu), B, H, W, C, K, IN_EPS)
    else:
# ... 68 lines not shown
```

### depth-aware-endoscopy-sr_amd/tape.py

```python
from . import ops


class Var:
    __slots__ = ("data", "grad", "requires_grad", "name", "uses", "epilogue", "grad_is_preact", "event",
                 "grad_event", "stats", "split", "amax", "pack")

    def __init__(self, data, requires_grad=False, name=None):
        self.data = data
        self.grad = None
        self.requires_grad = requires_grad
        self.name = name
        self.uses = 0
        self.epilogue = None
        self.grad_is_preact = False
        self.event = None
        self.grad_event = None
        self.stats = None
        self.split = None
        self.amax = None
        self.pack = None

    @property
    def shape(self):
        return self.data.shape


class Tape:

    def __init__(self, enabled=True, act_dtype=None):
        import torch
        self.enabled = enabled
        self.act_dtype = act_dtype if act_dtype is not None else torch.float32
        self.nodes = []
        self._stream = None
        self.side_streams = []
        self.fold_cache = None
        self.prepack = None
        self.marks = []
        self.on_mark = None

    def record(self, fn):
        if self.enabled:
            self.nodes.append((fn, self._stream))

    def mark(self):
        if self.enabled:
            self.marks.append(len(self.nodes))

    def on_stream(self, stream):
        tape = self

        class _Ctx:
            def __enter__(self_inner):
                import torch
                self_inner.prev = tape._stream
                tape._stream = stream
                if stream not in tape.side_streams:
                    tape.side_streams.append(stream)
                self_inner.guard = torch.cuda.stream(stream)
                self_inner.guard.__enter__()

            def __exit__(self_inner, *exc):
                self_inner.guard.__exit__(*exc)
                tape._stream = self_inner.prev

        return _Ctx()

    def backward(self):
        import torch
        while self.nodes:
            fn, stream = self.nodes.pop()
            if stream is None:
                fn()
            else:
                with torch.cuda.stream(stream):
                    fn()
            while self.marks and len(self.nodes) <= self.marks[-1]:
                self.marks.pop()
                if self.on_mark is not None:
                    self.on_mark()
        for s in self.side_streams:
            torch.cuda.current_stream().wait_stream(s)


def accum(var, g, owned=True):
    if var is None or not var.requires_grad or g is None:
        return
    if var.grad is None:
        if owned:
            var.grad = g
        else:
            var.grad = ops.copy_(ops.empty(g.shape, g, g.dtype), g)
    else:
        ops.accumulate_(var.grad, g)
```

### include/dasr.h

```cpp
#ifndef DASR_H
#define DASR_H

#include <stddef.h>
#include <stdint.h>

#ifdef __cplusplus
extern "C" {
#endif

#define DASR_OK 0
#define DASR_E_NULL (-1)
#define DASR_E_SHAPE (-2)
#define DASR_E_UNSUPPORTED (-3)
#define DASR_E_WORKSPACE (-4)

#define DASR_ACT_NONE 0
#define DASR_ACT_RELU 1
#define DASR_ACT_LRELU02 2

int dasr_version(void);
const char* dasr_error_string(int code);
int dasr_is_device_build(void);

int dasr_nchw_to_nhwc(const float* src, float* dst, int B, int C, int H, int W, void* stream);
int dasr_nhwc_to_nchw(const float* src, float* dst, int B, int C, int H, int W, void* stream);
int dasr_clamp_to_nchw(const float* y_nhwc, float* out_nchw, int B, int C, int H, int W, float lo, float hi,
                       void* stream);
int dasr_clamp_to_nchw_bwd(const float* dout_nchw, const float* y_nhwc, float* dy_nhwc, int B, int C, int H, int W,
                           float lo, float hi, void* stream);
int dasr_resize_nearest_nchw(const float* src, float* dst, int BC, int h, int w, int H, int W, void* stream);
int dasr_resize_nearest_u8(const unsigned char* src, unsigned char* dst, int B, int h, int w, int H, int W,
                           void* stream);

int dasr_weight_pack_fwd(const float* v, const float* g, float* w_hwio, float* inv_norm, int O, int I, int KH, int KW,
                         int transposed, int ldo, int o_off, void* stream);
typedef struct dasr_pack_job {
    const float* v; const float* g; void* w; float* inv_norm; float* amax;
    int O, I, KK, transposed, ldo, o_off, bf16, plain, wg_begin, reserved;
} dasr_pack_job;
int dasr_weight_pack_multi(const dasr_pack_job* jobs_host, const dasr_pack_job* jobs_device, int njobs, void* stream);
int dasr_weight_pack_bwd(const float* dw_hwio, const float* v, const float* g, const float* inv_norm, float* dv,
                         float* dg, int O, int I, int KH, int KW, int transposed, int ldo, int o_off, void* stream);

int dasr_conv2d_fwd(const float* x, const float* w_hwio, const float* bias, const float* residual, float* y, float* y_amax,
                    int B, int H, int W, int Cin, int Ho, int Wo, int Cout, int KH, int KW, int stride, int pad,
                    int transposed, int act, int ps_r, void* stream);
size_t dasr_conv2d_fwd_stats_workspace(int B, int H, int W, int Cin, int Cout);
int dasr_conv2d_fwd_stats(const float* x, const float* w, const float* bias, float* y, float* mean, float* var,
                          void* workspace, size_t workspace_bytes, int B, int H, int W, int Cin, int Cout, void* stream);

int dasr_conv2d_epilogue_bwd(const float* dy, const float* y, float* dconv, float* dconv_amax, int B, int Ho, int Wo,
                             int Cout, int act, int ps_r, void* stream);
int dasr_conv2d_dgrad(const float* dconv, const float* w_hwio, float* dx, int accumulate, int B, int H, int W, int Cin,
                      int Ho, int Wo, int Cout, int KH, int KW, int stride, int pad, int transposed, void* stream);
int dasr_conv2d_dgrad_act_supported(int B, int H, int W, int Cin, int Ho, int Wo, int Cout, int KH, int KW, int stride,
                                    int pad, int transposed, int ps_r);
int dasr_conv2d_dgrad_act(const float* dconv, const float* w_hwio, const float* x_act, float* dprev, int B, int H, int W,
                          int Cin, int Ho, int Wo, int Cout, int KH, int KW, int stride, int pad, int transposed,
                          int act, int ps_r, void* stream);
size_t dasr_conv2d_wgrad_workspace(int B, int H, int W, int Cin, int Ho, int Wo, int Cout, int KH, int KW, int stride,
                                   int pad, int transposed);
int dasr_conv2d_wgrad(const float* x, const float* dconv, float* dw_hwio, float* dbias, void* workspace,
                      size_t workspace_bytes, int B, int H, int W, int Cin, int Ho, int Wo, int Cout, int KH, int KW,
                      int stride, int pad, int transposed, void* stream);

int dasr_conv2d_wgrad_act_fused(int B, int H, int W, int Cin, int Ho, int Wo, int Cout, int KH, int KW, int stride, int pad,
                                int transposed);
int dasr_conv2d_wgrad_act(const float* x, const float* dy, const float* y, float* dw_hwio, float* dbias,
                          float* dconv_scratch, void* workspace, size_t workspace_bytes, int B, int H, int W, int Cin,
                          int Ho, int Wo, int Cout, int KH, int KW, int stride, int pad, int transposed, int act,
                          void* stream);

int dasr_conv3x3_split_supported(int H, int W, int Cin, int Cout);
size_t dasr_conv3x3_split_weights_bytes(int Cin, int Cout);
int dasr_conv3x3_split_weights(const float* w_packed, unsigned short* w_split, int Cin, int Cout, void* stream);
int dasr_conv3x3_fwd_split(const float* x, const unsigned short* w_split, const float* bias, const float* residual, float* y,
                           int B, int H, int W, int Cin, int Cout, int act, int ps_r, void* stream);
int dasr_conv3x3_dgrad_split(const float* dconv, const unsigned short* w_split, float* dx, int accumulate, int B, int H,
                             int W, int Cin, int Cout, void* stream);
size_t dasr_conv3x3_wgrad_split_workspace(int B, int H, int W, int Cin, int Cout);
int dasr_conv3x3_wgrad_split(const float* x, const float* dconv, float* dw_hwio, float* dbias, void* workspace,
                             size_t workspace_bytes, int B, int H, int W, int Cin, int Cout, void* stream);

#define DASR_AMAX_MAX_PARTS 4096
#define DASR_AMAX_FLOATS (1 + DASR_AMAX_MAX_PARTS)
int dasr_absmax(const float* x, size_t n, float* amax, void* stream);
size_t dasr_conv3x3_split2_weights_bytes(int Cin, int Cout);
int dasr_conv3x3_split2_weights(const float* w_packed, const float* wmax, unsigned short* w_split, int Cin, int Cout,
                                void* stream);
typedef struct dasr_split_job {
    const float* w_packed; const float* wmax; unsigned short* w_split;
    int Cin, Cout, wg_begin, reserved;
} dasr_split_job;
int dasr_conv3x3_split2_weights_slabs(int Cin, int Cout);
int dasr_conv3x3_split2_weights_multi(const dasr_split_job* jobs_host, const dasr_split_job* jobs_device, int njobs, void* stream);
int dasr_conv3x3_fwd_split2(const float* x, const float* xmax, const unsigned short* w_split, const float* wmax,
                            const float* bias, const float* residual, float* y, float* y_amax, int B, int H, int W, int Cin,
                            int Cout, int act, int ps_r, void* stream);
int dasr_conv3x3_dgrad_split2(const float* dconv, const float* dmax, const unsigned short* w_split, const float* wmax,
                              float* dx, int accumulate, int B, int H, int W, int Cin, int Cout, void* stream);
int dasr_conv3x3_wgrad_split2(const float* x, const float* xmax, const float* dconv, const float* dmax, float* dw_hwio,
                              float* dbias, void* workspace, size_t workspace_bytes, int B, int H, int W, int Cin, int Cout,
                              void* stream);

int dasr_conv9_split_supported(int H, int W, int Cin, int Cout);
int dasr_conv9_fwd_split2(const float* x, const float* xmax, const float* w_hwio, const float* wmax, const float* bias, float* y,
                          int B, int H, int W, int Cin, int Cout, void* stream);
int dasr_conv9_dgrad_split2(const float* dconv, const float* dmax, const float* w_hwio, const float* wmax, float* dx,
                            int accumulate, int B, int H, int W, int Cin, int Cout, void* stream);
size_t dasr_conv9_wgrad_split2_workspace(int B, int H, int W, int Cin, int Cout);
int dasr_conv9_wgrad_split2(const float* x, const float* xmax, const float* dconv, const float* dmax, float* dw_hwio, float* dbias,
                            void* workspace, size_t workspace_bytes, int B, int H, int W, int Cin, int Cout, void* stream);

size_t dasr_instnorm_stats_workspace(int B, int HW, int C);
int dasr_instnorm_stats(const float* x, float* mean, float* var, void* workspace, size_t workspace_bytes, int B, int HW,
                        int C, void* stream);

int dasr_dynk_fwd(const float* st, const float* A_w, const float* A_b, const float* W_gamma, const float* W_beta,
                  float* stp, float* D, int B, int K, int L, int C, void* stream);
int dasr_dynk_bwd(const float* dD, const float* st, const float* stp, const float* A_w, const float* W_gamma,
                  const float* W_beta, float* dW_gamma, float* dW_beta, float* dA_w, float* dA_b, float* dst,
                  float* dstp, int B, int K, int L, int C, void* stream);

int dasr_mask_compress(const float* mask, unsigned char* region, int* onehot_flag, int B, int K, int H, int W,
                       void* stream);
int dasr_sean_fwd(const float* t, const float* mean, const float* var, const float* gb2, const float* mask,
                  const unsigned char* region, const int* onehot_flag, const float* D, const float* bias_gamma, const float* bias_beta, const float* alpha_gamma,
                  const float* alpha_beta, const float* residual, float* out, float* out_amax, int relu, int B, int H,
                  int W, int C, int K, float eps, void* stream);
size_t dasr_sean_bwd_workspace(int B, int H, int W, int C, int K);
int dasr_sean_bwd(const float* dout, const float* out, const float* t, const float* mean, const float* var,
                  const float* gb2, const float* mask, const unsigned char* region, const int* onehot_flag,
                  const float* D, const float* bias_gamma, const float* bias_beta,
                  const float* alpha_gamma, const float* alpha_beta, float* dt, float* dgb2, float* dD,
                  float* dbias_gamma, float* dbias_beta, float* dalpha_gamma, float* dalpha_beta, float* dres,
                  float* dt_amax, float* dgb2_amax, void* workspace, size_t workspace_bytes, int relu, int B, int H, int W,
                  int C, int K, float eps, void* stream);

int dasr_sean_soft_mask_max_regions(void);

int dasr_region_pool_fwd(const float* feat, const float* mask, float* maskr, float* area, float* out, int B, int K,
                         int L, int h, int w, int H, int W, void* stream);
int dasr_region_pool_bwd(const float* dout, const float* maskr, const float* area, float* dfeat, int B, int K, int L,
                         int h, int w, void* stream);

size_t dasr_depth_to_masks_workspace(int B, int HW);
int dasr_depth_to_masks(const float* depth, const float* fixed_edges, float* masks, unsigned char* region,
                        void* workspace, size_t workspace_bytes, int B, int HW, int K, void* stream);

int dasr_loss_sums(const float* sr, const float* hr, const unsigned char* region, float* sums, int B, int C, int h,
                   int w, int scale, int K, void* stream);
int dasr_loss_bwd(const float* sr, const float* hr, const unsigned char* region, const float* dsums, float* dsr, int B,
                  int C, int h, int w, int scale, int K, void* stream);

int dasr_add(const float* a, const float* b, float* out, size_t n, void* stream);
int dasr_accumulate(float* dst, const float* src, size_t n, void* stream);
int dasr_copy(float* dst, const float* src, size_t n, void* stream);


int dasr_weight_pack_fwd_bf16(const float* v, const float* g, unsigned short* w, float* inv_norm, int O, int I, int KH, int KW,
                              int transposed, int ldo, int o_off, void* stream);
int dasr_conv2d_fwd_bf16(const void* x, const void* w, const float* bias, const unsigned short* residual, void* y, int B,
                         int H, int W, int Cin, int Ho, int Wo, int Cout, int KH, int KW, int stride, int pad, int transposed,
                         int act, int ps_r, void* stream);
int dasr_conv2d_epilogue_bwd_bf16(const unsigned short* dy, const unsigned short* y, unsigned short* dconv, int B, int Ho,
                                  int Wo, int Cout, int act, int ps_r, void* stream);
int dasr_set_conv_bf16_impl(int impl);
int dasr_get_conv_bf16_impl(void);
int dasr_conv_bf16_v2_launches(void);
int dasr_conv2d_dgrad_bf16(const void* dconv, const void* w, unsigned short* dx, int accumulate, int B, int H, int W, int Cin,
                           int Ho, int Wo, int Cout, int KH, int KW, int stride, int pad, int transposed, void* stream);
size_t dasr_conv2d_wgrad_workspace_bf16(int B, int H, int W, int Cin, int Ho, int Wo, int Cout, int KH, int KW, int stride,
                                        int pad, int transposed);
int dasr_conv2d_wgrad_bf16(const unsigned short* x, const void* dconv, float* dw, float* dbias, void* workspace,
                           size_t workspace_bytes, int B, int H, int W, int Cin, int Ho, int Wo, int Cout, int KH, int KW,
                           int stride, int pad, int transposed, void* stream);
int dasr_conv2d_wgrad_act_bf16(const float* x, const unsigned short* dy, const unsigned short* y, float* dw, float* dbias,
                               int B, int H, int W, int Cin, int Ho, int Wo, int Cout, int KH, int KW, int stride, int pad,
                               int transposed, int act, void* stream);
int dasr_instnorm_stats_bf16(const unsigned short* x, float* mean, float* var, void* workspace, size_t workspace_bytes, int B,
                             int HW, int C, void* stream);
int dasr_sean_fwd_bf16(const unsigned short* t, const float* mean, const float* var, const unsigned short* gb2,
                       const float* mask, const unsigned char* region, const int* onehot_flag, const float* D,
                       const float* bias_gamma, const float* bias_beta, const float* alpha_gamma, const float* alpha_beta,
                       const unsigned short* residual, unsigned short* out, int relu, int B, int H, int W, int C, int K,
                       float eps, void* stream);
int dasr_sean_bwd_bf16(const unsigned short* dout, const unsigned short* out, const unsigned short* t, const float* mean,
                       const float* var, const unsigned short* gb2, const float* mask, const unsigned char* region,
                       const int* onehot_flag, const float* D, const float* bias_gamma, const float* bias_beta,
                       const float* alpha_gamma, const float* alpha_beta, unsigned short* dt, unsigned short* dgb2, float* dD,
                       float* dbias_gamma, float* dbias_beta, float* dalpha_gamma, float* dalpha_beta, unsigned short* dres,
                       void* workspace, size_t workspace_bytes, int relu, int B, int H, int W, int C, int K, float eps,
                       void* stream);
int dasr_add_bf16(const unsigned short* a, const unsigned short* b, unsigned short* out, size_t n, void* stream);
int dasr_accumulate_bf16(unsigned short* dst, const unsigned short* src, size_t n, void* stream);
int dasr_cast_f32_to_bf16(const float* src, unsigned short* dst, size_t n, void* stream);
int dasr_cast_bf16_to_f32(const unsigned short* src, float* dst, int accumulate, size_t n, void* stream);

int dasr_space_to_depth2_bf16(const void* x, int x_is_bf16, unsigned short* y, int B, int H, int W, int C, int Hv, int Wv,
                              void* stream);
int dasr_depth_to_space2_bwd_bf16(const unsigned short* dy, void* dx, int dx_is_bf16, int accumulate, int B, int H, int W,
                                  int C, int Hv, int Wv, void* stream);
int dasr_weight_expand_s2_bf16(const float* w_hwio, unsigned short* out, int Cin, int Cout, void* stream);
int dasr_weight_collapse_s2(const float* dw_expanded, float* dw_hwio, int Cin, int Cout, void* stream);
int dasr_weight_expand_t2_bf16(const float* w_hwio, const float* bias, unsigned short* out, float* bias_out, int Cin,
                               int Cout, void* stream);
int dasr_weight_collapse_t2(const float* dw_expanded, const float* dbias_expanded, float* dw_hwio, float* dbias, int Cin,
                            int Cout, void* stream);

size_t dasr_ssim_workspace(int B, int C, int H, int W);
int dasr_ssim(const float* img1, const float* img2, const float* window11, float* out_per_sample, void* workspace,
              size_t workspace_bytes, int B, int C, int H, int W, void* stream);

#ifdef __cplusplus
}
#endif
#endif
```

Before: 248.5 frames/s.

## Store activation sign bitmasks in forward and use them for backward gradient masking

Forward conv kernels with a LeakyReLU/ReLU epilogue now also write a packed one-bit-per-channel sign mask. The backward epilogue and the fused c1 wgrad read this mask instead of the full fp32 activation. The goal is to cut backward memory traffic for activation-gradient masking by about 32x in bytes read. The cost is an extra mask write in forward, a lane OR-reduction per pixel, and a padded pixel loop in the c1 kernel. Whether the mask path is actually wired into the model's default path is not fully visible.

Result: slower. 237.4 frames/s (-4.5%).

```diff
diff --git a/depth-aware-endoscopy-sr_amd/csrc/conv_api.hip b/depth-aware-endoscopy-sr_amd/csrc/conv_api.hip
--- a/depth-aware-endoscopy-sr_amd/csrc/conv_api.hip
+++ b/depth-aware-endoscopy-sr_amd/csrc/conv_api.hip
@@ -44,6 +44,22 @@
     return absmax_raise(y, (size_t)B * Ho * Wo * Cout, y_amax, stream);
 }
 
+extern "C" size_t dasr_sign_mask_words(int B, int H, int W, int C) {
+    if (B <= 0 || H <= 0 || W <= 0 || C <= 0 || (C % 32) != 0) return 0;
+    return (size_t)B * H * W * (C / 32);
+}
+extern "C" int dasr_conv2d_fwd_mask(const float* x, const float* w, const float* bias, float* y, float* y_amax, int* y_mask, int B,
+                                    int H, int W, int Cin, int Ho, int Wo, int Cout, int KH, int KW, int stride, int pad,
+                                    int transposed, int act, void* stream) {
+    DASR_CHECK_PTR(x); DASR_CHECK_PTR(w); DASR_CHECK_PTR(y); DASR_CHECK_PTR(y_mask);
+    ConvGeom g{B, H, W, Cin, Ho, Wo, Cout, KH, KW, stride, pad, transposed};
+    int rc = check_geom(g);
+    if (rc) return rc;
+    if (act < 0 || act > 2) return DASR_E_UNSUPPORTED;
+    if (conv_mfma_supported(g) || !conv_c1_supported(g) || (Cout % 32) != 0) return DASR_E_UNSUPPORTED;
+    return conv_c1_fwd(g, x, w, bias, y, act, stream, y_amax, (unsigned*)y_mask);
+}
+
 extern "C" size_t dasr_conv2d_fwd_stats_workspace(int B, int H, int W, int Cin, int Cout) {
     if (B <= 0 || H <= 0 || W <= 0 || Cin <= 0 || Cout <= 0) return 0;
     ConvGeom g{B, H, W, Cin, H, W, Cout, 3, 3, 1, 1, 0};
@@ -75,6 +91,17 @@
     if (ps_r > 1 && (Cout % (ps_r * ps_r)) != 0) return DASR_E_SHAPE;
     ConvGeom g{B, Ho, Wo, 1, Ho, Wo, Cout, 1, 1, 1, 0, 0};
     return conv_epilogue_bwd(g, dy, y, dconv, act, ps_r, stream, dconv_amax);
+}
+
+extern "C" int dasr_conv2d_epilogue_bwd_mask(const float* dy, const int* y_mask, float* dconv, float* dconv_amax, int B, int Ho,
+                                             int Wo, int Cout, int act, int ps_r, void* stream) {
+    DASR_CHECK_PTR(dy); DASR_CHECK_PTR(y_mask); DASR_CHECK_PTR(dconv);
+    DASR_CHECK_SHAPE(B > 0 && Ho > 0 && Wo > 0 && Cout > 0);
+    if (act < 0 || act > 2) return DASR_E_UNSUPPORTED;
+    if (ps_r < 1) ps_r = 1;
+    if (ps_r > 1 && (Cout % (ps_r * ps_r)) != 0) return DASR_E_SHAPE;
+    ConvGeom g{B, Ho, Wo, 1, Ho, Wo, Cout, 1, 1, 1, 0, 0};
+    return conv_epilogue_bwd_mask(g, dy, (const unsigned*)y_mask, dconv, act, ps_r, stream, dconv_amax);
 }
 
 extern "C" int dasr_conv2d_dgrad(const float* dconv, const float* w, float* dx, int accumulate, int B, int H, int W,
@@ -144,6 +171,18 @@
                              stride, pad, transposed, stream);
 }
 
+extern "C" int dasr_conv2d_wgrad_act_mask(const float* x, const float* dy, const int* y_mask, float* dw, float* dbias, int B, int H,
+                                          int W, int Cin, int Ho, int Wo, int Cout, int KH, int KW, int stride, int pad,
+                                          int transposed, int act, void* stream) {
+    DASR_CHECK_PTR(x); DASR_CHECK_PTR(dy); DASR_CHECK_PTR(y_mask); DASR_CHECK_PTR(dw);
+    ConvGeom g{B, H, W, Cin, Ho, Wo, Cout, KH, KW, stride, pad, transposed};
+    int rc = check_geom(g);
+    if (rc) return rc;
+    if (act < 0 || act > 2) return DASR_E_UNSUPPORTED;
+    if (!conv_c1_supported(g) || (Cout % 32) != 0) return DASR_E_UNSUPPORTED;
+    return conv_c1_wgrad_mask(g, x, dy, (const unsigned*)y_mask, act, dw, dbias, stream);
+}
+
 extern "C" int dasr_conv2d_wgrad_act_fused(int B, int H, int W, int Cin, int Ho, int Wo, int Cout, int KH, int KW,
                                            int stride, int pad, int transposed) {
     ConvGeom g{B, H, W, Cin, Ho, Wo, Cout, KH, KW, stride, pad, transposed};
diff --git a/depth-aware-endoscopy-sr_amd/csrc/conv_c1.hip b/depth-aware-endoscopy-sr_amd/csrc/conv_c1.hip
--- a/depth-aware-endoscopy-sr_amd/csrc/conv_c1.hip
+++ b/depth-aware-endoscopy-sr_amd/csrc/conv_c1.hip
@@ -27,7 +27,8 @@
 template <typename T, int CIN>
 __global__ void __launch_bounds__(256) k_conv3x3_c1_fwd(const float* __restrict__ x, const float* __restrict__ w,
                                                         const float* __restrict__ bias, T* __restrict__ y, int B,
-                                                        int H, int W, int Cout, int act, float* __restrict__ amax) {
+                                                        int H, int W, int Cout, int act, float* __restrict__ amax,
+                                                        unsigned* __restrict__ smask) {
     DASR_DYN_SMEM(smem);
     float* sRow = (float*)smem;
     const int nq = Cout / 4;
@@ -42,13 +43,18 @@
     const bool relu = act == DASR_ACT_RELU;
     auto neg = [&](float v) { return relu ? 0.f : slope * v; };
     float om = 0.f;
+    const bool wm = sizeof(T) == 4 && smask != nullptr;
+    const int wend = wm ? (W + npl - 1) / npl * npl : W;
+    const int mw = Cout / 32;
     for (int row = blockIdx.x; row < B * H; row += gridDim.x) {
         const int b = row / H, py = row - b * H;
         __syncthreads();
         c1_stage_rows<CIN>(x, sRow, b, py, H, W);
         __syncthreads();
         T* yrow = y + ((size_t)row * W) * Cout + 4 * q;
-        for (int px = pl; px < W; px += npl) {
+        for (int px0 = pl; px0 < wend; px0 += npl) {
+            const bool live = px0 < W;
+            const int px = live ? px0 : W - 1;
             float4 acc = bv;
 #pragma unroll
             for (int t = 0; t < NT; ++t) {
@@ -58,14 +64,18 @@
             }
             acc.x = acc.x > 0.f ? acc.x : neg(acc.x); acc.y = acc.y > 0.f ? acc.y : neg(acc.y);
             acc.z = acc.z > 0.f ? acc.z : neg(acc.z); acc.w = acc.w > 0.f ? acc.w : neg(acc.w);
-            st4(yrow + (size_t)px * Cout, acc);
+            if (live) st4(yrow + (size_t)px * Cout, acc);
             om = dasr_amax4(om, acc);
+            if (wm) {
+                const unsigned word = dasr_or_lanes8(dasr_sign4(acc.x, acc.y, acc.z, acc.w) << (4 * (q & 7)));
+                if (live && (q & 7) == 0) smask[((size_t)row * W + px) * mw + (q >> 3)] = word;
+            }
         }
     }
     if (amax) dasr_amax_commit(amax, om, sRow, dasr_flat_wg(), dasr_flat_nwg());
 }
 
-template <typename T, int CIN, bool HASY>
+template <typename T, int CIN, int YM>
 __global__ void __launch_bounds__(256) k_conv3x3_c1_wgrad(const float* __restrict__ x, const T* __restrict__ dy,
                                                           const T* __restrict__ yact, float* __restrict__ dw,
                                                           float* __restrict__ dbias, int B, int H, int W, int Cout,
@@ -84,6 +94,9 @@
     constexpr int NPX = sizeof(T) == 2 ? 8 : 4;
     typedef typename raw4<T>::type Raw;
     Raw gq[NPX], yq[NPX];
+    unsigned mq[NPX];
+    const unsigned* smask = (const unsigned*)yact;
+    const int mw = Cout / 32, msh = 4 * (q & 7);
     const int nrows = B * H, step = NPX * npl;
     auto issue = [&](int row, int base) {
         const size_t ro = ((size_t)row * W) * Cout + 4 * q;
@@ -91,7 +104,8 @@
         for (int u = 0; u < NPX; ++u) {
             const int px = base + pl + u * npl < W ? base + pl + u * npl : W - 1;
             gq[u] = ld4_raw(dy + ro + (size_t)px * Cout);
-            if (HASY) yq[u] = ld4_raw(yact + ro + (size_t)px * Cout);
+            if (YM == 1) yq[u] = ld4_raw(yact + ro + (size_t)px * Cout);
+            if (YM == 2) mq[u] = smask[((size_t)row * W + px) * mw + (q >> 3)];
         }
     };
     if ((int)blockIdx.x < nrows) issue(blockIdx.x, 0);
@@ -105,10 +119,15 @@
 #pragma unroll
             for (int u = 0; u < NPX; ++u) {
                 g[u] = cvt4<T>(gq[u]);
-                if (HASY) {
+                if (YM == 1) {
                     const float4 yv = cvt4<T>(yq[u]);
                     g[u].x *= yv.x > 0.f ? 1.f : slope; g[u].y *= yv.y > 0.f ? 1.f : slope;
                     g[u].z *= yv.z > 0.f ? 1.f : slope; g[u].w *= yv.w > 0.f ? 1.f : slope;
+                }
+                if (YM == 2) {
+                    const unsigned nib = mq[u] >> msh;
+                    g[u].x *= (nib & 1u) ? 1.f : slope; g[u].y *= (nib & 2u) ? 1.f : slope;
+                    g[u].z *= (nib & 4u) ? 1.f : slope; g[u].w *= (nib & 8u) ? 1.f : slope;
                 }
             }
             {
@@ -164,24 +183,26 @@
 }
 template <typename T>
 static int conv_c1_fwd_impl(const ConvGeom& g, const float* x, const float* w, const float* bias, T* y, int act, void* stream,
-                            float* amax = nullptr) {
+                            float* amax = nullptr, unsigned* smask = nullptr) {
+    if (smask && (sizeof(T) != 4 || (g.Cout % 32) != 0)) return DASR_E_UNSUPPORTED;
     unsigned grid = (unsigned)(g.B * g.H);
     if (grid > 256 * 8) grid = 256 * 8;
     const size_t lds = sizeof(float) * 3 * (g.W + 2) * g.Cin;
-    if (g.Cin == 3) DASR_LAUNCH((k_conv3x3_c1_fwd<T, 3>), dim3(grid), dim3(256), lds, stream, x, w, bias, y, g.B, g.H, g.W, g.Cout, act, amax);
-    else            DASR_LAUNCH((k_conv3x3_c1_fwd<T, 1>), dim3(grid), dim3(256), lds, stream, x, w, bias, y, g.B, g.H, g.W, g.Cout, act, amax);
+    if (g.Cin == 3) DASR_LAUNCH((k_conv3x3_c1_fwd<T, 3>), dim3(grid), dim3(256), lds, stream, x, w, bias, y, g.B, g.H, g.W, g.Cout, act, amax, smask);
+    else            DASR_LAUNCH((k_conv3x3_c1_fwd<T, 1>), dim3(grid), dim3(256), lds, stream, x, w, bias, y, g.B, g.H, g.W, g.Cout, act, amax, smask);
     DASR_RETURN_LAUNCH_STATUS();
 }
 int conv_c1_fwd(const ConvGeom& g, const float* x, const float* w, const float* bias, float* y, int act, void* stream,
-                float* amax) {
-    return conv_c1_fwd_impl<float>(g, x, w, bias, y, act, stream, amax);
+                float* amax, unsigned* smask) {
+    return conv_c1_fwd_impl<float>(g, x, w, bias, y, act, stream, amax, smask);
 }
 int conv_c1_fwd_bf16(const ConvGeom& g, const float* x, const float* w, const float* bias, bf16_t* y, int act, void* stream) {
     return conv_c1_fwd_impl<bf16_t>(g, x, w, bias, y, act, stream);
 }
 template <typename T>
 static int conv_c1_wgrad_impl(const ConvGeom& g, const float* x, const T* dy, const T* yact, int act, float* dw, float* dbias,
-                              void* stream) {
+                              void* stream, const unsigned* smask = nullptr) {
+    if (smask && (sizeof(T) != 4 || (g.Cout % 32) != 0)) return DASR_E_UNSUPPORTED;
     DASR_LAUNCH(k_c1_zero, dim3(dasr_cdiv((size_t)(9 * g.Cin + 1) * g.Cout, 256)), dim3(256), 0, stream, dw, 9 * g.Cin * g.Cout,
                 dbias, g.Cout);
     unsigned grid = (unsigned)(g.B * g.H);
@@ -194,11 +215,19 @@
     const unsigned cap = sizeof(T) == 2 ? C1_WGRAD_WGS_BF16 : C1_WGRAD_WGS_F32;
     if (grid > cap) grid = cap;
     const size_t lds = sizeof(float) * (256 * 4 + 3 * (g.W + 2) * g.Cin);
-#define C1_WGRAD(CIN, HASY) \
-    DASR_LAUNCH((k_conv3x3_c1_wgrad<T, CIN, HASY>), dim3(grid), dim3(256), lds, stream, x, dy, yact, dw, dbias, g.B, g.H, g.W, g.Cout, act)
-    const bool hasy = yact != nullptr && act != DASR_ACT_NONE;
-    if (g.Cin == 3) { if (hasy) C1_WGRAD(3, true); else C1_WGRAD(3, false); }
-    else            { if (hasy) C1_WGRAD(1, true); else C1_WGRAD(1, false); }
+#define C1_WGRAD(CIN, YM) \
+    DASR_LAUNCH((k_conv3x3_c1_wgrad<T, CIN, YM>), dim3(grid), dim3(256), lds, stream, x, dy, yp, dw, dbias, g.B, g.H, g.W, g.Cout, act)
+    const int ym = act == DASR_ACT_NONE ? 0 : (smask && sizeof(T) == 4) ? 2 : yact != nullptr ? 1 : 0;
+    const T* yp = yact;
+    if constexpr (sizeof(T) == 4) {
+        if (ym == 2) {
+            yp = (const T*)smask;
+            if (g.Cin == 3) C1_WGRAD(3, 2); else C1_WGRAD(1, 2);
+            DASR_RETURN_LAUNCH_STATUS();
+        }
+    }
+    if (g.Cin == 3) { if (ym == 1) C1_WGRAD(3, 1); else C1_WGRAD(3, 0); }
+    else            { if (ym == 1) C1_WGRAD(1, 1); else C1_WGRAD(1, 0); }
 #undef C1_WGRAD
     DASR_RETURN_LAUNCH_STATUS();
 }
@@ -206,6 +235,10 @@
                   void* stream) {
     return conv_c1_wgrad_impl<float>(g, x, dy, yact, act, dw, dbias, stream);
 }
+int conv_c1_wgrad_mask(const ConvGeom& g, const float* x, const float* dy, const unsigned* smask, int act, float* dw,
+                       float* dbias, void* stream) {
+    return conv_c1_wgrad_impl<float>(g, x, dy, (const float*)nullptr, act, dw, dbias, stream, smask);
+}
 int conv_c1_wgrad_bf16(const ConvGeom& g, const float* x, const bf16_t* dy, const bf16_t* yact, int act, float* dw,
                        float* dbias, void* stream) {
     return conv_c1_wgrad_impl<bf16_t>(g, x, dy, yact, act, dw, dbias, stream);
diff --git a/depth-aware-endoscopy-sr_amd/csrc/conv_direct.hip b/depth-aware-endoscopy-sr_amd/csrc/conv_direct.hip
--- a/depth-aware-endoscopy-sr_amd/csrc/conv_direct.hip
+++ b/depth-aware-endoscopy-sr_amd/csrc/conv_direct.hip
@@ -192,7 +192,23 @@
     }
     if (amax) dasr_amax_commit(amax, om, s_part, dasr_flat_wg(), dasr_flat_nwg());
 }
-template <int R, typename T>
+__global__ void __launch_bounds__(256) k_conv_epilogue_bwd_flat4_mask(const float* __restrict__ dy, const unsigned* __restrict__ smask,
+                                                                      float* __restrict__ dconv, size_t n4, int act,
+                                                                      float* __restrict__ amax) {
+    __shared__ float s_part[16];
+    const float slope = dasr_act_neg_slope(act);
+    float om = 0.f;
+    for (size_t i = (size_t)blockIdx.x * blockDim.x + threadIdx.x; i < n4; i += (size_t)gridDim.x * blockDim.x) {
+        const float4 d = ld4(dy + 4 * i);
+        const unsigned nib = smask[i >> 3] >> (4 * ((unsigned)i & 7u));
+        const float4 o = make_float4(d.x * ((nib & 1u) ? 1.f : slope), d.y * ((nib & 2u) ? 1.f : slope),
+                                     d.z * ((nib & 4u) ? 1.f : slope), d.w * ((nib & 8u) ? 1.f : slope));
+        st4(dconv + 4 * i, o);
+        om = dasr_amax4(om, o);
+    }
+    if (amax) dasr_amax_commit(amax, om, s_part, dasr_flat_wg(), dasr_flat_nwg());
+}
+template <int R, typename T, bool MASK = false>
 __global__ void __launch_bounds__(256) k_conv_epilogue_bwd_ps(const T* __restrict__ dy, const T* __restrict__ y,
                                                               T* __restrict__ dconv, int Wo, int Cq, int act, int rows,
                                                               float* __restrict__ amax) {
@@ -202,6 +218,10 @@
     const int e = livee ? e0 : Wo * Cq - 1;
     const int ox = e / Cq, c = e - ox * Cq;
     const size_t srow = (size_t)Wo * R * Cq;
+    const unsigned* smask = (const unsigned*)y;
+    const int mw = Cq / 32;
+    const size_t mrow = (size_t)Wo * R * mw;
+    const float slope = dasr_act_neg_slope(act);
     float om = 0.f;
     for (size_t row0 = blockIdx.y; row0 < (size_t)rows; row0 += 2 * (size_t)gridDim.y) {
         const size_t row1 = row0 + gridDim.y;
@@ -211,13 +231,16 @@
 #pragma unroll
         for (int h = 0; h < 2; ++h) {
             const T* dyp = dy + rws[h] * R * srow + (size_t)ox * R * Cq + c;
-            const T* yp = y + rws[h] * R * srow + (size_t)ox * R * Cq + c;
+            const size_t yo = MASK ? rws[h] * R * mrow + (size_t)ox * R * mw + (c >> 5) : rws[h] * R * srow + (size_t)ox * R * Cq + c;
 #pragma unroll
             for (int i = 0; i < R; ++i)
 #pragma unroll
                 for (int j = 0; j < R; ++j) {
                     const size_t o = (size_t)i * srow + (size_t)j * Cq;
-                    out[h][i * R + j] = ld1(dyp + o) * dasr_act_grad_from_out(ld1(yp + o), act);
+                    if constexpr (MASK)
+                        out[h][i * R + j] = ld1(dyp + o) * (((smask[yo + (size_t)i * mrow + (size_t)j * mw] >> (c & 31)) & 1u) ? 1.f : slope);
+                    else
+                        out[h][i * R + j] = ld1(dyp + o) * dasr_act_grad_from_out(ld1(y + yo + o), act);
                 }
         }
 #pragma unroll
@@ -239,6 +262,15 @@
     if (amax) dasr_amax_commit(amax, om, s_part, dasr_flat_wg(), dasr_flat_nwg());
 }
 
+static bool conv_epilogue_bwd_ps_grid(const ConvGeom& g, int Cq, bool amax, dim3& grid) {
+    const size_t rows = (size_t)g.B * g.Ho;
+    const unsigned gx = dasr_cdiv((size_t)g.Wo * Cq, 256);
+    size_t gy = rows < 65535 ? rows : 65535;
+    if (amax && (size_t)gx * gy > DASR_AMAX_MAX_PARTS) gy = DASR_AMAX_MAX_PARTS / gx > 0 ? DASR_AMAX_MAX_PARTS / gx : 1;
+    if (amax && (size_t)gx * gy > DASR_AMAX_MAX_PARTS) return false;
+    grid = dim3(gx, (unsigned)gy);
+    return true;
+}
 template <typename T>
 static int conv_epilogue_bwd_impl(const ConvGeom& g, const T* dy, const T* y, T* dconv, int act, int ps_r, void* stream,
                                   float* amax = nullptr) {
@@ -249,11 +281,8 @@
     } else if ((ps_r == 2 || ps_r == 3) && (g.Cout % (ps_r * ps_r)) == 0 && rows < ((size_t)1 << 31) &&
                (size_t)g.Wo * (g.Cout / (ps_r * ps_r)) < (1u << 30)) {
         const int Cq = g.Cout / (ps_r * ps_r);
-        const unsigned gx = dasr_cdiv((size_t)g.Wo * Cq, 256);
-        size_t gy = rows < 65535 ? rows : 65535;
-        if (amax && (size_t)gx * gy > DASR_AMAX_MAX_PARTS) gy = DASR_AMAX_MAX_PARTS / gx > 0 ? DASR_AMAX_MAX_PARTS / gx : 1;
-        if (amax && (size_t)gx * gy > DASR_AMAX_MAX_PARTS) return DASR_E_UNSUPPORTED;
-        const dim3 grid(gx, (unsigned)gy);
+        dim3 grid;
+        if (!conv_epilogue_bwd_ps_grid(g, Cq, amax != nullptr, grid)) return DASR_E_UNSUPPORTED;
         if (ps_r == 2)
             DASR_LAUNCH((k_conv_epilogue_bwd_ps<2, T>), grid, dim3(256), 0, stream, dy, y, dconv, g.Wo, Cq, act, (int)rows, amax);
         else
@@ -266,6 +295,23 @@
 int conv_epilogue_bwd(const ConvGeom& g, const float* dy, const float* y, float* dconv, int act, int ps_r, void* stream,
                       float* amax) {
     return conv_epilogue_bwd_impl<float>(g, dy, y, dconv, act, ps_r, stream, amax);
+}
+int conv_epilogue_bwd_mask(const ConvGeom& g, const float* dy, const unsigned* smask, float* dconv, int act, int ps_r,
+                           void* stream, float* amax) {
+    const size_t n = (size_t)g.B * g.Ho * g.Wo * g.Cout;
+    const size_t rows = (size_t)g.B * g.Ho;
+    if (ps_r <= 1 && (g.Cout % 32) == 0) {
+        DASR_LAUNCH(k_conv_epilogue_bwd_flat4_mask, dim3(dasr_ew_grid(n / 4)), dim3(256), 0, stream, dy, smask, dconv, n / 4, act, amax);
+    } else if (ps_r == 2 && (g.Cout % 128) == 0 && rows < ((size_t)1 << 31) && (size_t)g.Wo * (g.Cout / 4) < (1u << 30)) {
+        const int Cq = g.Cout / 4;
+        dim3 grid;
+        if (!conv_epilogue_bwd_ps_grid(g, Cq, amax != nullptr, grid)) return DASR_E_UNSUPPORTED;
+        DASR_LAUNCH((k_conv_epilogue_bwd_ps<2, float, true>), grid, dim3(256), 0, stream, dy, (const float*)smask,
+                    dconv, g.Wo, Cq, act, (int)rows, amax);
+    } else {
+        return DASR_E_UNSUPPORTED;
+    }
+    DASR_RETURN_LAUNCH_STATUS();
 }
 int conv_epilogue_bwd_bf16(const ConvGeom& g, const bf16_t* dy, const bf16_t* y, bf16_t* dconv, int act, int ps_r,
                            void* stream) {
diff --git a/depth-aware-endoscopy-sr_amd/csrc/conv_kernels.h b/depth-aware-endoscopy-sr_amd/csrc/conv_kernels.h
--- a/depth-aware-endoscopy-sr_amd/csrc/conv_kernels.h
+++ b/depth-aware-endoscopy-sr_amd/csrc/conv_kernels.h
@@ -18,6 +18,8 @@
                     float* y, int act, int ps_r, void* stream);
 int conv_epilogue_bwd(const ConvGeom& g, const float* dy, const float* y, float* dconv, int act, int ps_r,
                       void* stream, float* amax = nullptr);
+int conv_epilogue_bwd_mask(const ConvGeom& g, const float* dy, const unsigned* smask, float* dconv, int act, int ps_r,
+                           void* stream, float* amax = nullptr);
 int conv_direct_dgrad(const ConvGeom& g, const float* dconv, const float* w, float* dx, int accumulate, void* stream);
 int conv_direct_wgrad(const ConvGeom& g, const float* x, const float* dconv, float* dw, void* stream);
 int conv_colsum(const float* m, float* out, size_t rows, int C, void* stream);
@@ -57,10 +59,12 @@
 
 bool conv_c1_supported(const ConvGeom& g);
 int conv_c1_fwd(const ConvGeom& g, const float* x, const float* w, const float* bias, float* y, int act, void* stream,
-                float* amax = nullptr);
+                float* amax = nullptr, unsigned* smask = nullptr);
 int absmax_raise(const float* x, size_t n, float* amax, void* stream);
 int conv_c1_wgrad(const ConvGeom& g, const float* x, const float* dy, const float* yact, int act, float* dw, float* dbias,
                   void* stream);
+int conv_c1_wgrad_mask(const ConvGeom& g, const float* x, const float* dy, const unsigned* smask, int act, float* dw,
+                       float* dbias, void* stream);
 
 bool conv_bf16_supported(const ConvGeom& g);
 bool conv_bf16_dgrad_supported(const ConvGeom& g);
diff --git a/depth-aware-endoscopy-sr_amd/csrc/conv_split_bf16.hip b/depth-aware-endoscopy-sr_amd/csrc/conv_split_bf16.hip
--- a/depth-aware-endoscopy-sr_amd/csrc/conv_split_bf16.hip
+++ b/depth-aware-endoscopy-sr_amd/csrc/conv_split_bf16.hip
@@ -27,6 +27,7 @@
     const float* xmax;
     const float* wmax;
     float* ymax;
+    unsigned* smask;
 };
 
 template <int N>
@@ -169,6 +170,7 @@
     return r;
 }
 
+template <int V> struct SpInt { static constexpr int value = V; };
 template <int NT, int NP, int RW = 2>
 __device__ __forceinline__ void sp_epilogue(f32x16 (&acc)[RW][NT], const ConvSplitArgs& a, char* const scr, const float* sBias,
                                             const float inv, const int x0, const int y0, const int n0, const int bb,
@@ -177,9 +179,10 @@
     const bool is_relu = a.act == DASR_ACT_RELU;
     const float slope = a.act == DASR_ACT_LRELU02 ? 0.2f : 1.f;
     const bool has_act = a.act != DASR_ACT_NONE;
-#pragma unroll
-    for (int m = 0; m < RW; ++m) {
+    auto row = [&](auto mc) __attribute__((always_inline)) {
+        constexpr int m = decltype(mc)::value;
         const int gy = y0 + rbase + m;
+        unsigned psbits[2] = {0u, 0u};
 #pragma unroll
         for (int n = 0; n < NT; ++n) {
 #pragma unroll
@@ -193,34 +196,42 @@
 #pragma unroll
                     for (int u = 0; u < 2; ++u) {
                         const int v = lane + 64 * u, pix = v >> 2, cg = v & 3;
-                        if (pix >= wvalid) continue;
-                        const float4 lo = *(const float4*)(scr + pix * SP_EPITCH + 32 * cg);
-                        const float4 hi = *(const float4*)(scr + pix * SP_EPITCH + 32 * cg + 16);
-                        float o[8] = {lo.x, lo.y, lo.z, lo.w, hi.x, hi.y, hi.z, hi.w};
-                        if (NP == 2) {
-                            const float* bp = sBias + n0 + 32 * n + 8 * cg;
-#pragma unroll
-                            for (int t = 0; t < 8; ++t) o[t] = fmaf(o[t], inv, bp[t]);
+                        unsigned bits = 0u;
+                        if (pix < wvalid) {
+                            const float4 lo = *(const float4*)(scr + pix * SP_EPITCH + 32 * cg);
+                            const float4 hi = *(const float4*)(scr + pix * SP_EPITCH + 32 * cg + 16);
+                            float o[8] = {lo.x, lo.y, lo.z, lo.w, hi.x, hi.y, hi.z, hi.w};
+                            if (NP == 2) {
+                                const float* bp = sBias + n0 + 32 * n + 8 * cg;
+#pragma unroll
+                                for (int t = 0; t < 8; ++t) o[t] = fmaf(o[t], inv, bp[t]);
+                            }
+                            const size_t idx = (((size_t)bb * a.H + gy) * a.W + x0 + pix) * a.Cout + n0 + 32 * n + 8 * cg;
+                            if (a.residual) {
+                                const float4 r0 = *(const float4*)(a.residual + idx), r1 = *(const float4*)(a.residual + idx + 4);
+                                o[0] += r0.x; o[1] += r0.y; o[2] += r0.z; o[3] += r0.w;
+                                o[4] += r1.x; o[5] += r1.y; o[6] += r1.z; o[7] += r1.w;
+                            }
+                            if (has_act) {
+#pragma unroll
+                                for (int t = 0; t < 8; ++t) o[t] = is_relu ? fmaxf(o[t], 0.f) : fmaxf(o[t], o[t] * slope);
+                            }
+                            float* yp = a.y + idx;
+                            if (a.accumulate) {
+                                const float4 o0 = *(const float4*)yp, o1 = *(const float4*)(yp + 4);
+                                o[0] += o0.x; o[1] += o0.y; o[2] += o0.z; o[3] += o0.w;
+                                o[4] += o1.x; o[5] += o1.y; o[6] += o1.z; o[7] += o1.w;
+                            }
+                            *(float4*)yp = make_float4(o[0], o[1], o[2], o[3]);
+                            *(float4*)(yp + 4) = make_float4(o[4], o[5], o[6], o[7]);
+                            om = dasr_amax4(dasr_amax4(om, make_float4(o[0], o[1], o[2], o[3])), make_float4(o[4], o[5], o[6], o[7]));
+                            if (a.smask) bits = (dasr_sign4(o[0], o[1], o[2], o[3]) | dasr_sign4(o[4], o[5], o[6], o[7]) << 4) << (8 * cg);
                         }
-                        const size_t idx = (((size_t)bb * a.H + gy) * a.W + x0 + pix) * a.Cout + n0 + 32 * n + 8 * cg;
-                        if (a.residual) {
-                            const float4 r0 = *(const float4*)(a.residual + idx), r1 = *(const float4*)(a.residual + idx + 4);
-                            o[0] += r0.x; o[1] += r0.y; o[2] += r0.z; o[3] += r0.w;
-                            o[4] += r1.x; o[5] += r1.y; o[6] += r1.z; o[7] += r1.w;
+                        if (a.smask) {
+                            bits = dasr_or_lanes4(bits);
+                            if (cg == 0 && pix < wvalid)
+                                a.smask[(((size_t)bb * a.H + gy) * a.W + x0 + pix) * (a.Cout >> 5) + ((n0 + 32 * n) >> 5)] = bits;
                         }
-                        if (has_act) {
-#pragma unroll
-                            for (int t = 0; t < 8; ++t) o[t] = is_relu ? fmaxf(o[t], 0.f) : fmaxf(o[t], o[t] * slope);
-                        }
-                        float* yp = a.y + idx;
-                        if (a.accumulate) {
-                            const float4 o0 = *(const float4*)yp, o1 = *(const float4*)(yp + 4);
-                            o[0] += o0.x; o[1] += o0.y; o[2] += o0.z; o[3] += o0.w;
-                            o[4] += o1.x; o[5] += o1.y; o[6] += o1.z; o[7] += o1.w;
-                        }
-                        *(float4*)yp = make_float4(o[0], o[1], o[2], o[3]);
-                        *(float4*)(yp + 4) = make_float4(o[4], o[5], o[6], o[7]);
-                        om = dasr_amax4(dasr_amax4(om, make_float4(o[0], o[1], o[2], o[3])), make_float4(o[4], o[5], o[6], o[7]));
                     }
                 } else {
                     const int Cq = a.Cout / 4;
@@ -240,12 +251,26 @@
                         *(float4*)yp = make_float4(o[0], o[1], o[2], o[3]);
                         *(float4*)(yp + 4) = make_float4(o[4], o[5], o[6], o[7]);
                         om = dasr_amax4(dasr_amax4(om, make_float4(o[0], o[1], o[2], o[3])), make_float4(o[4], o[5], o[6], o[7]));
+                        if (a.smask) {
+                            psbits[u] |= (dasr_sign4(o[0], o[1], o[2], o[3]) | dasr_sign4(o[4], o[5], o[6], o[7]) << 4) << (8 * n);
+                            if (n == NT - 1) {
+                                unsigned char* mp = (unsigned char*)a.smask +
+                                    (((((size_t)bb * a.H * 2 + 2 * gy + i) * ((size_t)a.W * 2) + 2 * (x0 + pix) + j) * Cq + n0 / 4) >> 3);
+                                if (NT == 4) *(unsigned*)mp = psbits[u];
+                                else if (NT == 2) *(unsigned short*)mp = (unsigned short)psbits[u];
+                                else *mp = (unsigned char)psbits[u];
+                            }
+                        }
                     }
                 }
             }
             DASR_WAVE_SYNC();
         }
-    }
+    };
+    row(SpInt<0>{});
+    if constexpr (RW > 1) row(SpInt<1>{});
+    if constexpr (RW > 2) { row(SpInt<2>{}); row(SpInt<3>{}); }
+    static_assert(RW == 1 || RW == 2 || RW == 4, "tile rows per wave");
 }
 
 template <int NT, int NP, int RW = 2, int CW = 1>
@@ -844,14 +869,16 @@
 }
 static int sp_fwd(const float* x, const float* xmax, const unsigned short* w_split, const float* wmax, const float* bias,
                   const float* residual, float* y, float* ymax, int B, int H, int W, int Cin, int Cout, int act, int ps_r,
-                  void* stream) {
+                  void* stream, unsigned* smask = nullptr) {
     DASR_CHECK_PTR(x); DASR_CHECK_PTR(w_split); DASR_CHECK_PTR(y);
     DASR_CHECK_SHAPE(B > 0);
     if (!dasr_conv3x3_split_supported(H, W, Cin, Cout)) return DASR_E_UNSUPPORTED;
     if (act < 0 || act > 2) return DASR_E_UNSUPPORTED;
     if (ps_r < 1) ps_r = 1;
     if (ps_r > 2 || (ps_r == 2 && (residual != nullptr || (Cout % 128) != 0))) return DASR_E_UNSUPPORTED;
-    ConvSplitArgs a{x, (const bf16_t*)w_split, bias, residual, y, B, H, W, Cin, Cout, 0, act, ps_r, 0, 0, 0, 0, 0, 0, xmax, wmax, ymax};
+    if (smask && ((ps_r == 2 ? Cout / 4 : Cout) % 32) != 0) return DASR_E_UNSUPPORTED;
+    ConvSplitArgs a{x, (const bf16_t*)w_split, bias, residual, y, B, H, W, Cin, Cout, 0, act, ps_r, 0, 0, 0, 0, 0, 0, xmax, wmax, ymax,
+                    smask};
     return xmax ? sp_launch<2>(a, stream) : sp_launch<3>(a, stream);
 }
 extern "C" int dasr_conv3x3_fwd_split(const float* x, const unsigned short* w_split, const float* bias,
@@ -864,6 +891,12 @@
                                        int W, int Cin, int Cout, int act, int ps_r, void* stream) {
     DASR_CHECK_PTR(xmax); DASR_CHECK_PTR(wmax);
     return sp_fwd(x, xmax, w_split, wmax, bias, residual, y, y_amax, B, H, W, Cin, Cout, act, ps_r, stream);
+}
+extern "C" int dasr_conv3x3_fwd_split2_mask(const float* x, const float* xmax, const unsigned short* w_split, const float* wmax,
+                                            const float* bias, const float* residual, float* y, float* y_amax, int* y_mask,
+                                            int B, int H, int W, int Cin, int Cout, int act, int ps_r, void* stream) {
+    DASR_CHECK_PTR(xmax); DASR_CHECK_PTR(wmax);
+    return sp_fwd(x, xmax, w_split, wmax, bias, residual, y, y_amax, B, H, W, Cin, Cout, act, ps_r, stream, (unsigned*)y_mask);
 }
 static int sp_dgrad(const float* dconv, const float* dmax, const unsigned short* w_split, const float* wmax, float* dx,
                     int accumulate, int B, int H, int W, int Cin, int Cout, void* stream) {
diff --git a/depth-aware-endoscopy-sr_amd/csrc/dasr_common.h b/depth-aware-endoscopy-sr_amd/csrc/dasr_common.h
--- a/depth-aware-endoscopy-sr_amd/csrc/dasr_common.h
+++ b/depth-aware-endoscopy-sr_amd/csrc/dasr_common.h
@@ -111,6 +111,32 @@
     return 1.f;
 }
 
+__device__ __forceinline__ float dasr_act_neg_slope(int act) {
+    return act == DASR_ACT_RELU ? 0.f : act == DASR_ACT_LRELU02 ? 0.2f : 1.f;
+}
+__device__ __forceinline__ unsigned dasr_sign4(float a, float b, float c, float d) {
+    return (a > 0.f ? 1u : 0u) | (b > 0.f ? 2u : 0u) | (c > 0.f ? 4u : 0u) | (d > 0.f ? 8u : 0u);
+}
+__device__ __forceinline__ unsigned dasr_or_lanes4(unsigned v) {
+#ifdef DASR_HIPEMU
+    v |= __shfl_xor(v, 1);
+    v |= __shfl_xor(v, 2);
+#else
+    v |= (unsigned)__builtin_amdgcn_update_dpp(0, (int)v, 0xB1, 0xF, 0xF, true);
+    v |= (unsigned)__builtin_amdgcn_update_dpp(0, (int)v, 0x4E, 0xF, 0xF, true);
+#endif
+    return v;
+}
+__device__ __forceinline__ unsigned dasr_or_lanes8(unsigned v) {
+    v = dasr_or_lanes4(v);
+#ifdef DASR_HIPEMU
+    v |= __shfl_xor(v, 4);
+#else
+    v |= (unsigned)__builtin_amdgcn_update_dpp(0, (int)v, 0x141, 0xF, 0xF, true);
+#endif
+    return v;
+}
+
 __device__ __forceinline__ float dasr_double_in_scale(float var, float eps) {
     float r1 = 1.0f / sqrtf(var + eps);
     float v2 = var / (var + eps);
diff --git a/depth-aware-endoscopy-sr_amd/graph.py b/depth-aware-endoscopy-sr_amd/graph.py
--- a/depth-aware-endoscopy-sr_amd/graph.py
+++ b/depth-aware-endoscopy-sr_amd/graph.py
@@ -19,6 +19,7 @@
 SPLIT_PIECES = 2
 FUSE_AMAX = True
 SPLIT_CONV9 = True
+SIGN_MASKS = True
 SPLIT_MIN_PIXELS = 1 << 14
 WGRAD_STREAM = False
 _SIDE = {}
@@ -268,6 +269,10 @@
          side_wgrad=False, want_stats=False, out_dtype=None):
     stats = None
     f32 = x.data.dtype == torch.float32 and out_dtype in (None, torch.float32)
+    needs = x.requires_grad or w.requires_grad or (bias is not None and bias.requires_grad) or \
+        (residual is not None and residual.requires_grad)
+    want_mask = SIGN_MASKS and tape.enabled and needs and f32
+    smask = None
     if (want_stats and FUSE_INSTNORM_STATS and f32 and act == ops.ACT_NONE and ps_r == 1 and residual is None and
             stride == 1 and pad == 1 and not transposed and tuple(w.data.shape[1:3]) == (3, 3)):
         y, mean, var = ops.conv2d_fwd_stats(x.data, w.data, bias.data if bias is not None else None)
@@ -284,9 +289,12 @@
             if w.pack is not None and isinstance(w.split, tuple):
                 tape.prepack.note_split(w.pack, w.split)
         if isinstance(w.split, tuple):
+            if want_mask and act != ops.ACT_NONE and (x.requires_grad or residual is not None or ps_r > 1):
+                Cs = w.data.shape[4] // (ps_r * ps_r)
+                smask = ops.sign_mask_buffer((x.data.shape[0], x.data.shape[1] * ps_r, x.data.shape[2] * ps_r, Cs), x.data)
             y = ops.conv3x3_fwd_split2(x.data, _amax(x), w.split, bias.data if bias is not None else None, w.data.shape[4],
                                        residual.data if residual is not None else None, act, ps_r,
-                                       amax=want_amax(tape, x.data))
+                                       amax=want_amax(tape, x.data), mask=smask)
         else:
             y = ops.conv3x3_fwd_split(x.data, w.split, bias.data if bias is not None else None, w.data.shape[4],
                                       residual.data if residual is not None else None, act, ps_r)
@@ -301,12 +309,14 @@
         y = ops.conv9_fwd_split2(x.data, _amax(x), w.data, w.split[1], bias.data if bias is not None else None)
     else:
         am = want_amax(tape, x.data) if (f32 and x.data.shape[3] in (1, 3) and ps_r == 1) else None
+        if (want_mask and act != ops.ACT_NONE and ps_r == 1 and residual is None and w.data.dtype == torch.float32 and
+                ops.conv2d_wgrad_act_fused(x.data.shape, w.data.shape[1:], stride, pad, transposed)):
+            smask = ops.sign_mask_buffer(tuple(x.data.shape[:3]) + (w.data.shape[4],), x.data)
         y = ops.conv2d_fwd(x.data, w.data, bias.data if bias is not None else None,
                            residual.data if residual is not None else None, stride, pad, transposed, act, ps_r, out_dtype,
-                           amax=am)
-    needs = x.requires_grad or w.requires_grad or (bias is not None and bias.requires_grad) or \
-        (residual is not None and residual.requires_grad)
+                           amax=am, mask=smask)
     out = Var(y, needs)
+    out.sign_mask = smask
     out.stats = stats
     x.uses += 1
     if residual is not None:
@@ -328,7 +338,7 @@
             dy.record_stream(torch.cuda.current_stream())
         if not x.requires_grad and residual is None and ps_r == 1 and act != ops.ACT_NONE:
             dw, db = ops.conv2d_wgrad_act(x.data, dy, y, wshape, act, stride, pad, transposed,
-                                          want_bias=bias is not None)
+                                          want_bias=bias is not None, mask=smask)
             accum(w, dw)
             if bias is not None:
                 accum(bias, db)
@@ -337,7 +347,8 @@
             dconv = dy
         elif act != ops.ACT_NONE or ps_r > 1:
             dconv = ops.conv2d_epilogue_bwd(dy, y, Ho, Wo, Cout, act, ps_r,
-                                            amax=want_amax(tape, dy, (B, Ho, Wo, Cout)) if isinstance(w.split, tuple) else None)
+                                            amax=want_amax(tape, dy, (B, Ho, Wo, Cout)) if isinstance(w.split, tuple) else None,
+                                            mask=smask)
         else:
             dconv = dy
         dmax = None
diff --git a/depth-aware-endoscopy-sr_amd/ops.py b/depth-aware-endoscopy-sr_amd/ops.py
--- a/depth-aware-endoscopy-sr_amd/ops.py
+++ b/depth-aware-endoscopy-sr_amd/ops.py
@@ -110,6 +110,17 @@
 def drop_amax(t):
     if t is not None and getattr(t, "_dasr_amax", None) is not None:
         t._dasr_amax = None
+
+
+def sign_mask_buffer(shape, like):
+    B, H, W, C = shape
+    if int(_lib.get().dasr_sign_mask_words(B, H, W, C)) == 0:
+        return None
+    return torch.empty((B, H, W, C // 32), dtype=torch.int32, device=like.device)
+
+
+def _pm(mask):
+    return _lib.ptr(mask, False, torch.int32)
 
 
 def add(a, b):
@@ -326,7 +337,7 @@
 
 
 def conv2d_fwd(x, w, bias=None, residual=None, stride=1, pad=1, transposed=False, act=ACT_NONE, ps_r=1, out_dtype=None,
-               amax=None):
+               amax=None, mask=None):
     B, H, W, Cin = x.shape
     KH, KW, wi, Cout = _wdims(w)
     assert wi == Cin, (w.shape, x.shape)
@@ -342,6 +353,11 @@
     if bf:
         _call("dasr_conv2d_fwd_bf16", _pa(x), _pa(w), _p(bias, True), _pa(residual, True), _pa(y), B, H, W, Cin, Ho, Wo,
               Cout, KH, KW, stride, pad, int(transposed), act, ps_r)
+    elif mask is not None:
+        assert residual is None and ps_r == 1
+        _call("dasr_conv2d_fwd_mask", _p(x), _p(w), _p(bias, True), _p(y), _p(amax, True), _pm(mask), B, H, W, Cin, Ho, Wo,
+              Cout, KH, KW, stride, pad, int(transposed), act)
+        set_amax(y, amax)
     else:
         _call("dasr_conv2d_fwd", _p(x), _p(w), _p(bias, True), _p(residual, True), _p(y), _p(amax, True), B, H, W, Cin, Ho, Wo,
               Cout, KH, KW, stride, pad, int(transposed), act, ps_r)
@@ -349,10 +365,13 @@
     return y
 
 
-def conv2d_epilogue_bwd(dy, y, Ho, Wo, Cout, act, ps_r, amax=None):
+def conv2d_epilogue_bwd(dy, y, Ho, Wo, Cout, act, ps_r, amax=None, mask=None):
     B = y.shape[0]
     dconv = empty((B, Ho, Wo, Cout), y, y.dtype)
-    if _is_bf(dy, y):
+    if mask is not None:
+        _call("dasr_conv2d_epilogue_bwd_mask", _p(dy), _pm(mask), _p(dconv), _p(amax, True), B, Ho, Wo, Cout, act, ps_r)
+        set_amax(dconv, amax)
+    elif _is_bf(dy, y):
         _call("dasr_conv2d_epilogue_bwd_bf16", _pa(dy), _pa(y), _pa(dconv), B, Ho, Wo, Cout, act, ps_r)
     else:
         _call("dasr_conv2d_epilogue_bwd", _p(dy), _p(y), _p(dconv), _p(amax, True), B, Ho, Wo, Cout, act, ps_r)
@@ -415,11 +434,26 @@
     return dw, db
 
 
-def conv2d_wgrad_act(x, dy, y, w_shape, act, stride=1, pad=1, transposed=False, want_bias=True):
+def conv2d_wgrad_act_fused(x_shape, w_shape, stride=1, pad=1, transposed=False):
+    B, H, W, Cin = x_shape
+    KH, KW, _, Cout = w_shape
+    Ho, Wo = conv_out_hw(H, W, KH, KW, stride, pad, transposed)
+    return bool(_lib.get().dasr_conv2d_wgrad_act_fused(B, H, W, Cin, Ho, Wo, Cout, KH, KW, stride, pad, int(transposed)))
+
+
+def conv2d_wgrad_act(x, dy, y, w_shape, act, stride=1, pad=1, transposed=False, want_bias=True, mask=None):
     B, H, W, Cin = x.shape
     KH, KW, _, Cout = w_shape
     _, Ho, Wo, _ = y.shape
     lib = _lib.get()
+    if mask is not None and not conv2d_wgrad_act_fused(x.shape, w_shape, stride, pad, transposed):
+        mask = None
+    if mask is not None:
+        dw = empty(w_shape, x)
+        db = empty((Cout,), x) if want_bias else None
+        _call("dasr_conv2d_wgrad_act_mask", _p(x), _p(dy), _pm(mask), _p(dw), _p(db, True), B, H, W, Cin, Ho, Wo, Cout, KH, KW,
+              stride, pad, int(transposed), act)
+        return dw, db
     if _is_bf(dy, y):
         dw = empty(w_shape, x)
         db = empty((Cout,), x) if want_bias else None
@@ -499,12 +533,16 @@
     return ws, wmax
 
 
-def conv3x3_fwd_split2(x, xmax, ws, bias, Cout, residual=None, act=ACT_NONE, ps_r=1, amax=None):
+def conv3x3_fwd_split2(x, xmax, ws, bias, Cout, residual=None, act=ACT_NONE, ps_r=1, amax=None, mask=None):
     B, H, W, Cin = x.shape
     if ps_r > 1:
         y = empty((B, H * ps_r, W * ps_r, Cout // (ps_r * ps_r)), x)
     else:
         y = empty((B, H, W, Cout), x)
+    if mask is not None:
+        _call("dasr_conv3x3_fwd_split2_mask", _p(x), _p(xmax), _lib.ptr(ws[0], False, torch.float16), _p(ws[1]), _p(bias, True),
+              _p(residual, True), _p(y), _p(amax, True), _pm(mask), B, H, W, Cin, Cout, act, ps_r)
+        return set_amax(y, amax)
     _call("dasr_conv3x3_fwd_split2", _p(x), _p(xmax), _lib.ptr(ws[0], False, torch.float16), _p(ws[1]), _p(bias, True),
           _p(residual, True), _p(y), _p(amax, True), B, H, W, Cin, Cout, act, ps_r)
     return set_amax(y, amax)
diff --git a/depth-aware-endoscopy-sr_amd/tape.py b/depth-aware-endoscopy-sr_amd/tape.py
--- a/depth-aware-endoscopy-sr_amd/tape.py
+++ b/depth-aware-endoscopy-sr_amd/tape.py
@@ -3,7 +3,7 @@
 
 class Var:
     __slots__ = ("data", "grad", "requires_grad", "name", "uses", "epilogue", "grad_is_preact", "event",
-                 "grad_event", "stats", "split", "amax", "pack")
+                 "grad_event", "stats", "split", "amax", "pack", "sign_mask")
 
     def __init__(self, data, requires_grad=False, name=None):
         self.data = data
@@ -19,6 +19,7 @@
         self.split = None
         self.amax = None
         self.pack = None
+        self.sign_mask = None
 
     @property
     def shape(self):
diff --git a/include/dasr.h b/include/dasr.h
--- a/include/dasr.h
+++ b/include/dasr.h
@@ -45,12 +45,18 @@
 int dasr_conv2d_fwd(const float* x, const float* w_hwio, const float* bias, const float* residual, float* y, float* y_amax,
                     int B, int H, int W, int Cin, int Ho, int Wo, int Cout, int KH, int KW, int stride, int pad,
                     int transposed, int act, int ps_r, void* stream);
+size_t dasr_sign_mask_words(int B, int H, int W, int C);
+int dasr_conv2d_fwd_mask(const float* x, const float* w_hwio, const float* bias, float* y, float* y_amax, int* y_mask, int B,
+                         int H, int W, int Cin, int Ho, int Wo, int Cout, int KH, int KW, int stride, int pad, int transposed,
+                         int act, void* stream);
 size_t dasr_conv2d_fwd_stats_workspace(int B, int H, int W, int Cin, int Cout);
 int dasr_conv2d_fwd_stats(const float* x, const float* w, const float* bias, float* y, float* mean, float* var,
                           void* workspace, size_t workspace_bytes, int B, int H, int W, int Cin, int Cout, void* stream);
 
 int dasr_conv2d_epilogue_bwd(const float* dy, const float* y, float* dconv, float* dconv_amax, int B, int Ho, int Wo,
                              int Cout, int act, int ps_r, void* stream);
+int dasr_conv2d_epilogue_bwd_mask(const float* dy, const int* y_mask, float* dconv, float* dconv_amax, int B, int Ho, int Wo,
+                                  int Cout, int act, int ps_r, void* stream);
 int dasr_conv2d_dgrad(const float* dconv, const float* w_hwio, float* dx, int accumulate, int B, int H, int W, int Cin,
                       int Ho, int Wo, int Cout, int KH, int KW, int stride, int pad, int transposed, void* stream);
 int dasr_conv2d_dgrad_act_supported(int B, int H, int W, int Cin, int Ho, int Wo, int Cout, int KH, int KW, int stride,
@@ -70,6 +76,10 @@
                           float* dconv_scratch, void* workspace, size_t workspace_bytes, int B, int H, int W, int Cin,
                           int Ho, int Wo, int Cout, int KH, int KW, int stride, int pad, int transposed, int act,
                           void* stream);
+
+int dasr_conv2d_wgrad_act_mask(const float* x, const float* dy, const int* y_mask, float* dw_hwio, float* dbias, int B, int H,
+                               int W, int Cin, int Ho, int Wo, int Cout, int KH, int KW, int stride, int pad, int transposed,
+                               int act, void* stream);
 
 int dasr_conv3x3_split_supported(int H, int W, int Cin, int Cout);
 size_t dasr_conv3x3_split_weights_bytes(int Cin, int Cout);
@@ -97,6 +107,9 @@
 int dasr_conv3x3_fwd_split2(const float* x, const float* xmax, const unsigned short* w_split, const float* wmax,
                             const float* bias, const float* residual, float* y, float* y_amax, int B, int H, int W, int Cin,
                             int Cout, int act, int ps_r, void* stream);
+int dasr_conv3x3_fwd_split2_mask(const float* x, const float* xmax, const unsigned short* w_split, const float* wmax,
+                                 const float* bias, const float* residual, float* y, float* y_amax, int* y_mask, int B, int H,
+                                 int W, int Cin, int Cout, int act, int ps_r, void* stream);
 int dasr_conv3x3_dgrad_split2(const float* dconv, const float* dmax, const unsigned short* w_split, const float* wmax,
                               float* dx, int accumulate, int B, int H, int W, int Cin, int Cout, void* stream);
 int dasr_conv3x3_wgrad_split2(const float* x, const float* xmax, const float* dconv, const float* dmax, float* dw_hwio,
```
